# MrOlm/inStrain

Measured on AMD Instinct MI355X. Metric: Gbp profiled/s, higher is better.
Workload: dtype u32

## Files before the change

include/instrain_amd.h:

```cpp
#ifndef INSTRAIN_AMD_H
#define INSTRAIN_AMD_H

#include <stdint.h>

#ifdef __cplusplus
extern "C" {
#endif

#define ISX_OK 0
#define ISX_ERR_ARG (-1)
#define ISX_ERR_HIP (-2)
#define ISX_ERR_CAPACITY (-3)
#define ISX_ERR_MM_RANGE (-4)
#define ISX_ERR_IO (-5)
#define ISX_ERR_STATE (-6)

#define ISX_ABI_VERSION 5


typedef struct isx_ctx isx_ctx;
typedef struct isx_batch isx_batch;
typedef struct isx_bam isx_bam;
struct isx_bam_params_s;
struct isx_bam_info_s;
// ... 231 lines not shown
int isx_genes_create(isx_ctx *ctx, int64_t n_genes, const isx_gene *genes, const char *seq, int64_t seq_bytes, isx_genes **out);
void isx_genes_destroy(isx_genes *g);
int isx_genes_sites(isx_genes *g, double *sites, float *device_ms);
int isx_batch_profile_genes(isx_batch *b, isx_genes *g, int32_t n_scaffolds, const int64_t *scaffold_bounds, const int32_t *gene_first,
                            const int32_t *gene_last, isx_gene_cov *cov_out, uint8_t *scaffold_flags, float *device_ms);
int isx_genes_profile_snvs(isx_genes *g, int32_t n_scaffolds, const int64_t *scaffold_bounds, const int32_t *gene_first,
                           const int32_t *gene_last, int64_t n_snv, const isx_snv *snv, int32_t n_levels, isx_gene_mutation *mut_out,
                           isx_gene_snv_count *cnt_out, float *device_ms);

typedef struct isx_pipe isx_pipe;

typedef struct {
    int64_t max_pos;
    int64_t max_obs;
    int32_t max_splits;
    int32_t depth;
    int32_t host_threads;
    int32_t pin_threads;
    double jump_slack;
    int32_t want_counts;
    int32_t ring_kib;
    int32_t stage_async;
    int32_t lean_output;
    int64_t max_segs;
} isx_pipe_params;

typedef struct {
    uint32_t gpos;
    float clon_rarefied;
} isx_rare;

typedef struct {
    uint32_t gpos;
    uint32_t coverage;
} isx_sat;

typedef struct {
    int64_t ticket;
    int64_t n_pos, n_obs;
    isx_sizes sizes;
    const uint16_t *coverage16;
    const float *clon;
    const isx_rare *rare;
    int64_t n_rare, n_saturated;
    const uint32_t *counts;
    const float *clon_rarefied;
    const isx_snv *snv;
    isx_batch *batch;
    float encode_ms;
    float h2d_ms, kernel_ms, d2h_ms;
    float collect_wait_ms;
    int32_t record_bytes;
    int32_t encode_passes;
    int64_t h2d_bytes, d2h_bytes;
    const isx_ld *ld;
    const uint8_t *coverage8;
    const isx_rare *clon_sparse;
    int64_t n_clon;
    const isx_sat *saturated;
    const uint8_t *coverage4;
    const uint16_t *cov_rows;
    const uint32_t *cov_row_window;
    int64_t n_cov_rows;
    int32_t cov_window, pad_cov;
    const void *lev_mask;
    const void *lev_cov;
    const uint32_t *lev_win_off;
    const isx_rare *lev_clon, *lev_rare;
    const isx_sat *lev_sat;
    int64_t n_lev, n_lev_clon, n_lev_rare, n_lev_sat;
    int32_t lev_mask_bytes, lev_cov_bytes, lev_window, n_lev_windows, lev_min_cov, pad_lev;
    uint64_t rows_checksum;
} isx_pipe_result;

int isx_levels_expand(const isx_pipe_result *r, int32_t host_threads, uint32_t *gpos, uint32_t *mm_cov, float *clon, float *clon_rarefied);

int isx_pipe_create(isx_ctx *ctx, const isx_params *params, const isx_pipe_params *pp, isx_pipe **out);
void isx_pipe_destroy(isx_pipe *p);
int isx_pipe_submit(isx_pipe *p, int64_t n_pos, const uint8_t *ref, int32_t n_splits, const int64_t *split_bounds,
                    int64_t n_obs, const isx_obs *obs, const uint32_t *pair, int64_t *ticket);
int isx_pipe_submit_bam(isx_pipe *p, isx_bam *bam, const struct isx_bam_params_s *bp, const int32_t *refs, int32_t n_refs,
                        const uint8_t *ref, int32_t n_splits, const int64_t *split_bounds, struct isx_bam_info_s *info,
                        int64_t *ticket);
int isx_pipe_collect(isx_pipe *p, int64_t ticket, isx_pipe_result *out);
int isx_pipe_release(isx_pipe *p, int64_t ticket);
int isx_pipe_fetch_entries(isx_pipe *p, int64_t ticket, isx_entry *out);
int isx_pipe_fetch_entries_shrunk(isx_pipe *p, int64_t ticket, uint32_t *gpos, uint32_t *mm_cov, float *clon, float *clon_rarefied);


#define ISX_SEG_BASES 150
#define ISX_SEG_WORDS 15
#define ISX_SEG_SKIP_WORD 0x24924924u
#define ISX_DREC_WORDS 8
#define ISX_DREC_EXC 6
#define ISX_DREC_EXC_FULL 3
#define ISX_DREC_DUAL 0x80000000u
#define ISX_DREC_NO_EXC 0x3FFFFFFFu

typedef struct {
    int64_t n_seg;
    const uint32_t *gpos;
    const uint8_t *len;
    const uint8_t *mm;
    const uint32_t *pair;
    const uint32_t *bases;
} isx_segs;

int isx_batch_create_reads(isx_ctx *ctx, const isx_params *params, int64_t n_pos, const uint8_t *ref, int32_t n_splits,
                           const int64_t *split_bounds, const isx_segs *segs, isx_batch **out);
int isx_pipe_submit_reads(isx_pipe *p, int64_t n_pos, const uint8_t *ref, int32_t n_splits, const int64_t *split_bounds,
                          const isx_segs *segs, int64_t *ticket);

typedef struct isx_wire isx_wire;
int isx_pipe_stage_reads(isx_pipe *p, int64_t n_pos, const uint8_t *ref, int32_t n_splits, const int64_t *split_bounds,
                         const isx_segs *segs, isx_wire **out);
int isx_pipe_submit_wire(isx_pipe *p, const isx_wire *wire, int64_t *ticket);
int64_t isx_wire_bytes(const isx_wire *wire);
void isx_wire_free(isx_wire *wire);
int isx_wire_keep_reference(isx_pipe *p, isx_wire *wire);

#define ISX_PLANE_WORDS 8
typedef struct {
    int64_t n_seg;
    const uint32_t *gpos;
    const uint8_t *len;
    const uint32_t *pair;
    const uint64_t *planes;
    const uint8_t *mm;
} isx_read_planes;

typedef struct {
    const uint8_t *plane2;
    const uint8_t *nplane;
    uint64_t key;
} isx_ref_planes;

int isx_pack_ref_planes(const uint8_t *ref, int64_t n_pos, int32_t host_threads, uint8_t *plane2, uint8_t *nplane, int32_t *has_n);
int isx_planes_from_segs(const isx_segs *segs, int32_t host_threads, uint64_t *planes);
int isx_pack_read_planes(int64_t n_reads, const int64_t *ref_start, const int64_t *clip_lo, const int64_t *clip_hi,
                         const uint32_t *cigar, const int64_t *cigar_off, const char *seq, const uint8_t *qual, const int64_t *seq_off,
                         const uint32_t *pair, int32_t min_base_quality, int64_t cap_seg, uint32_t *seg_gpos,
                         uint8_t *seg_len, uint32_t *seg_pair, uint64_t *seg_planes, int64_t *n_seg);
int isx_pipe_submit_planes(isx_pipe *p, int64_t n_pos, const isx_ref_planes *ref, int32_t n_splits, const int64_t *split_bounds,
                           const isx_read_planes *reads, int64_t *ticket);
int isx_pipe_stage_planes(isx_pipe *p, int64_t n_pos, const isx_ref_planes *ref, int32_t n_splits, const int64_t *split_bounds,
                          const isx_read_planes *reads, isx_wire **out);
int isx_pipe_set_reference_budget(isx_pipe *p, int64_t mib);
int isx_host_register(const void *ptr, int64_t bytes);
int isx_host_unregister(const void *ptr);
int isx_encode_planes(const isx_read_planes *reads, const isx_ref_planes *ref, int64_t n_pos, int32_t host_threads, int32_t slack_groups,
                      int64_t cap_rec, int64_t ring_records, uint32_t *rec, uint32_t *gbase, int64_t *n_rec, int64_t *need_slack);
int isx_encode_planes_mm(const isx_read_planes *reads, const isx_ref_planes *ref, int64_t n_pos, int32_t n_mm_bins, int32_t host_threads, int32_t slack_groups,
                         int64_t cap_rec, int64_t ring_records, uint32_t *rec, uint32_t *gbase, int64_t *n_rec, int64_t *need_slack);

int isx_count_read_segs(int64_t n_reads, const uint32_t *cigar, const int64_t *cigar_off, const int64_t *ref_start,
                        const int64_t *clip_lo, const int64_t *clip_hi, int64_t *n_seg);
int isx_pack_reads(int64_t n_reads, const int64_t *ref_start, const int64_t *clip_lo, const int64_t *clip_hi,
                   const uint32_t *cigar, const int64_t *cigar_off, const char *seq, const uint8_t *qual, const int64_t *seq_off,
                   const uint8_t *mm, const uint32_t *pair, int32_t min_base_quality, int64_t cap_seg, uint32_t *seg_gpos,
                   uint8_t *seg_len, uint8_t *seg_mm, uint32_t *seg_pair, uint32_t *seg_bases, int64_t *n_seg);

int isx_encode_segs(const isx_segs *segs, int64_t n_pos, int32_t n_mm_bins, int32_t host_threads, int64_t cap_rec, uint32_t *rec,
                    uint32_t *gbase, uint32_t *pair_out, int64_t *n_rec);
int64_t isx_seg_records_needed(const uint32_t *gpos, int64_t n_seg, int32_t host_threads);
int isx_encode_segs_ring(const isx_segs *segs, int64_t n_pos, int32_t n_mm_bins, int32_t host_threads, int64_t cap_rec, int64_t ring_records,
                         uint32_t *rec, uint32_t *gbase, uint32_t *pair_out, int64_t *n_rec);

int isx_encode_delta(const isx_segs *segs, const uint8_t *ref, int64_t n_pos, int32_t n_mm_bins, int32_t host_threads, int32_t slack_groups,
                     int64_t cap_rec, int64_t ring_records, uint32_t *rec, uint32_t *gbase, uint32_t *pair_out, int64_t *n_rec, int64_t *need_slack);
int64_t isx_delta_records_needed(const uint32_t *gpos, int64_t n_seg, int32_t host_threads, int32_t slack_groups);

int isx_encode_obs(const isx_obs *obs, const uint32_t *pair, int64_t n_obs, int64_t n_pos, int32_t record_bytes,
                   int32_t host_threads, double slack, int64_t cap_rec, void *rec, uint32_t *gbase, uint32_t *pair_out,
                   int64_t *n_rec, int32_t *passes);
int isx_encode_obs_ring(const isx_obs *obs, const uint32_t *pair, int64_t n_obs, int64_t n_pos, int32_t record_bytes,
                        int32_t host_threads, double slack, int64_t cap_rec, int64_t ring_records, void *rec,
                        uint32_t *gbase, uint32_t *pair_out, int64_t *n_rec, int32_t *passes);

typedef struct {
    int64_t in_off;
    int32_t in_len;
    int32_t out_len;
    int64_t out_off;
} isx_bgzf_block;
int isx_bgzf_index(const uint8_t *image, int64_t n_bytes, int64_t cap_blocks, isx_bgzf_block *blocks, int64_t *n_blocks, int64_t *out_bytes);
int isx_bgzf_inflate_device(isx_ctx *ctx, const uint8_t *image, int64_t n_bytes, const isx_bgzf_block *blocks, int64_t n_blocks,
                            uint8_t *out, int64_t out_bytes, float *kernel_ms);
int isx_bgzf_inflate_host(const uint8_t *image, int64_t n_bytes, const isx_bgzf_block *blocks, int64_t n_blocks, uint8_t *out, int64_t out_bytes);
int isx_bgzf_inflate_fast(const uint8_t *image, int64_t n_bytes, const isx_bgzf_block *blocks, int64_t n_blocks, uint8_t *out, int64_t out_bytes);

typedef struct isx_bam_params_s {
    double min_read_ani;
    int32_t min_mapq;
    double max_insert_relative;
    int32_t min_insert;
    int32_t min_base_quality;
    int32_t skip_mm;
    int32_t window_length;
    int32_t pairing_filter;
} isx_bam_params;

typedef struct isx_bam_info_s {
    int32_t n_refs;
    int32_t n_splits;
    int64_t n_reads;
    int64_t n_pos;
    int64_t n_obs;
    int64_t n_pairs;
    int64_t unfiltered_pairs, filtered_pairs;
    int64_t filtered_bases;
    double median_insert;
    int32_t max_mm;
    int32_t pad;
    int64_t unfiltered_reads, unfiltered_singletons, filtered_singletons;
    int64_t n_segs;
} isx_bam_info;

int isx_bam_open(const char *path, isx_bam **out);
void isx_bam_close(isx_bam *bam);
void isx_bam_close_wait(isx_bam *bam);
int isx_bam_set_threads(isx_bam *bam, int32_t threads);
int isx_bam_ref(const isx_bam *bam, int32_t i, const char **name, int64_t *length, int64_t *flat_offset);
int isx_bam_set_priority_reads(isx_bam *bam, int64_t n, const char *names, const int64_t *offs);
int isx_bam_scan(isx_bam *bam, isx_bam_info *info );
int isx_bam_scan_part(isx_bam *bam, int32_t part, int32_t n_parts, isx_bam_info *info );
int isx_bam_set_wanted_refs(isx_bam *bam, const int32_t *refs, int32_t n);
int isx_bam_insert_sizes(isx_bam *bam, int64_t *out, int64_t cap, int64_t *n);
int isx_bam_filter(isx_bam *bam, const isx_bam_params *p, double median_insert , isx_bam_info *info);
int isx_bam_pair_keys(isx_bam *bam, uint64_t *h1, uint64_t *h2, int32_t *tid, int64_t *info4, int64_t cap, int64_t *n);
int isx_bam_set_cross_names(isx_bam *bam, int64_t n, const int64_t *entry, const int64_t *occurrences, const int64_t *info4);
int isx_bam_filter_insert_sizes(isx_bam *bam, int64_t *out, int64_t cap, int64_t *n);
int isx_bam_set_r2m(isx_bam *bam, int32_t ref, int64_t n, const char *names, const int64_t *offs, const int32_t *mm );
int isx_bam_set_mm_cap(isx_bam *bam, int32_t cap);
int isx_bam_mm_levels(const isx_bam *bam, int32_t *levels, int32_t cap, int32_t *n);
int isx_bam_set_mm_levels(isx_bam *bam, const int32_t *levels, int32_t n);
int isx_bam_batch_pair_names(const isx_bam *bam, int64_t *n, int64_t *name_bytes, char *names, int64_t *offs);
int isx_bam_r2m(const isx_bam *bam, int32_t ref, int64_t *n, int64_t *name_bytes, char *names, int64_t *offs, int32_t *mm);
int isx_bam_drop_names(isx_bam *bam);
int isx_bam_ref_counts(const isx_bam *bam, int64_t *reads, int64_t *filtered_pairs);
int isx_bam_expand_refs(isx_bam *bam, const isx_bam_params *p, const int32_t *refs, int32_t n_refs, isx_bam_info *info);
int isx_bam_segment_refs(isx_bam *bam, const isx_bam_params *p, const int32_t *refs, int32_t n_refs, isx_bam_info *info, int64_t *n_seg);
int isx_bam_copy_segs(const isx_bam *bam, uint32_t *gpos, uint8_t *len, uint8_t *mm, uint32_t *pair, uint32_t *bases,
                      int64_t *split_bounds, int32_t *split_ref);
int isx_bam_copy_read_planes(const isx_bam *bam, uint64_t *planes);
int isx_bam_expand_region(isx_bam *bam, const isx_bam_params *p, int32_t ref, int64_t start, int64_t stop, isx_bam_info *info);
int isx_bam_expand(isx_bam *bam, const isx_bam_params *p, isx_bam_info *info);
int isx_bam_copy(const isx_bam *bam, isx_obs *obs, uint32_t *pair, int64_t *split_bounds, int32_t *split_ref);
int isx_bam_view(const isx_bam *bam, const isx_obs **obs, const uint32_t **pair);

#ifdef __cplusplus
}
#endif
#endif
```

instrain_amd/_lib.py:

```python
import ctypes as C
import os

import numpy as np

_HERE = os.path.dirname(os.path.abspath(__file__))
LIB_PATH = os.path.join(_HERE, "libinstrain_amd.so")
if os.environ.get("ISX_LIB"):
    LIB_PATH = os.path.abspath(os.environ["ISX_LIB"])

BGZF_BLOCK_DT = np.dtype([("in_off", np.int64), ("in_len", np.int32), ("out_len", np.int32), ("out_off", np.int64)])
OBS_DT = np.dtype([("gpos", "<u4"), ("mm", "<u2"), ("base", "u1"), ("flags", "u1")])
ENTRY_DT = np.dtype([("gpos", "<u4"), ("mm", "<u2"), ("flags", "<u2"), ("cnt", "<u4", (4,)), ("clon", "<f4"),
                     ("clon_rarefied", "<f4")])
SNV_DT = np.dtype([("gpos", "<u4"), ("mm", "<u2"), ("con_base", "u1"), ("var_base", "u1"),
                   ("allele_count", "u1"), ("cls", "u1"), ("cryptic", "u1"), ("ref_base", "u1"),
                   ("cnt", "<u4", (4,))])
LD_DT = np.dtype([("gpos_a", "<u4"), ("gpos_b", "<u4"), ("mm", "<u2"), ("allele_A", "u1"), ("allele_a", "u1"),
                  ("allele_B", "u1"), ("allele_b", "u1"), ("pad", "<u2"), ("total", "<u4"), ("countAB", "<u4"),
                  ("countAb", "<u4"), ("countaB", "<u4"), ("countab", "<u4"), ("pad2", "<u4"),
                  ("r2", "<f8"), ("d_prime", "<f8"), ("r2_normalized", "<f8"), ("d_prime_normalized", "<f8")])
AO_DT = np.dtype([("pair", "<u4"), ("gpos", "<u4"), ("order", "<u4"), ("mm", "<u2"), ("base", "u1"), ("pad", "u1")])
assert AO_DT.itemsize == 16
assert OBS_DT.itemsize == 8 and ENTRY_DT.itemsize == 32 and SNV_DT.itemsize == 28 and LD_DT.itemsize == 72


class Params(C.Structure):
    _fields_ = [("min_cov", C.c_int32), ("min_snp", C.c_int32), ("min_freq", C.c_double),
                ("rarefied_coverage", C.c_int32), ("n_mm_bins", C.c_int32), ("enable_linkage", C.c_int32),
                ("linkage_mode", C.c_int32), ("window", C.c_int32), ("seed", C.c_uint64), ("layout", C.c_int32),
                ("reserved", C.c_int32)]


LAYOUT_WIDE_RECORDS, LAYOUT_NO_SHORT_RECORDS, LAYOUT_NO_PACKED_COUNTERS, LAYOUT_SEG64_RECORDS = 1, 2, 4, 8


class PipeParams(C.Structure):
    _fields_ = [("max_pos", C.c_int64), ("max_obs", C.c_int64), ("max_splits", C.c_int32), ("depth", C.c_int32),
                ("host_threads", C.c_int32), ("pin_threads", C.c_int32), ("jump_slack", C.c_double),
                ("want_counts", C.c_int32), ("ring_kib", C.c_int32), ("stage_async", C.c_int32), ("lean_output", C.c_int32),
                ("max_segs", C.c_int64)]


SEG_BASES, SEG_WORDS, SEG_SKIP_WORD = 150, 15, 0x24924924


class Segs(C.Structure):
    _fields_ = [("n_seg", C.c_int64), ("gpos", C.c_void_p), ("len", C.c_void_p), ("mm", C.c_void_p), ("pair", C.c_void_p),
                ("bases", C.c_void_p)]


PLANE_WORDS = 8
LAYOUT_MM_ENTRIES = 16
LAYOUT_MM_DELTA_RECORDS = 32
ABI_VERSION = 5


class ReadPlanes(C.Structure):
    _fields_ = [("n_seg", C.c_int64), ("gpos", C.c_void_p), ("len", C.c_void_p), ("pair", C.c_void_p), ("planes", C.c_void_p), ("mm", C.c_void_p)]


class RefPlanes(C.Structure):
    _fields_ = [("plane2", C.c_void_p), ("nplane", C.c_void_p), ("key", C.c_uint64)]


RARE_DT = np.dtype([("gpos", "<u4"), ("clon_rarefied", "<f4")])
CLON_DT = np.dtype([("gpos", "<u4"), ("clon", "<f4")])
SAT_DT = np.dtype([("gpos", "<u4"), ("coverage", "<u4")])


class Sizes(C.Structure):
    _fields_ = [(n, C.c_int64) for n in ("n_entries", "n_snv", "n_sites", "n_allele_obs", "n_increments",
                                         "n_edges", "n_ld")]


class Timings(C.Structure):
    _fields_ = [(n, C.c_float) for n in ("pileup_ms", "sites_ms", "allele_ms", "group_ms", "incr_ms", "ld_ms",
                                         "total_ms")] + \
               [(n, C.c_int32) for n in ("pileup_blocks", "pileup_threads", "pileup_lds_bytes", "pileup_window")] + \
               [("mfma_ms", C.c_float), ("dense_tiles", C.c_int32), ("dense_macs", C.c_int64), ("dense_bytes", C.c_int64),
                ("record_bytes", C.c_int32), ("pad", C.c_int32)]


class PipeResult(C.Structure):
    _fields_ = [("ticket", C.c_int64), ("n_pos", C.c_int64), ("n_obs", C.c_int64), ("sizes", Sizes),
                ("coverage16", C.c_void_p), ("clon", C.c_void_p), ("rare", C.c_void_p), ("n_rare", C.c_int64),
                ("n_saturated", C.c_int64), ("counts", C.c_void_p), ("clon_rarefied", C.c_void_p), ("snv", C.c_void_p),
                ("batch", C.c_void_p),
                ("encode_ms", C.c_float), ("h2d_ms", C.c_float), ("kernel_ms", C.c_float), ("d2h_ms", C.c_float),
                ("collect_wait_ms", C.c_float), ("record_bytes", C.c_int32), ("encode_passes", C.c_int32),
                ("h2d_bytes", C.c_int64), ("d2h_bytes", C.c_int64), ("ld", C.c_void_p),
                ("coverage8", C.c_void_p), ("clon_sparse", C.c_void_p), ("n_clon", C.c_int64), ("saturated", C.c_void_p),
                ("coverage4", C.c_void_p), ("cov_rows", C.c_void_p), ("cov_row_window", C.c_void_p), ("n_cov_rows", C.c_int64),
                ("cov_window", C.c_int32), ("pad_cov", C.c_int32),
                ("lev_mask", C.c_void_p), ("lev_cov", C.c_void_p), ("lev_win_off", C.c_void_p), ("lev_clon", C.c_void_p), ("lev_rare", C.c_void_p),
                ("lev_sat", C.c_void_p), ("n_lev", C.c_int64), ("n_lev_clon", C.c_int64), ("n_lev_rare", C.c_int64), ("n_lev_sat", C.c_int64),
                ("lev_mask_bytes", C.c_int32), ("lev_cov_bytes", C.c_int32), ("lev_window", C.c_int32), ("n_lev_windows", C.c_int32),
                ("lev_min_cov", C.c_int32), ("pad_lev", C.c_int32), ("rows_checksum", C.c_uint64)]


class BamParams(C.Structure):
    _fields_ = [("min_read_ani", C.c_double), ("min_mapq", C.c_int32), ("max_insert_relative", C.c_double),
                ("min_insert", C.c_int32), ("min_base_quality", C.c_int32), ("skip_mm", C.c_int32),
                ("window_length", C.c_int32), ("pairing_filter", C.c_int32)]


PAIRING_FILTERS = {"paired_only": 0, "non_discordant": 1, "all_reads": 2}


class BamInfo(C.Structure):
    _fields_ = [("n_refs", C.c_int32), ("n_splits", C.c_int32), ("n_reads", C.c_int64), ("n_pos", C.c_int64),
                ("n_obs", C.c_int64), ("n_pairs", C.c_int64), ("unfiltered_pairs", C.c_int64),
                ("filtered_pairs", C.c_int64), ("filtered_bases", C.c_int64), ("median_insert", C.c_double),
                ("max_mm", C.c_int32), ("pad", C.c_int32), ("unfiltered_reads", C.c_int64),
                ("unfiltered_singletons", C.c_int64), ("filtered_singletons", C.c_int64), ("n_segs", C.c_int64)]


SCAFFOLD_LEVEL_DT = np.dtype([("nonzero", "<i8"), ("sum_cov", "<u8"), ("sumsq_cov", "<u8"), ("median_cov", "<f8"),
                              ("counted", "<i8"), ("sum_clon", "<f8"), ("median_clon", "<f8"),
                              ("counted_rarefied", "<i8"), ("sum_clon_rarefied", "<f8"),
                              ("median_clon_rarefied", "<f8"), ("mm", "<i4"), ("present", "<i4")])
assert SCAFFOLD_LEVEL_DT.itemsize == 88
GENOME_LEVEL_DT = np.dtype([("n", "<i8"), ("sum_cov", "<u8"), ("sumsq_cov", "<u8"), ("median_cov", "<f8"), ("mm", "<i4"), ("pad", "<i4")])
assert GENOME_LEVEL_DT.itemsize == 40
GENOME_COV_DT = np.dtype([("n", "<i8"), ("sum_cov", "<u8"), ("sumsq_cov", "<u8"), ("max_cov", "<u4"), ("pad", "<u4")])
SNV_LEVEL_DT = np.dtype([(n, "<u4") for n in ("divergent", "sns", "snv", "con", "pop")])
LD_LEVEL_DT = np.dtype([("n", "<i8"), ("n_r2", "<i8"), ("n_dprime", "<i8"), ("sum_distance", "<i8"), ("sum_r2", "<f8"), ("sum_dprime", "<f8")])
assert GENOME_COV_DT.itemsize == 32 and SNV_LEVEL_DT.itemsize == 20 and LD_LEVEL_DT.itemsize == 48


COMPARE_LEVEL_DT = np.dtype([("both", "<i8"), ("either", "<i8"), ("mm", "<i4"), ("present_a", "<i4"),
                             ("present_b", "<i4"), ("pad", "<i4"), ("consensus_snps", "<i8"), ("population_snps", "<i8")])
assert COMPARE_LEVEL_DT.itemsize == 48
COMPARE_SNP_DT = np.dtype([("gpos", "<u4"), ("mm", "<u2"), ("consensus_snp", "u1"), ("population_snp", "u1"),
                           ("has_a", "u1"), ("has_b", "u1"), ("con_a", "u1"), ("ref_a", "u1"), ("var_a", "u1"),
                           ("con_b", "u1"), ("ref_b", "u1"), ("var_b", "u1"), ("cnt_a", "<u4", (4,)), ("cnt_b", "<u4", (4,))])
assert COMPARE_SNP_DT.itemsize == 48


GENE_DT = np.dtype([("start", "<i8"), ("end", "<i8"), ("seq_off", "<i8"), ("strand", "<i4"), ("pad", "<i4")])
GENE_COV_DT = np.dtype([("sum_cov", "<u8"), ("nonzero", "<u4"), ("counted", "<u4"), ("sum_clon", "<f8")])
GENE_SNV_COUNT_DT = np.dtype([(n, "<u4") for n in ("divergent", "sns", "sns_n", "sns_s", "snv", "snv_n", "snv_s")])
GENE_MUTATION_DT = np.dtype([("gene", "<i4"), ("k", "<i4"), ("type", "u1"), ("aa_old", "u1"), ("aa_new", "u1"), ("n_genes", "u1"),
                             ("pad", "<u4")])
assert GENE_DT.itemsize == 32 and GENE_COV_DT.itemsize == 24 and GENE_SNV_COUNT_DT.itemsize == 28 and GENE_MUTATION_DT.itemsize == 16
GENE_LEVEL_PRESENT, GENE_COV_ANY, GENE_CLON_ANY = 1, 2, 4


ERR_CAPACITY = -3


class IsxError(RuntimeError):
    def __init__(self, code, msg):
        super().__init__("libinstrain_amd error %d: %s" % (code, msg))
        self.code = code


SYMBOLS = ["isx_last_error", "isx_abi_version", "isx_ctx_create", "isx_ctx_destroy", "isx_ctx_reserve_cus", "isx_set_null_model",
           "isx_batch_create", "isx_batch_create_reads", "isx_batch_destroy", "isx_batch_run", "isx_batch_launch", "isx_batch_wait", "isx_batch_sizes", "isx_batch_timings",
           "isx_batch_fetch_entries", "isx_batch_fetch_dense", "isx_batch_fetch_snv", "isx_batch_fetch_ld", "isx_batch_fetch_allele_obs",
           "isx_batch_summarize", "isx_batch_summarize_genomes", "isx_batch_genome_coverage", "isx_snv_level_counts", "isx_ld_level_sums", "isx_compare_coverage", "isx_compare_scaffolds", "isx_compare_fetch_snps",
           "isx_genes_create", "isx_genes_destroy", "isx_genes_sites", "isx_batch_profile_genes", "isx_genes_profile_snvs",
           "isx_pipe_create", "isx_pipe_destroy", "isx_pipe_submit", "isx_pipe_submit_reads", "isx_pipe_stage_reads", "isx_pipe_submit_wire", "isx_wire_bytes", "isx_wire_free", "isx_wire_keep_reference", "isx_pipe_submit_bam", "isx_encode_segs", "isx_encode_segs_ring", "isx_seg_records_needed", "isx_encode_delta", "isx_delta_records_needed", "isx_count_read_segs", "isx_pack_reads", "isx_pipe_collect", "isx_pipe_release", "isx_pipe_fetch_entries", "isx_pipe_fetch_entries_shrunk", "isx_levels_expand", "isx_encode_obs", "isx_encode_obs_ring",
           "isx_pack_ref_planes", "isx_planes_from_segs", "isx_pack_read_planes", "isx_pipe_submit_planes", "isx_pipe_stage_planes", "isx_encode_planes", "isx_encode_planes_mm", "isx_pipe_set_reference_budget", "isx_host_register", "isx_host_unregister",
           "isx_bgzf_index", "isx_bgzf_inflate_device", "isx_bgzf_inflate_host", "isx_bgzf_inflate_fast",
           "isx_bam_open", "isx_bam_close", "isx_bam_close_wait", "isx_bam_set_threads", "isx_bam_ref", "isx_bam_set_priority_reads", "isx_bam_scan", "isx_bam_scan_part",
           "isx_bam_insert_sizes", "isx_bam_set_wanted_refs", "isx_bam_pair_keys", "isx_bam_set_cross_names", "isx_bam_filter_insert_sizes", "isx_bam_filter", "isx_bam_set_r2m", "isx_bam_r2m", "isx_bam_drop_names", "isx_bam_batch_pair_names", "isx_bam_set_mm_cap", "isx_bam_mm_levels", "isx_bam_set_mm_levels", "isx_bam_ref_counts",
           "isx_bam_expand_refs", "isx_bam_segment_refs", "isx_bam_copy_segs", "isx_bam_copy_read_planes", "isx_bam_expand_region", "isx_bam_expand", "isx_bam_copy", "isx_bam_view"]

_lib = None


def load():
    global _lib
    if _lib is not None:
        return _lib
    if not os.path.exists(LIB_PATH):
        raise IsxError(-2, "%s not built: run `python -c 'import __graft_entry__ as g; g.build()'` "
                           "(hipcc --offload-arch=gfx950)" % LIB_PATH)
    lib = C.CDLL(LIB_PATH)
    vp, i32, i64 = C.c_void_p, C.c_int32, C.c_int64
    lib.isx_last_error.restype = C.c_char_p
    lib.isx_abi_version.restype = C.c_int
    if lib.isx_abi_version() != ABI_VERSION:
        raise IsxError(-6, "%s has ABI version %d, this package binds version %d: rebuild it (python -c 'import __graft_entry__ as g; g.build()')"
                       % (LIB_PATH, lib.isx_abi_version(), ABI_VERSION))
    lib.isx_ctx_create.argtypes = [C.c_int, C.POINTER(vp)]
    lib.isx_ctx_destroy.argtypes = [vp]
    lib.isx_ctx_reserve_cus.argtypes = [vp, C.c_int]
    lib.isx_bgzf_index.argtypes = [vp, i64, i64, vp, C.POINTER(i64), C.POINTER(i64)]
    lib.isx_bgzf_inflate_device.argtypes = [vp, vp, i64, vp, i64, vp, i64, C.POINTER(C.c_float)]
    lib.isx_bgzf_inflate_host.argtypes = [vp, i64, vp, i64, vp, i64]
    lib.isx_bgzf_inflate_fast.argtypes = [vp, i64, vp, i64, vp, i64]
    lib.isx_ctx_destroy.restype = None
    lib.isx_set_null_model.argtypes = [vp, vp, i64, i32]
    lib.isx_batch_create.argtypes = [vp, C.POINTER(Params), i64, vp, i32, vp, i64, vp, vp, C.POINTER(vp)]
    lib.isx_batch_create_reads.argtypes = [vp, C.POINTER(Params), i64, vp, i32, vp, C.POINTER(Segs), C.POINTER(vp)]
    lib.isx_pipe_submit_reads.argtypes = [vp, i64, vp, i32, vp, C.POINTER(Segs), C.POINTER(i64)]
    lib.isx_pipe_stage_reads.argtypes = [vp, i64, vp, i32, vp, C.POINTER(Segs), C.POINTER(vp)]
    lib.isx_pipe_submit_wire.argtypes = [vp, vp, C.POINTER(i64)]
    lib.isx_wire_bytes.argtypes = [vp]
    lib.isx_wire_bytes.restype = i64
    lib.isx_wire_free.argtypes = [vp]
    lib.isx_wire_keep_reference.argtypes = [vp, vp]
    lib.isx_wire_free.restype = None
    lib.isx_encode_segs.argtypes = [C.POINTER(Segs), i64, i32, i32, i64, vp, vp, vp, C.POINTER(i64)]
    lib.isx_encode_segs_ring.argtypes = [C.POINTER(Segs), i64, i32, i32, i64, i64, vp, vp, vp, C.POINTER(i64)]
    lib.isx_encode_delta.argtypes = [C.POINTER(Segs), vp, i64, i32, i32, i32, i64, i64, vp, vp, vp, C.POINTER(i64), C.POINTER(i64)]
    lib.isx_delta_records_needed.argtypes = [vp, i64, i32, i32]
    lib.isx_delta_records_needed.restype = i64
    lib.isx_seg_records_needed.argtypes = [vp, i64, i32]
    lib.isx_seg_records_needed.restype = i64
    lib.isx_count_read_segs.argtypes = [i64, vp, vp, vp, vp, vp, C.POINTER(i64)]
    lib.isx_pack_reads.argtypes = [i64, vp, vp, vp, vp, vp, vp, vp, vp, vp, vp, i32, i64, vp, vp, vp, vp, vp, C.POINTER(i64)]
    lib.isx_batch_destroy.argtypes = [vp]
    lib.isx_batch_destroy.restype = None
    lib.isx_batch_run.argtypes = [vp]
    lib.isx_batch_launch.argtypes = [vp]
    lib.isx_batch_wait.argtypes = [vp]
    lib.isx_batch_sizes.argtypes = [vp, C.POINTER(Sizes)]
    lib.isx_batch_timings.argtypes = [vp, C.POINTER(Timings)]
    for f in ("isx_batch_fetch_entries", "isx_batch_fetch_snv", "isx_batch_fetch_ld", "isx_batch_fetch_allele_obs"):
        getattr(lib, f).argtypes = [vp, vp]
    lib.isx_batch_fetch_dense.argtypes = [vp, vp, vp, vp]
    lib.isx_batch_summarize.argtypes = [vp, i32, vp, vp, C.POINTER(C.c_float)]
    lib.isx_batch_summarize_genomes.argtypes = [vp, i32, vp, i32, vp, i32, vp, C.POINTER(C.c_float)]
    lib.isx_batch_genome_coverage.argtypes = [vp, i32, vp, vp, i32, i32, i32, vp, vp, C.POINTER(C.c_float)]
    lib.isx_snv_level_counts.argtypes = [vp, i32, vp, i64, vp, i32, vp, C.POINTER(C.c_float)]
    lib.isx_ld_level_sums.argtypes = [vp, i32, vp, i64, vp, i32, vp, C.POINTER(C.c_float)]
    lib.isx_compare_coverage.argtypes = [vp, vp, i32, vp, i32, vp, C.POINTER(C.c_float)]
    lib.isx_compare_scaffolds.argtypes = [vp, vp, i32, vp, i32, C.c_double, vp, C.POINTER(i64), C.POINTER(C.c_float)]
    lib.isx_compare_fetch_snps.argtypes = [vp, vp]
    lib.isx_genes_create.argtypes = [vp, i64, vp, C.c_char_p, i64, C.POINTER(vp)]
    lib.isx_genes_destroy.argtypes = [vp]
    lib.isx_genes_destroy.restype = None
    lib.isx_genes_sites.argtypes = [vp, vp, C.POINTER(C.c_float)]
    lib.isx_batch_profile_genes.argtypes = [vp, vp, i32, vp, vp, vp, vp, vp, C.POINTER(C.c_float)]
    lib.isx_genes_profile_snvs.argtypes = [vp, i32, vp, vp, vp, i64, vp, i32, vp, vp, C.POINTER(C.c_float)]
    lib.isx_pipe_create.argtypes = [vp, C.POINTER(Params), C.POINTER(PipeParams), C.POINTER(vp)]
    lib.isx_pipe_destroy.argtypes = [vp]
    lib.isx_pipe_destroy.restype = None
    lib.isx_pipe_submit.argtypes = [vp, i64, vp, i32, vp, i64, vp, vp, C.POINTER(i64)]
    lib.isx_pipe_submit_bam.argtypes = [vp, vp, C.POINTER(BamParams), vp, i32, vp, i32, vp, C.POINTER(BamInfo), C.POINTER(i64)]
    lib.isx_pipe_collect.argtypes = [vp, i64, C.POINTER(PipeResult)]
    lib.isx_pipe_release.argtypes = [vp, i64]
    lib.isx_pipe_fetch_entries.argtypes = [vp, i64, vp]
    lib.isx_pipe_fetch_entries_shrunk.argtypes = [vp, i64, vp, vp, vp, vp]
    lib.isx_levels_expand.argtypes = [C.POINTER(PipeResult), i32, vp, vp, vp, vp]
    lib.isx_encode_obs.argtypes = [vp, vp, i64, i64, i32, i32, C.c_double, i64, vp, vp, vp, C.POINTER(i64), C.POINTER(i32)]
    lib.isx_encode_obs_ring.argtypes = [vp, vp, i64, i64, i32, i32, C.c_double, i64, i64, vp, vp, vp, C.POINTER(i64), C.POINTER(i32)]
    lib.isx_bam_open.argtypes = [C.c_char_p, C.POINTER(vp)]
    lib.isx_bam_close.argtypes = [vp]
    lib.isx_bam_close.restype = None
    lib.isx_bam_close_wait.argtypes = [vp]
    lib.isx_bam_close_wait.restype = None
    lib.isx_bam_expand.argtypes = [vp, C.POINTER(BamParams), C.POINTER(BamInfo)]
    lib.isx_bam_set_threads.argtypes = [vp, i32]
    lib.isx_bam_set_priority_reads.argtypes = [vp, i64, C.c_char_p, vp]
    lib.isx_bam_scan.argtypes = [vp, C.POINTER(BamInfo)]
    lib.isx_bam_scan_part.argtypes = [vp, i32, i32, C.POINTER(BamInfo)]
    lib.isx_bam_set_wanted_refs.argtypes = [vp, vp, i32]
    lib.isx_bam_insert_sizes.argtypes = [vp, vp, i64, C.POINTER(i64)]
    lib.isx_bam_filter_insert_sizes.argtypes = [vp, vp, i64, C.POINTER(i64)]
    lib.isx_bam_pair_keys.argtypes = [vp, vp, vp, vp, vp, i64, C.POINTER(i64)]
    lib.isx_bam_set_cross_names.argtypes = [vp, i64, vp, vp, vp]
    lib.isx_bam_filter.argtypes = [vp, C.POINTER(BamParams), C.c_double, C.POINTER(BamInfo)]
    lib.isx_bam_set_r2m.argtypes = [vp, i32, i64, C.c_char_p, vp, vp]
    lib.isx_bam_drop_names.argtypes = [vp]
    lib.isx_bam_r2m.argtypes = [vp, i32, C.POINTER(i64), C.POINTER(i64), vp, vp, vp]
    lib.isx_bam_batch_pair_names.argtypes = [vp, C.POINTER(i64), C.POINTER(i64), vp, vp]
    lib.isx_bam_set_mm_cap.argtypes = [vp, i32]
    lib.isx_bam_mm_levels.argtypes = [vp, vp, i32, vp]
    lib.isx_bam_set_mm_levels.argtypes = [vp, vp, i32]
    lib.isx_bam_ref_counts.argtypes = [vp, vp, vp]
    lib.isx_bam_expand_region.argtypes = [vp, C.POINTER(BamParams), i32, i64, i64, C.POINTER(BamInfo)]
    lib.isx_bam_expand_refs.argtypes = [vp, C.POINTER(BamParams), vp, i32, C.POINTER(BamInfo)]
    lib.isx_bam_segment_refs.argtypes = [vp, C.POINTER(BamParams), vp, i32, C.POINTER(BamInfo), C.POINTER(i64)]
    lib.isx_bam_copy_segs.argtypes = [vp, vp, vp, vp, vp, vp, vp, vp]
    lib.isx_bam_copy_read_planes.argtypes = [vp, vp]
    lib.isx_pack_ref_planes.argtypes = [vp, i64, i32, vp, vp, C.POINTER(i32)]
    lib.isx_planes_from_segs.argtypes = [C.POINTER(Segs), i32, vp]
    lib.isx_pack_read_planes.argtypes = [i64, vp, vp, vp, vp, vp, vp, vp, vp, vp, i32, i64, vp, vp, vp, vp, C.POINTER(i64)]
    lib.isx_pipe_submit_planes.argtypes = [vp, i64, C.POINTER(RefPlanes), i32, vp, C.POINTER(ReadPlanes), C.POINTER(i64)]
    lib.isx_pipe_set_reference_budget.argtypes = [vp, i64]
    lib.isx_host_register.argtypes = [vp, i64]
    lib.isx_host_unregister.argtypes = [vp]
    lib.isx_pipe_stage_planes.argtypes = [vp, i64, C.POINTER(RefPlanes), i32, vp, C.POINTER(ReadPlanes), C.POINTER(vp)]
    lib.isx_encode_planes.argtypes = [C.POINTER(ReadPlanes), C.POINTER(RefPlanes), i64, i32, i32, i64, i64, vp, vp, C.POINTER(i64), C.POINTER(i64)]
    lib.isx_encode_planes_mm.argtypes = [C.POINTER(ReadPlanes), C.POINTER(RefPlanes), i64, i32, i32, i32, i64, i64, vp, vp, C.POINTER(i64), C.POINTER(i64)]
    lib.isx_bam_ref.argtypes = [vp, i32, C.POINTER(C.c_char_p), C.POINTER(i64), C.POINTER(i64)]
    lib.isx_bam_copy.argtypes = [vp, vp, vp, vp, vp]
    lib.isx_bam_view.argtypes = [vp, C.POINTER(vp), C.POINTER(vp)]
    _lib = lib
    return lib


def check(rc):
    if rc != 0:
        raise IsxError(rc, load().isx_last_error().decode(errors="replace"))
```

instrain_amd/csrc/isx_api.hip:

```cpp
#include <algorithm>
#include <atomic>
#include <cmath>
#include <chrono>
#include <cstdlib>
#include <cstring>
#include <map>
#include <mutex>
#include <string>
#include <unordered_map>
#include <thread>
#include <type_traits>
#include <vector>
#include <unistd.h>
#include <sys/prctl.h>
#include <time.h>

#include "isx_batch.h"
#include "seg_encode.h"

static thread_local std::string g_err;
void isx_set_error(const std::string &msg) { g_err = msg; }

namespace {
struct BlockCache {
// ... 19 lines not shown
        const size_t m = (v + (((size_t)1 << e) - 1)) >> e;
        return m << e;
    }
    int current() const
    {
        int d = -1;
        if (per_device && hipGetDevice(&d) != hipSuccess) d = -1;
        return d;
    }
    void trim(int dev = -2)
    {
        std::vector<std::pair<int, void *>> dead;
        {
            std::lock_guard<std::mutex> lk(mu);
            for (auto it = free_blocks.begin(); it != free_blocks.end();) {
                if (dev < -1 || it->first.dev == dev) {
                    dead.emplace_back(it->first.dev, it->second);
                    cached[it->first.dev] -= it->first.cls;
                    it = free_blocks.erase(it);
                } else ++it;
            }
        }
        int keep = -1;
        const bool sw = per_device && hipGetDevice(&keep) == hipSuccess;
        for (auto &d : dead) {
            if (sw && d.first >= 0) (void)hipSetDevice(d.first);
            (void)raw_free(d.second);
        }
        if (sw && keep >= 0) (void)hipSetDevice(keep);
    }
    hipError_t get(void **p, size_t bytes)
    {
        const Key k{current(), class_of(bytes)};
        {
            std::lock_guard<std::mutex> lk(mu);
            auto it = free_blocks.find(k);
            if (it != free_blocks.end()) {
                *p = it->second;
                free_blocks.erase(it);
                cached[k.dev] -= k.cls;
                live[*p] = k;
                return hipSuccess;
            }
        }
        hipError_t e = raw_alloc(p, k.cls);
        if (e != hipSuccess) {
            (void)hipGetLastError();
            trim();
            e = raw_alloc(p, k.cls);
            if (e != hipSuccess) return e;
        }
        std::lock_guard<std::mutex> lk(mu);
        live[*p] = k;
        return hipSuccess;
    }
    void put(void *p)
    {
        if (!p) return;
        {
            std::lock_guard<std::mutex> lk(mu);
            auto it = live.find(p);
            if (it != live.end()) {
                const Key k = it->second;
                live.erase(it);
                if (cached[k.dev] + k.cls <= limit_of(k.dev)) { free_blocks.emplace(k, p); cached[k.dev] += k.cls; return; }
            }
        }
        (void)raw_free(p);
    }
};
hipError_t raw_dev_alloc(void **p, size_t n) { return hipMalloc(p, n); }
hipError_t raw_dev_free(void *p) { return hipFree(p); }
hipError_t raw_pin_alloc(void **p, size_t n) { return hipHostMalloc(p, n, hipHostMallocDefault); }
hipError_t raw_pin_free(void *p) { return hipHostFree(p); }
size_t dev_limit(int dev)
{
    static std::mutex mu;
    static std::map<int, size_t> lim;
    std::lock_guard<std::mutex> lk(mu);
    auto it = lim.find(dev);
    if (it != lim.end()) return it->second;
    size_t v = (size_t)8 << 30;
    hipDeviceProp_t pr;
    if (dev >= 0 && hipGetDeviceProperties(&pr, dev) == hipSuccess) v = pr.totalGlobalMem / 6;
    else (void)hipGetLastError();
    lim[dev] = v;
    return v;
}
size_t pin_limit(int)
{
    static const size_t v = [] {
        const long pages = sysconf(_SC_PHYS_PAGES), psz = sysconf(_SC_PAGE_SIZE);
        const size_t ram = pages > 0 && psz > 0 ? (size_t)pages * (size_t)psz : (size_t)64 << 30;
        return std::min<size_t>((size_t)8 << 30, ram / 8);
    }();
    return v;
}
BlockCache &dev_cache() { static BlockCache c(true, dev_limit, raw_dev_alloc, raw_dev_free); return c; }
BlockCache &pin_cache() { static BlockCache c(false, pin_limit, raw_pin_alloc, raw_pin_free); return c; }
}

hipError_t isx_dev_malloc(void **p, size_t bytes) { return dev_cache().get(p, bytes); }
void isx_dev_free(void *p) { dev_cache().put(p); }
hipError_t isx_pin_malloc(void **p, size_t bytes) { return pin_cache().get(p, bytes); }
void isx_pin_free(void *p) { pin_cache().put(p); }
void isx_dev_trim() { dev_cache().trim(); pin_cache().trim(); }
hipError_t isx_raw_dev_malloc(void **p, size_t bytes)
{
    hipError_t e = hipMalloc(p, bytes);
    if (e != hipSuccess) {
        (void)hipGetLastError();
        dev_cache().trim();
        e = hipMalloc(p, bytes);
    }
    return e;
}

namespace {
struct HostRange { uintptr_t a; size_t n; };
std::mutex g_hreg_mu;
std::vector<HostRange> g_hreg;
}

bool isx_host_is_registered(const void *ptr, size_t bytes)
{
    if (!ptr || !bytes) return false;
    const uintptr_t a = reinterpret_cast<uintptr_t>(ptr);
    std::lock_guard<std::mutex> lk(g_hreg_mu);
    for (const HostRange &r : g_hreg) if (a >= r.a && a + bytes <= r.a + r.n) return true;
    return false;
}

extern "C" int isx_host_register(const void *ptr, int64_t bytes)
{
    if (!ptr || bytes <= 0) { isx_set_error("isx_host_register: bad argument"); return ISX_ERR_ARG; }
    const uintptr_t a = reinterpret_cast<uintptr_t>(ptr);
    const uintptr_t pa = a & ~(uintptr_t)4095, pe = (a + (size_t)bytes + 4095) & ~(uintptr_t)4095;
    std::lock_guard<std::mutex> lk(g_hreg_mu);
    for (const HostRange &r : g_hreg) {
        const uintptr_t ra = r.a & ~(uintptr_t)4095, re = (r.a + r.n + 4095) & ~(uintptr_t)4095;
        if (pa < re && ra < pe) { isx_set_error("isx_host_register: the range shares a page with a registered one"); return ISX_ERR_ARG; }
    }
    HIP_TRY(hipHostRegister(const_cast<void *>(ptr), (size_t)bytes, hipHostRegisterDefault));
    g_hreg.push_back(HostRange{a, (size_t)bytes});
    return ISX_OK;
}

extern "C" int isx_host_unregister(const void *ptr)
{
    const uintptr_t a = reinterpret_cast<uintptr_t>(ptr);
    std::lock_guard<std::mutex> lk(g_hreg_mu);
    for (size_t i = 0; i < g_hreg.size(); i++)
        if (g_hreg[i].a == a) {
            g_hreg.erase(g_hreg.begin() + (long)i);
            HIP_TRY(hipHostUnregister(const_cast<void *>(ptr)));
            return ISX_OK;
        }
    isx_set_error("isx_host_unregister: not a registered range");
    return ISX_ERR_ARG;
}

namespace {
__global__ void __launch_bounds__(256) k_copy_out(uint4 *__restrict__ dst, const uint4 *__restrict__ src, size_t n16)
{
    typedef uint32_t u32x4 __attribute__((ext_vector_type(4)));
    const size_t stride = (size_t)gridDim.x * blockDim.x;
    for (size_t i = (size_t)blockIdx.x * blockDim.x + threadIdx.x; i < n16; i += stride) {
        const u32x4 v = __builtin_nontemporal_load(reinterpret_cast<const u32x4 *>(src) + i);
        reinterpret_cast<u32x4 *>(dst)[i] = v;
    }
}
}

namespace {
template <class T>
__global__ void __launch_bounds__(256) k_copy_small(T *__restrict__ dst, const T *__restrict__ src, size_t n)
{
    const size_t stride = (size_t)gridDim.x * blockDim.x;
    for (size_t i = (size_t)blockIdx.x * blockDim.x + threadIdx.x; i < n; i += stride) dst[i] = src[i];
}
}

hipError_t isx_copy_to_host(void *hdst, const void *dsrc, size_t bytes, hipStream_t stream)
{
    static const size_t dma_min = [] { const char *e = getenv("ISX_D2H_DMA_MIN"); return e ? (size_t)atoll(e) : (size_t)1 << 20; }();
    return isx_copy_to_host_route(hdst, dsrc, bytes, stream, bytes < dma_min);
}

hipError_t isx_copy_to_host_route(void *hdst, const void *dsrc, size_t bytes, hipStream_t stream, bool by_kernel)
{
    if (!bytes) return hipSuccess;
    if (!by_kernel) return hipMemcpyAsync(hdst, dsrc, bytes, hipMemcpyDeviceToHost, stream);
    const uintptr_t both = reinterpret_cast<uintptr_t>(hdst) | reinterpret_cast<uintptr_t>(dsrc);
    size_t done = 0;
    if ((both & 15) == 0 && bytes >= 4096) {
        const size_t n16 = bytes / 16;
        const int blocks = (int)std::min<size_t>(128, (n16 + 1023) / 1024);
        hipLaunchKernelGGL(k_copy_out, dim3(blocks), dim3(256), 0, stream, static_cast<uint4 *>(hdst), static_cast<const uint4 *>(dsrc), n16);
        done = n16 * 16;
    }
    if (done < bytes) {
        const size_t rest = bytes - done;
        uint8_t *d = static_cast<uint8_t *>(hdst) + done;
        const uint8_t *s = static_cast<const uint8_t *>(dsrc) + done;
        const bool words = (((both | rest) & 3) == 0);
        const size_t n = words ? rest / 4 : rest;
        const int blocks = (int)std::min<size_t>(64, (n + 255) / 256);
        if (words) hipLaunchKernelGGL(k_copy_small<uint32_t>, dim3(blocks), dim3(256), 0, stream, reinterpret_cast<uint32_t *>(d), reinterpret_cast<const uint32_t *>(s), n);
        else hipLaunchKernelGGL(k_copy_small<uint8_t>, dim3(blocks), dim3(256), 0, stream, d, s, n);
    }
    return hipGetLastError();
}

namespace {
__global__ void __launch_bounds__(256) k_copy_counted(uint4 *__restrict__ dst, const uint4 *__restrict__ src, const uint32_t *cursor,
                                                      uint32_t base, uint32_t row_bytes, uint64_t cap_rows)
{
    const uint64_t rows = min((uint64_t)(*cursor - base), cap_rows);
    const uint64_t n16 = (rows * row_bytes + 15) / 16;
    const uint64_t stride = (uint64_t)gridDim.x * blockDim.x;
    for (uint64_t i = (uint64_t)blockIdx.x * blockDim.x + threadIdx.x; i < n16; i += stride) dst[i] = src[i];
}
}

hipError_t isx_copy_rows_to_host(void *hdst, const void *dsrc, const uint32_t *d_cursor, uint32_t base, uint32_t row_bytes,
                                 size_t cap_rows, hipStream_t stream)
{
    if (!cap_rows) return hipSuccess;
    if (((reinterpret_cast<uintptr_t>(hdst) | reinterpret_cast<uintptr_t>(dsrc)) & 15) != 0) return hipErrorInvalidValue;
    const size_t n16 = (cap_rows * row_bytes + 15) / 16;
    const int blocks = (int)std::min<size_t>(64, (n16 + 1023) / 1024);
    hipLaunchKernelGGL(k_copy_counted, dim3(std::max(blocks, 1)), dim3(256), 0, stream, static_cast<uint4 *>(hdst), static_cast<const uint4 *>(dsrc),
                       d_cursor, base, row_bytes, (uint64_t)cap_rows);
    return hipGetLastError();
}

namespace {
struct CopyJobs { uint4 *dst[ISX_COPY_JOBS]; const uint4 *src[ISX_COPY_JOBS]; uint32_t n16[ISX_COPY_JOBS]; uint32_t first[ISX_COPY_JOBS + 1]; int n; };
__global__ void __launch_bounds__(256) k_copy_multi(const CopyJobs J)
{
    int j = 0;
    while (j + 1 < J.n && blockIdx.x >= J.first[j + 1]) j++;
    const uint32_t nb = J.first[j + 1] - J.first[j], lb = blockIdx.x - J.first[j];
    for (uint32_t i = lb * 256u + threadIdx.x; i < J.n16[j]; i += nb * 256u) J.dst[j][i] = J.src[j][i];
}
}

hipError_t isx_copy_multi_to_host(const isx_copy_job *jobs, int n, hipStream_t stream)
{
    CopyJobs J{};
    uint32_t blocks = 0;
    for (int i = 0; i < n && J.n < ISX_COPY_JOBS; i++) {
        if (!jobs[i].bytes) continue;
        if (((reinterpret_cast<uintptr_t>(jobs[i].dst) | reinterpret_cast<uintptr_t>(jobs[i].src)) & 15) != 0 || jobs[i].bytes > ((size_t)1 << 35)) return hipErrorInvalidValue;
        const uint32_t n16 = (uint32_t)((jobs[i].bytes + 15) / 16);
        J.dst[J.n] = static_cast<uint4 *>(jobs[i].dst); J.src[J.n] = static_cast<const uint4 *>(jobs[i].src); J.n16[J.n] = n16;
        J.first[J.n] = blocks;
        blocks += std::max<uint32_t>(1, std::min<uint32_t>(64, (n16 + 1023) / 1024));
        J.n++;
    }
    if (!J.n) return hipSuccess;
    J.first[J.n] = blocks;
    hipLaunchKernelGGL(k_copy_multi, dim3(blocks), dim3(256), 0, stream, J);
    return hipGetLastError();
}

namespace {
struct ReadBack {
    uint8_t *pin = nullptr;
    size_t used = 0;
    struct Item { void *dst; size_t off, bytes; };
    std::vector<Item> items;
    bool batching = false;
    std::vector<isx_copy_job> jobs;
    static constexpr size_t CAP = (size_t)1 << 20;
    ~ReadBack() { if (pin) isx_pin_free(pin); }
};
thread_local ReadBack g_rb;
}

void isx_read_batch(bool on) { g_rb.batching = on; }

hipError_t isx_read_back(void *host_dst, const void *dsrc, size_t bytes, hipStream_t stream)
{
    if (!bytes) return hipSuccess;
    ReadBack &rb = g_rb;
    if (!rb.pin && isx_pin_malloc(reinterpret_cast<void **>(&rb.pin), ReadBack::CAP) != hipSuccess) rb.pin = nullptr;
    const size_t off = (rb.used + 15) & ~(size_t)15;
    if (!rb.pin || off + ((bytes + 15) & ~(size_t)15) > ReadBack::CAP) {
        const hipError_t e = hipMemcpyAsync(host_dst, dsrc, bytes, hipMemcpyDeviceToHost, stream);
        if (e != hipSuccess) { rb.items.clear(); rb.jobs.clear(); rb.used = 0; }
        return e;
    }
    if (rb.batching && (reinterpret_cast<uintptr_t>(dsrc) & 15) == 0 && rb.jobs.size() < ISX_COPY_JOBS) {
        rb.jobs.push_back(isx_copy_job{rb.pin + off, dsrc, bytes});
    } else {
        const hipError_t e = isx_copy_to_host(rb.pin + off, dsrc, bytes, stream);
        if (e != hipSuccess) { rb.items.clear(); rb.jobs.clear(); rb.used = 0; return e; }
    }
    rb.items.push_back({host_dst, off, bytes});
    rb.used = off + bytes;
    return hipSuccess;
}

void isx_read_drop()
{
    g_rb.items.clear();
    g_rb.jobs.clear();
// ... 1531 lines not shown
```

instrain_amd/csrc/isx_pipe.hip:

```cpp
#include <atomic>
#include <algorithm>
#include <chrono>
#include <cmath>
#include <condition_variable>
#include <cstring>
#include <deque>
#include <mutex>
#include <memory>
#include <string>
#include <thread>
#include <vector>

#include "bam_front.h"
#include "isx_batch.h"
#include "obs_encode.h"
#include "seg_encode.h"
#include "isx_summary.h"
#include <unordered_map>

namespace {

constexpr size_t ALIGN = 256;
inline size_t up(size_t v, size_t a = ALIGN) { return (v + a - 1) / a * a; }

double now_ms()
{
    return std::chrono::duration<double, std::milli>(std::chrono::steady_clock::now().time_since_epoch()).count();
}

int host_block_alloc(void **p, size_t bytes, bool pinned)
{
    *p = nullptr;
    if (pinned) { HIP_TRY(isx_pin_malloc(p, std::max<size_t>(bytes, 1))); return ISX_OK; }
    if (posix_memalign(p, 4096, std::max<size_t>(bytes, 4096)) != 0) { *p = nullptr; isx_set_error("out of host memory"); return ISX_ERR_ARG; }
    return ISX_OK;
}

void host_block_free(void *p, bool pinned)
{
    if (!p) return;
    if (pinned) isx_pin_free(p); else free(p);
}

static const bool pipe_timing = getenv("ISX_PIPE_TIMING") != nullptr;
#define H2D(p, s) ((s).h2d ? (s).h2d : (p)->s_h2d)
struct Slot {
    isx_batch *b = nullptr;
    hipStream_t h2d = nullptr;
    uint8_t *h_in = nullptr, *d_in = nullptr;
    size_t in_bytes = 0;
    size_t off_bounds = 0, off_win = 0, off_ref = 0, off_gbase = 0, off_ridx = 0, off_rec = 0;
    size_t off_pairs = 0;
    isxenc::PairRun *h_runs = nullptr;
    bool runs_pinned = true;
    uint2 *d_runs = nullptr;
    size_t cap_runs = 0;
    hipEvent_t ev_ring[2] = {nullptr, nullptr};
    bool ring_busy[2] = {false, false};
    uint8_t *h_out = nullptr;
    uint8_t *h_small = nullptr;
    size_t small_bytes = 0;
    bool out_pinned = true;
    size_t out_bytes = 0, o_counts = 0, o_clon = 0, o_clonr = 0, o_snv = 0, o_cov16 = 0, o_rare = 0;
    bool rare_dense = false;
    bool cov8 = false, clon_sparse = false;
    bool cov4 = false;
    size_t cov_rows_off = 0;
    int cov_window = 0;
    std::vector<uint32_t> cov_row_win;
    std::vector<isx_sat> sat_rows;
    bool sat_complete = true;
    void *sort_temp = nullptr;
    size_t sort_temp_bytes = 0;
    std::vector<float> clonr_big;
    std::vector<isx_rare> rare_big;
    std::vector<uint32_t> cmin, cmax, dir_pmax, dir_smin;
    std::vector<uint8_t> cany;
    std::vector<uint2> win;
    size_t o_lmask = 0, o_lwin = 0, o_lcov = 0, o_lclon = 0, o_lrare = 0;
    size_t lcov_room = 0, lclon_room = 0, lrare_room = 0;
    std::vector<uint8_t> lcov_big;
    std::vector<isx_rare> lclon_big, lrare_big;
    std::vector<isx_snv> snv_big;
    std::vector<isx_ld> ld_rows;
    uint64_t rows_checksum = 0;
    hipEvent_t ev_h2d0 = nullptr, ev_h2d1 = nullptr, ev_pass = nullptr, ev_d2h0 = nullptr, ev_d2h1 = nullptr;
    hipEvent_t ev_h2da = nullptr, ev_h2db = nullptr;
    bool h2d_split = false;
    int64_t ticket = -1;
    BamBatch *dead_batch = nullptr;
    bool ref_has_n = false;
    int state = 0;
    int rc = 0;
    std::string err;
    float finish_wait_ms = 0.f;
    float encode_ms = 0.f;
    int encode_passes = 0;
    int64_t h2d_bytes = 0, d2h_bytes = 0;
    uint16_t *d_gpos16 = nullptr;
};

static uint64_t bytes_checksum(const void *p, size_t bytes, uint64_t seed)
{
    const uint8_t *b = static_cast<const uint8_t *>(p);
    uint64_t a[4] = {seed ^ 0x9E3779B97F4A7C15ull, seed + 0xC2B2AE3D27D4EB4Full, seed ^ 0x165667B19E3779F9ull, seed + 0x27D4EB2F165667C5ull};
    const size_t n8 = bytes / 8;
    size_t i = 0;
    for (; i + 4 <= n8; i += 4) {
        uint64_t w[4];
        memcpy(w, b + 8 * i, 32);
        for (int k = 0; k < 4; k++) a[k] = a[k] * 0x100000001B3ull + w[k];
    }
    uint64_t h = (uint64_t)bytes;
    for (; i < n8; i++) { uint64_t w; memcpy(&w, b + 8 * i, 8); h = h * 0x100000001B3ull + w; }
    for (size_t j = n8 * 8; j < bytes; j++) h = h * 0x100000001B3ull + b[j];
    for (int k = 0; k < 4; k++) { h ^= a[k]; h *= 0xFF51AFD7ED558CCDull; h ^= h >> 33; }
    return h;
}

static inline size_t ref2_bytes(int64_t n_pos) { return (((size_t)n_pos + 3) / 4 + 15) & ~(size_t)15; }
static inline size_t refn_bytes(int64_t n_pos) { return (((size_t)n_pos + 7) / 8 + 15) & ~(size_t)15; }

static bool copy_ref_planes(isxenc::HostPool &pool, const isx_ref_planes *rp, int64_t n_pos, uint8_t *plane2, uint8_t *nplane)
{
    const size_t b2 = ((size_t)n_pos + 3) / 4, bn = ((size_t)n_pos + 7) / 8;
    const size_t piece = (size_t)1 << 20;
    const int t2 = (int)((b2 + piece - 1) / piece), tn = rp->nplane ? (int)((bn + piece - 1) / piece) : 0;
    std::atomic<int> any{0};
    pool.run(t2 + tn, [&](int t) {
        if (t < t2) { const size_t a = (size_t)t * piece; memcpy(plane2 + a, rp->plane2 + a, std::min(piece, b2 - a)); return; }
        const size_t a = (size_t)(t - t2) * piece, n = std::min(piece, bn - a);
        const uint8_t *src = rp->nplane + a;
        uint8_t acc = 0;
        for (size_t i = 0; i < n; i++) acc |= src[i];
        memcpy(nplane + a, src, n);
        if (acc) any.store(1, std::memory_order_relaxed);
    });
    return any.load() != 0;
}

static bool plane_any(isxenc::HostPool &pool, const uint8_t *pl, size_t bytes)
{
    const size_t piece = (size_t)1 << 20;
    const int nt = (int)((bytes + piece - 1) / piece);
    std::atomic<int> any{0};
    pool.run(nt, [&](int t) {
        const size_t a = (size_t)t * piece, n = std::min(piece, bytes - a);
        uint64_t acc = 0;
        size_t i = 0;
        for (; i + 8 <= n; i += 8) { uint64_t v; memcpy(&v, pl + a + i, 8); acc |= v; }
        for (; i < n; i++) acc |= pl[a + i];
        if (acc) any.store(1, std::memory_order_relaxed);
    });
    return any.load() != 0;
}

static uint64_t ref_plane_checksum(const uint8_t *plane2, int64_t n_pos)
{
    const size_t words = (((size_t)n_pos + 3) / 4) / 8;
    uint64_t h = 0x9E3779B97F4A7C15ull ^ (uint64_t)n_pos;
    if (!words) { for (size_t i = 0; i < ((size_t)n_pos + 3) / 4; i++) h = (h ^ plane2[i]) * 0x100000001B3ull; return h; }
    const size_t n_s = std::min<size_t>(words, 4096), step = words / n_s;
    for (size_t k = 0; k < n_s; k++) {
        uint64_t w;
        memcpy(&w, plane2 + 8 * (k * step), 8);
        h = (h ^ w) * 0x100000001B3ull;
        h ^= h >> 29;
    }
    return h;
}

int cgroup_cpus()
{
    if (FILE *f = fopen("/sys/fs/cgroup/cpu.max", "r")) {
        char q[64] = {0};
        long period = 0;
        const int n = fscanf(f, "%63s %ld", q, &period);
        fclose(f);
        if (n == 2 && period > 0 && strcmp(q, "max") != 0) return (int)std::max<long>(1, atol(q) / period);
    }
    return 0;
}

int gpu_numa_node(int device)
{
    char bus[64] = {0};
    if (hipDeviceGetPCIBusId(bus, sizeof bus, device) != hipSuccess) return -1;
    std::string id(bus);
    std::transform(id.begin(), id.end(), id.begin(), [](unsigned char ch) { return (char)std::tolower(ch); });
    int node = -1;
    if (FILE *f = fopen(("/sys/bus/pci/devices/" + id + "/numa_node").c_str(), "r")) {
        if (fscanf(f, "%d", &node) != 1) node = -1;
        fclose(f);
    }
    return node;
}

}

struct isx_pipe {
    isx_ctx *ctx = nullptr;
    isx_params prm{};
    isx_pipe_params pp{};
    std::unique_ptr<isxenc::HostPool> pool;
    std::vector<Slot> slots;
// ... 83 lines not shown
    }
    if (p->finisher.joinable()) {
        { std::lock_guard<std::mutex> lk(p->mu); p->stop = true; }
        p->cv_work.notify_all();
        p->finisher.join();
        if (p->finisher2.joinable()) p->finisher2.join();
        for (auto &t : p->more_finishers) if (t.joinable()) t.join();
    }
    (void)hipSetDevice(p->ctx->device);
    if (p->s_h2d) (void)isx_wait_stream(p->s_h2d);
    if (p->s_h2d2) (void)isx_wait_stream(p->s_h2d2);
    if (p->s_d2h) (void)isx_wait_stream(p->s_d2h);
    if (p->s_fin) (void)isx_wait_stream(p->s_fin);
    if (p->s_fin2) (void)isx_wait_stream(p->s_fin2);
    for (hipStream_t st : p->extra_fin) (void)isx_wait_stream(st);
    for (int i = 0; i < 2; i++) if (p->ctx->pstream[i]) (void)isx_wait_stream(p->ctx->pstream[i]);
    const double t_f0 = now_ms();
    double t_batch = 0, t_dev = 0, t_pin = 0;
    for (Slot &s : p->slots) {
        double t_x = now_ms();
        if (s.b) {
            isx_batch *b = s.b;
            b->d_seg = nullptr; b->d_drec = nullptr;
            b->d_rec = nullptr; b->d_rec32 = nullptr; b->d_rec16 = nullptr; b->d_gbase = nullptr; b->d_pair = nullptr;
            b->d_pair_runs = nullptr; b->d_run_index = nullptr;
            b->d_gpos = nullptr; b->d_gpos16 = nullptr; b->d_cbase = nullptr; b->d_ref = nullptr; b->d_win = nullptr;
            b->d_bounds = nullptr;
            isx_batch_destroy(b);
        }
        t_batch += now_ms() - t_x; t_x = now_ms();
        if (s.sort_temp) isx_dev_free(s.sort_temp);
        if (s.d_gpos16) isx_dev_free(s.d_gpos16);
        if (s.d_in) isx_dev_free(s.d_in);
        if (s.d_runs) isx_dev_free(s.d_runs);
        t_dev += now_ms() - t_x; t_x = now_ms();
        if (s.h_in) isx_pin_free(s.h_in);
        host_block_free(s.h_runs, s.runs_pinned);
        for (hipEvent_t e : s.ev_ring) if (e) (void)hipEventDestroy(e);
        host_block_free(s.h_out, s.out_pinned);
        if (s.h_small) isx_pin_free(s.h_small);
        t_pin += now_ms() - t_x;
        for (hipEvent_t e : {s.ev_h2d0, s.ev_h2d1, s.ev_pass, s.ev_d2h0, s.ev_d2h1, s.ev_h2da, s.ev_h2db}) if (e) (void)hipEventDestroy(e);
    }
    if (pipe_timing)
        fprintf(stderr, "[isx_pipe_destroy] device tables %.1f ms, device arena %.1f ms, pinned staging %.1f ms, total %.1f ms\n", t_batch, t_dev, t_pin, now_ms() - t_f0);
    for (auto &kv : p->ref_cache) { if (kv.second.d) isx_dev_free(kv.second.d); if (kv.second.ready) (void)hipEventDestroy(kv.second.ready); }
    for (int i = 0; i < 2; i++) {
        if (p->bounce[i]) isx_pin_free(p->bounce[i]);
        if (p->bounce_ev[i]) (void)hipEventDestroy(p->bounce_ev[i]);
    }
    if (p->s_h2d) (void)hipStreamDestroy(p->s_h2d);
    if (p->s_h2d2) (void)hipStreamDestroy(p->s_h2d2);
    if (p->s_d2h) (void)hipStreamDestroy(p->s_d2h);
    if (p->s_fin) (void)hipStreamDestroy(p->s_fin);
    if (p->s_fin2) (void)hipStreamDestroy(p->s_fin2);
    for (hipStream_t st : p->extra_fin) (void)hipStreamDestroy(st);
    delete p;
}

static int slot_batch_create(isx_pipe *p, Slot &s, int index)
{
    isx_ctx *c = p->ctx;
    const isx_params *prm = &p->prm;
    const double t_s0 = now_ms();
    isx_batch *b = new isx_batch();
    s.b = b;
    b->ctx = c; b->prm = *prm; b->M = prm->n_mm_bins;
    b->ps = getenv("ISX_ONE_PASS_QUEUE") ? 0 : (index & 1);
    b->cap_pos = p->pp.max_pos; b->cap_obs = p->pp.max_obs; b->arena = true; b->ref_packed = 2;
    b->n_pos = p->pp.max_pos; b->n_obs = p->pp.max_obs;
    b->segs = p->segs; b->drec = p->drec;
    b->lean = p->pp.lean_output != 0 && !p->pp.want_counts;
    b->lev_sparse = b->M > 1 && b->M <= 32 && p->segs && !p->pp.want_counts && !(prm->layout & ISX_LAYOUT_MM_ENTRIES);
    b->spin_us = (p->pp.host_threads > 0 && p->pp.host_threads < 8) ? 200 : 2000;
    const bool dense = b->M == 1;
    batch_pick_block(b);
    const int64_t cap_pos = p->pp.max_pos;
    for (auto &e : b->ev) HIP_TRY(hipEventCreate(&e));
    for (auto &e : b->ev_sum) HIP_TRY(hipEventCreate(&e));
    HIP_TRY(isx_dev_malloc(reinterpret_cast<void **>(&b->d_cursors), (CUR_N + 4) * sizeof(uint32_t)));
    b->d_flags = b->d_cursors + CUR_N;
    HIP_TRY(hipHostMalloc(&b->h_state, (CUR_N + 8) * sizeof(uint32_t), hipHostMallocMapped | hipHostMallocCoherent));
    memset(b->h_state, 0, (CUR_N + 8) * sizeof(uint32_t));
    HIP_TRY(hipHostGetDevicePointer(reinterpret_cast<void **>(&b->d_host_state), b->h_state, 0));
    HIP_TRY(hipMemset(b->d_cursors, 0, (CUR_N + 4) * sizeof(uint32_t)));
    {
        std::vector<uint16_t> thr = build_thresholds(c->h_lut, c->fallback, prm->min_freq);
        HIP_TRY(isx_dev_malloc(reinterpret_cast<void **>(&b->d_thr), thr.size() * sizeof(uint16_t)));
        HIP_TRY(hipMemcpy(b->d_thr, thr.data(), thr.size() * sizeof(uint16_t), hipMemcpyHostToDevice));
    }
    const uint64_t npm = (uint64_t)cap_pos * b->M;
    const uint64_t cap_obs = (uint64_t)std::max<int64_t>(p->pp.max_obs, 1);
    if (dense) {
        if (p->pp.want_counts) HIP_TRY(isx_dev_malloc(reinterpret_cast<void **>(&b->d_counts), (size_t)cap_pos * sizeof(uint4)));
        else {
            b->cap_clon = (size_t)cap_pos / 2 + 65536;
            HIP_TRY(isx_dev_malloc(reinterpret_cast<void **>(&b->d_cov8), (size_t)cap_pos));
            if (p->pp.lean_output) {
                b->cap_cov_row_win = (size_t)cap_pos / 64 + 2;
                HIP_TRY(isx_dev_malloc(reinterpret_cast<void **>(&b->d_cov_row_win), b->cap_cov_row_win * sizeof(uint32_t)));
            }
            HIP_TRY(isx_dev_malloc(reinterpret_cast<void **>(&b->d_clon_list), b->cap_clon * sizeof(uint2)));
            HIP_TRY(isx_dev_malloc(reinterpret_cast<void **>(&b->d_clon_sorted), b->cap_clon * sizeof(uint2)));
        }
        b->cap_sat = (size_t)cap_pos / 16 + 65536;
        HIP_TRY(isx_dev_malloc(reinterpret_cast<void **>(&b->d_sat), b->cap_sat * sizeof(uint2)));
        HIP_TRY(isx_dev_malloc(reinterpret_cast<void **>(&b->d_clon), (size_t)cap_pos * sizeof(float)));
        HIP_TRY(isx_dev_malloc(reinterpret_cast<void **>(&b->d_clon_r), (size_t)cap_pos * sizeof(float)));
        HIP_TRY(isx_dev_malloc(reinterpret_cast<void **>(&b->d_cov16), (size_t)cap_pos * sizeof(uint16_t)));
        if (prm->rarefied_coverage > 0) {
            b->cap_rare = p->cap_rare;
            HIP_TRY(isx_dev_malloc(reinterpret_cast<void **>(&b->d_rare), b->cap_rare * sizeof(uint2)));
        }
    } else if (b->lev_sparse) {
        b->lev_mask_bytes = b->M <= 8 ? 1 : (b->M <= 16 ? 2 : 4);
        b->cap_lev = (size_t)std::min<uint64_t>(std::min<uint64_t>(npm, 0xFFFFFFF0ull), std::max<uint64_t>((uint64_t)cap_pos * (uint64_t)std::min(b->M, 4), 1u << 20));
        HIP_TRY(isx_dev_malloc(&b->d_lev_mask, (size_t)cap_pos * b->lev_mask_bytes + 64));
        HIP_TRY(isx_dev_malloc(&b->d_lev_cov, b->cap_lev * 2 + 64));
        HIP_TRY(isx_dev_malloc(reinterpret_cast<void **>(&b->d_lev_win_off), ((size_t)cap_pos / 64 + 2) * sizeof(uint32_t)));
        if (!b->lean) {
            b->cap_entries = b->cap_lev;
            HIP_TRY(isx_dev_malloc(reinterpret_cast<void **>(&b->d_entries), b->cap_entries * sizeof(isx_entry)));
        }
        b->cap_clon = (size_t)cap_pos / 4 + 65536;
        HIP_TRY(isx_dev_malloc(reinterpret_cast<void **>(&b->d_clon_list), b->cap_clon * sizeof(uint2)));
        b->cap_sat = (size_t)cap_pos / 16 + 65536;
        HIP_TRY(isx_dev_malloc(reinterpret_cast<void **>(&b->d_sat), b->cap_sat * sizeof(uint2)));
        if (prm->rarefied_coverage > 0) {
            b->cap_rare = p->cap_rare;
            HIP_TRY(isx_dev_malloc(reinterpret_cast<void **>(&b->d_rare), b->cap_rare * sizeof(uint2)));
        }
    } else {
        b->slab_region = (size_t)(cap_pos + 2 * b->block) * (size_t)std::min(b->M, 4);
        const size_t ovf = b->M <= 4 ? 16 : (size_t)std::max<uint64_t>(1u << 20, std::min<uint64_t>(cap_obs, npm) / 4);
        if (b->slab_region + ovf >= 0xFFFFFFFFull) { isx_set_error("mm path: more than 2^32 entry slots in one batch"); return ISX_ERR_ARG; }
        b->cap_entries = b->slab_region + ovf;
        HIP_TRY(isx_dev_malloc(reinterpret_cast<void **>(&b->d_entries), b->cap_entries * sizeof(isx_entry)));
        HIP_TRY(isx_dev_malloc(reinterpret_cast<void **>(&b->d_win_nent), ((size_t)cap_pos / 64 + 2) * sizeof(uint32_t)));
    }
    b->cap_snv = (size_t)std::min<uint64_t>(npm, std::max<uint64_t>((uint64_t)cap_pos / 2, 1u << 20));
    b->cap_sites = (size_t)std::min<uint64_t>((uint64_t)cap_pos, std::max<uint64_t>((uint64_t)cap_pos / 4, 1u << 20));
    b->cap_ao = (size_t)std::max<uint64_t>(1, std::min<uint64_t>(cap_obs, std::max<uint64_t>(cap_obs / 4, 1u << 20)));
    HIP_TRY(isx_dev_malloc(reinterpret_cast<void **>(&b->d_snv), b->cap_snv * sizeof(isx_snv)));
    HIP_TRY(isx_dev_malloc(reinterpret_cast<void **>(&b->d_sites), b->cap_sites * sizeof(isx_site)));
    if (prm->enable_linkage) HIP_TRY(isx_dev_malloc(reinterpret_cast<void **>(&b->d_ao), b->cap_ao * sizeof(isx_ao)));
    if (!dense) {
        b->cap_slev = b->cap_sites * (size_t)std::min(b->M, 8);
        HIP_TRY(isx_dev_malloc(reinterpret_cast<void **>(&b->d_slev), b->cap_slev * sizeof(isx_slev)));
    }
    size_t o = 0;
    s.off_bounds = o; o = up(o + (size_t)(p->pp.max_splits + 1) * sizeof(int64_t));
    s.off_win = o; o = up(o + ((size_t)cap_pos / 64 + 2) * sizeof(uint2));
    s.off_ref = o; o = up(o + ref2_bytes(cap_pos) + refn_bytes(cap_pos));
    s.off_gbase = o; o = up(o + ((size_t)(p->cap_rec / p->G) + ISX_TAIL_GROUPS) * sizeof(uint32_t));
    s.off_ridx = o; if (prm->enable_linkage && !p->segs) o = up(o + ((size_t)p->cap_rec / ISX_CHUNK + 2) * sizeof(uint32_t));
    s.off_pairs = o; if (prm->enable_linkage && p->segs && !p->drec) o = up(o + (size_t)p->cap_rec * sizeof(uint32_t));
    s.off_rec = o;
    s.in_bytes = up(o + (size_t)p->cap_rec * p->rb + ISX_TAIL_BYTES);
    const size_t host_bytes = p->ring_half ? up(o + 2 * (size_t)p->ring_half * p->rb) : s.in_bytes;
    const double t_a0 = now_ms();
    HIP_TRY(isx_pin_malloc(reinterpret_cast<void **>(&s.h_in), host_bytes));
    const double t_a1 = now_ms();
    HIP_TRY(isx_dev_malloc(reinterpret_cast<void **>(&s.d_in), s.in_bytes));
    if (pipe_timing)
        fprintf(stderr, "[isx_pipe_create] slot %d: device tables %.1f ms, pinned input %.1f MB %.1f ms, device arena %.1f MB %.1f ms\n", index,
                t_a0 - t_s0, host_bytes / 1e6, t_a1 - t_a0, s.in_bytes / 1e6, now_ms() - t_a1);
    if (prm->enable_linkage && !p->segs) {
        s.cap_runs = (size_t)p->cap_rec / 64 + 4096;
        s.runs_pinned = p->pp.depth > 1;
        { const int hrc = host_block_alloc(reinterpret_cast<void **>(&s.h_runs), s.cap_runs * sizeof(isxenc::PairRun), s.runs_pinned); if (hrc != ISX_OK) return hrc; }
        HIP_TRY(isx_dev_malloc(reinterpret_cast<void **>(&s.d_runs), s.cap_runs * sizeof(uint2)));
    }
    if (p->ring_half) for (hipEvent_t &e : s.ev_ring) HIP_TRY(hipEventCreateWithFlags(&e, hipEventDisableTiming));
    if (prm->enable_linkage && p->rb == 4) HIP_TRY(isx_dev_malloc(reinterpret_cast<void **>(&s.d_gpos16), (size_t)p->cap_rec * sizeof(uint16_t)));
    o = 0;
    s.o_snv = o; o = up(o + p->snv_prefix * sizeof(isx_snv));
    s.o_rare = o; if (dense && prm->rarefied_coverage > 0) o = up(o + p->rare_prefix * sizeof(isx_rare));
    s.small_bytes = o;
    HIP_TRY(isx_pin_malloc(reinterpret_cast<void **>(&s.h_small), std::max<size_t>(s.small_bytes, 1)));
    o = 0;
    if (dense) {
        s.o_cov16 = o; o = up(o + (size_t)cap_pos * 2);
        s.o_clon = o; o = up(o + (size_t)cap_pos * 4);
        if (p->pp.want_counts) {
            s.o_counts = o; o = up(o + (size_t)cap_pos * 16);
            s.o_clonr = o; if (prm->rarefied_coverage > 0) o = up(o + (size_t)cap_pos * 4);
        }
    }
    if (b->lev_sparse) {
        s.o_lmask = o; o = up(o + (size_t)cap_pos * b->lev_mask_bytes);
        s.o_lwin = o; o = up(o + ((size_t)cap_pos / 64 + 2) * sizeof(uint32_t));
        s.lcov_room = (size_t)cap_pos * (size_t)std::min(b->M, 4);
        s.o_lcov = o; o = up(o + s.lcov_room);
        s.lclon_room = (size_t)cap_pos;
        s.o_lclon = o; o = up(o + s.lclon_room);
        s.lrare_room = prm->rarefied_coverage > 0 ? (size_t)cap_pos / 2 : 0;
        s.o_lrare = o; o = up(o + s.lrare_room);
    }
    s.out_bytes = o;
    const double t_o0 = now_ms();
    s.out_pinned = s.out_bytes <= ((size_t)64 << 20) || p->pp.depth > 2;
    { const int hrc = host_block_alloc(reinterpret_cast<void **>(&s.h_out), s.out_bytes, s.out_pinned); if (hrc != ISX_OK) return hrc; }
    if (pipe_timing) fprintf(stderr, "[isx_pipe_create] slot %d: %s results %.1f MB %.1f ms\n", index, s.out_pinned ? "pinned" : "pageable", s.out_bytes / 1e6, now_ms() - t_o0);
    for (hipEvent_t *e : {&s.ev_h2d0, &s.ev_h2d1, &s.ev_pass, &s.ev_d2h0, &s.ev_d2h1, &s.ev_h2da, &s.ev_h2db}) HIP_TRY(hipEventCreate(e));
    const size_t n_chunks = (size_t)(p->cap_rec / (p->segs ? (int64_t)p->G : (int64_t)ISX_CHUNK)) + 2;
    s.cmin.resize(n_chunks); s.cmax.resize(n_chunks); s.cany.resize(n_chunks);
    return ISX_OK;
}

static int finish_slot(isx_pipe *p, Slot &s, hipStream_t sfin)
{
    isx_ctx *c = p->ctx;
    isx_batch *b = s.b;
    const bool dense = b->M == 1;
    const double t0 = now_ms();
    HIP_TRY(isx_wait_event(s.ev_d2h1));
    s.finish_wait_ms = (float)(now_ms() - t0);
    const double t_c0 = now_ms();
    double t_fin = 0, t_rare = 0;
    hipStream_t ps = c->pstream[b->ps];
    bool redo = false;
    for (int attempt = 0;; attempt++) {
        uint32_t cf = 0;
        int rc = finish_pass_sizes(b, &cf, sfin);
        if (rc != ISX_OK) return rc;
        const bool cov8_overflow = !cf && dense && b->sparse_out && b->cov8_out && !b->nib_pass && (size_t)b->n_sat > b->cap_sat;
        const bool nib_overflow = !cf && dense && b->nib_pass &&
                                  ((size_t)b->n_pos / 2 + 128 + (size_t)b->n_cov_rows * (size_t)b->W * 2 > (size_t)b->n_pos * 2 ||
                                   ((size_t)b->n_cov_rows + 1) * (size_t)b->W > (size_t)(b->cap_pos ? b->cap_pos : b->n_pos));
        const bool clon_overflow = !cf && dense && b->sparse_out && b->lean && !b->clon_dense &&
                                   ((size_t)b->n_clon > b->cap_clon || (size_t)b->n_clon * 2 > (size_t)b->n_pos);
        const bool rare_overflow = !cf && dense && p->prm.rarefied_coverage > 0 && !b->rare_dense &&
                                   ((size_t)b->n_rare > p->cap_rare || (size_t)b->n_rare * 8 > (size_t)b->n_pos);
        const bool lev_overflow = !cf && b->lev_sparse && ((size_t)b->n_clon > b->cap_clon || (size_t)b->n_sat > b->cap_sat ||
                                                           (p->prm.rarefied_coverage > 0 && (size_t)b->n_rare > b->cap_rare));
        if (!cf && !cov8_overflow && !clon_overflow && !nib_overflow && !rare_overflow && !lev_overflow) break;
        if (attempt == 7) { isx_set_error("output tables still too small after 8 growth steps"); return ISX_ERR_CAPACITY; }
        if (cov8_overflow) b->cov8_out = false;
        if (nib_overflow) b->nib_out = false;
        if (clon_overflow) b->clon_dense = true;
        if (rare_overflow) b->rare_dense = true;
        if (cf && (rc = batch_grow_tables(b, cf)) != ISX_OK) return rc;
        if (lev_overflow) {
            auto regrow_list = [&](uint2 **lp, size_t *cap, size_t need) -> int {
                if (need <= *cap) return ISX_OK;
                HIP_TRY(isx_wait_stream(ps));
                if (*lp) isx_dev_free(*lp);
                *lp = nullptr;
                const size_t want = need + need / 4 + 65536;
                HIP_TRY(isx_dev_malloc(reinterpret_cast<void **>(lp), want * sizeof(uint2)));
                *cap = want;
                return ISX_OK;
            };
            if ((rc = regrow_list(&b->d_clon_list, &b->cap_clon, b->n_clon)) != ISX_OK) return rc;
            if ((rc = regrow_list(&b->d_sat, &b->cap_sat, b->n_sat)) != ISX_OK) return rc;
            if (p->prm.rarefied_coverage > 0 && (rc = regrow_list(&b->d_rare, &b->cap_rare, b->n_rare)) != ISX_OK) return rc;
        }
        if (!dense && !b->lev_sparse) b->cap_ovf = b->cap_entries - (size_t)b->n_win * b->slab;
        std::lock_guard<std::mutex> lk(p->launch_mu);
        if (dense && p->prm.rarefied_coverage > 0 && b->rare_dense)
            HIP_TRY(hipMemsetD32Async(reinterpret_cast<hipDeviceptr_t>(b->d_clon_r), 0x7FC00000, (size_t)b->n_pos, ps));
        if ((rc = launch_pass(b)) != ISX_OK) return rc;
        {
            PileupArgs pa{};
            pa.cursors = b->d_cursors; pa.host_state = b->d_host_state;
            launch_publish_state(pa, b->epoch, ps);
            b->publish_enqueued = true;
            if (c->unpublished[b->ps] == b) c->unpublished[b->ps] = nullptr;
        }
        redo = true;
    }
    s.d2h_bytes += (int64_t)(std::min((size_t)b->sizes.n_snv, p->snv_prefix) * sizeof(isx_snv));
    if (dense && p->prm.rarefied_coverage > 0) s.d2h_bytes += (int64_t)(std::min((size_t)b->n_rare, p->rare_prefix) * sizeof(isx_rare));
    auto pull = [&](void *hdst, const void *dsrc, size_t bytes) -> int {
        if (!bytes) return ISX_OK;
        HIP_TRY(isx_read_back(hdst, dsrc, bytes, sfin));
        HIP_TRY(isx_read_sync(sfin));
        return ISX_OK;
    };
    struct ReadBatch { ReadBatch() { isx_read_batch(true); } ~ReadBatch() { isx_read_drop(); } } read_batch;
    auto fetch = [&](void *hdst, const void *dsrc, size_t bytes) -> int {
        if (!bytes) return ISX_OK;
        if (!s.out_pinned) return bounce_d2h(p, hdst, dsrc, bytes, sfin);
        HIP_TRY(isx_copy_to_host(hdst, dsrc, bytes, sfin));
        return ISX_OK;
    };
    if (dense) {
        int rc = ISX_OK;
        if (redo) HIP_TRY(isx_wait_stream(ps));
        s.cov8 = false; s.cov4 = false; s.clon_sparse = false; s.sat_complete = (size_t)b->n_sat <= b->cap_sat;
        if (b->sparse_out) {
            s.cov8 = b->cov8_out && !b->nib_pass;
            if (b->nib_pass) {
                const size_t nib_bytes = ((size_t)b->n_pos + 1) / 2, rows_bytes = (size_t)b->n_cov_rows * (size_t)b->W * 2;
                s.cov4 = true; s.cov_window = b->W;
                s.cov_rows_off = (nib_bytes + 63) & ~(size_t)63;
                rc = fetch(s.h_out + s.o_cov16, b->d_cov8, nib_bytes);
                if (rc == ISX_OK) rc = fetch(s.h_out + s.o_cov16 + s.cov_rows_off, b->d_cov16, rows_bytes);
                s.cov_row_win.resize(b->n_cov_rows);
                if (rc == ISX_OK && b->n_cov_rows && isx_read_back(s.cov_row_win.data(), b->d_cov_row_win, (size_t)b->n_cov_rows * sizeof(uint32_t), sfin) != hipSuccess) {
                    isx_set_error("isx_pipe finisher: read-back of the coverage rows' windows"); isx_read_drop(); rc = ISX_ERR_HIP;
                }
                s.d2h_bytes += (int64_t)(nib_bytes + rows_bytes + (size_t)b->n_cov_rows * 4);
            } else if (s.cov8) rc = fetch(s.h_out + s.o_cov16, b->d_cov8, (size_t)b->n_pos);
            else rc = fetch(s.h_out + s.o_cov16, b->d_cov16, (size_t)b->n_pos * 2);
            if (rc != ISX_OK) return rc;
// ... 353 lines not shown
        *ticket = s.ticket;
        p->work.push_back(s.ticket);
    }
    p->cv_work.notify_one();
    return ISX_OK;
}


static int check_capacity(const isx_pipe *p, const char *who, int64_t n_pos, int64_t n_items, int64_t max_items, int32_t n_splits)
{
    if (n_pos > p->pp.max_pos || n_items > max_items || n_splits > p->pp.max_splits) {
        isx_set_error(std::string(who) + ": batch larger than the pipe was created for");
        return ISX_ERR_CAPACITY;
    }
    return ISX_OK;
}

static int slot_acquire(isx_pipe *p, const char *who, Slot **out)
{
    Slot &s = p->slots[(size_t)(p->next_ticket % (int64_t)p->slots.size())];
    {
        std::lock_guard<std::mutex> lk(p->mu);
        if (s.state != 0) { isx_set_error(std::string(who) + ": every slot is in use (collect + release the oldest batch first)"); return ISX_ERR_STATE; }
    }
    HIP_TRY(hipSetDevice(p->ctx->device));
    *out = &s;
    return ISX_OK;
}

static int queue_for_stager(isx_pipe *p, isx_pipe::StageJob &&job, const char *who, int64_t *ticket)
{
    const int rc = check_capacity(p, who, job.n_pos, job.planes ? job.reads.n_seg : job.segs.n_seg, p->pp.max_segs, (int32_t)job.bounds.size() - 1);
    if (rc != ISX_OK) return rc;
    {
        std::lock_guard<std::mutex> lk(p->mu);
        const int64_t t = p->next_promise, n = (int64_t)p->slots.size();
        const Slot &s = p->slots[(size_t)(t % n)];
        if (t - n >= p->next_ticket || s.state != 0) { isx_set_error(std::string(who) + ": every slot is in use (collect + release the oldest batch first)"); return ISX_ERR_STATE; }
        job.ticket = t;
        p->next_promise = t + 1;
        *ticket = t;
        p->stage_q.push_back(std::move(job));
    }
    p->cv_stage.notify_one();
    return ISX_OK;
}

struct RingFeed { hipError_t err = hipSuccess; size_t bytes = 0; };

static int ring_feed_install(isx_pipe *p, Slot &s, RingFeed &r, int64_t &ring_groups, std::function<void(int)> &wave_begin,
                             std::function<void(int, int64_t, int64_t)> &wave_flush)
{
    if (p->ring_half <= 0) return ISX_OK;
    HIP_TRY(hipEventRecord(s.ev_h2d0, H2D(p, s)));
    const size_t half_bytes = (size_t)p->ring_half * (size_t)p->rb, grp_bytes = (size_t)p->G * (size_t)p->rb;
    uint8_t *d_rec = s.d_in + s.off_rec;
    ring_groups = p->ring_half / (int64_t)p->G;
    wave_begin = [&s, &r](int h) {
        if (s.ring_busy[h]) { const hipError_t e = isx_wait_event(s.ev_ring[h]); if (e != hipSuccess && r.err == hipSuccess) r.err = e; s.ring_busy[h] = false; }
    };
    wave_flush = [p, &s, &r, half_bytes, grp_bytes, d_rec](int h, int64_t g0, int64_t g1) {
        const size_t n = (size_t)(g1 - g0) * grp_bytes;
        if (g0 == 0) r.bytes = 0;
        hipError_t e = hipMemcpyAsync(d_rec + (size_t)g0 * grp_bytes, s.h_in + s.off_rec + (size_t)h * half_bytes, n, hipMemcpyHostToDevice, H2D(p, s));
        if (e == hipSuccess) e = hipEventRecord(s.ev_ring[h], H2D(p, s));
        if (e != hipSuccess && r.err == hipSuccess) r.err = e;
        s.ring_busy[h] = true;
        r.bytes += n;
    };
    return ISX_OK;
}

static int slot_choose_windows(isx_pipe *p, Slot &s, uint32_t chunk, bool threads)
{
    isx_batch *b = s.b;
    DirThreads mt{*p->pool, s.dir_pmax, s.dir_smin};
    const ChunkDir dir{s.cmin.data(), s.cmax.data(), s.cany.data(), b->n_rec / chunk, chunk};
    b->W = choose_windows(b, b->n_pos, dir, threads ? &mt : nullptr, s.win, &b->packed);
    b->n_win = (int)s.win.size();
    if (s.win.size() > (size_t)p->pp.max_pos / 64 + 2) { isx_set_error("internal: window directory larger than the arena"); return ISX_ERR_STATE; }
    memcpy(s.h_in + s.off_win, s.win.data(), s.win.size() * sizeof(uint2));
    return ISX_OK;
}

constexpr double COV8_BELOW_DEPTH = 16.0;
constexpr double NIB_BELOW_DEPTH = 6.0;
constexpr double LEV_COV8_BELOW_DEPTH = 64.0;
constexpr double RARE_DENSE_OBS_FACTOR = 4.0;

static int slot_shape_pass(isx_pipe *p, Slot &s)
{
    isx_batch *b = s.b;
    const bool dense = b->M == 1;
    const double n_obs = (double)b->n_obs, n_pos = (double)b->n_pos;
    b->sparse_out = dense && b->d_clon_list != nullptr;
    b->cov8_out = b->sparse_out && n_obs < COV8_BELOW_DEPTH * n_pos;
    b->nib_out = b->cov8_out && b->lean && n_obs < NIB_BELOW_DEPTH * n_pos;
    b->clon_dense = false;
    b->rare_dense = !(b->lean && b->sparse_out) || n_obs * RARE_DENSE_OBS_FACTOR >= (double)p->prm.rarefied_coverage * n_pos;
    if (b->lev_sparse) b->lev_cov_bytes = n_obs < LEV_COV8_BELOW_DEPTH * n_pos ? 1 : 2;
    const int rc = batch_set_geometry(b);
    if (rc != ISX_OK) return rc;
    if (!dense && !b->lev_sparse) {
        const size_t used = (size_t)b->n_win * b->slab;
        if (used > b->slab_region) { isx_set_error("internal: entry slabs larger than the slot's region"); return ISX_ERR_STATE; }
        b->cap_ovf = b->cap_entries - used;
    }
    return ISX_OK;
}

static void slot_bind_inputs(isx_pipe *p, Slot &s, uint8_t *resident_ref)
{
    isx_batch *b = s.b;
    const bool linkage = p->prm.enable_linkage != 0;
    uint8_t *rec = s.d_in + s.off_rec;
    b->d_bounds = reinterpret_cast<int64_t *>(s.d_in + s.off_bounds);
    b->d_win = reinterpret_cast<uint2 *>(s.d_in + s.off_win);
    b->d_ref = resident_ref ? resident_ref : s.d_in + s.off_ref;
    b->d_ref_n = s.ref_has_n ? b->d_ref + ref2_bytes(b->n_pos) : nullptr;
    b->d_gbase = reinterpret_cast<uint32_t *>(s.d_in + s.off_gbase);
    b->d_rec16 = p->rb == 2 ? reinterpret_cast<uint16_t *>(rec) : nullptr;
    b->d_rec32 = p->rb == 4 ? reinterpret_cast<uint32_t *>(rec) : nullptr;
    if (p->segs) {
        b->d_seg = p->drec ? nullptr : reinterpret_cast<uint4 *>(rec);
        b->d_drec = p->drec ? reinterpret_cast<uint4 *>(rec) : nullptr;
        b->d_pair = linkage && !p->drec ? reinterpret_cast<uint32_t *>(s.d_in + s.off_pairs) : nullptr;
        b->d_pair_runs = nullptr; b->d_run_index = nullptr; b->n_runs = 0;
    } else {
        b->d_pair = nullptr;
        b->d_pair_runs = linkage ? s.d_runs : nullptr;
        b->d_run_index = linkage ? reinterpret_cast<uint32_t *>(s.d_in + s.off_ridx) : nullptr;
        b->d_gpos16 = s.d_gpos16; b->gpos16_shift = 5;
    }
}

static void ref_cache_insert(isx_pipe *p, Slot &s, const isx_ref_planes *rp, int64_t n_pos)
{
    const size_t rb_all = ref2_bytes(n_pos) + (s.ref_has_n ? refn_bytes(n_pos) : 0);
    if (p->ref_cache_bytes + rb_all > p->ref_cache_budget.load(std::memory_order_relaxed)) return;
    isx_pipe::RefEntry e;
    bool ok = isx_dev_malloc(reinterpret_cast<void **>(&e.d), rb_all + 64) == hipSuccess && hipEventCreateWithFlags(&e.ready, hipEventDisableTiming) == hipSuccess;
    ok = ok && hipMemcpyAsync(e.d, s.d_in + s.off_ref, rb_all, hipMemcpyDeviceToDevice, H2D(p, s)) == hipSuccess && hipEventRecord(e.ready, H2D(p, s)) == hipSuccess;
    if (ok) {
        e.bytes = rb_all; e.n_pos = n_pos; e.has_n = s.ref_has_n; e.sum = ref_plane_checksum(rp->plane2, n_pos);
        p->ref_cache_bytes += rb_all;
        p->ref_cache.emplace(rp->key, e);
    } else {
        if (e.d) isx_dev_free(e.d);
        if (e.ready) (void)hipEventDestroy(e.ready);
        (void)hipGetLastError();
    }
}

struct RefStage {
    bool early = false;
    uint8_t *resident = nullptr;
    double host_ms = 0.0;
};

static int stage_reference(isx_pipe *p, Slot &s, int64_t n_pos, const uint8_t *ref, const isx_ref_planes *rp, isxenc::SegJob &J, RefStage *out)
{
    const bool ring = p->ring_half > 0;
    const double t_r = now_ms();
    const size_t b2 = ((size_t)n_pos + 3) / 4, bn = ((size_t)n_pos + 7) / 8;
    hipStream_t st = H2D(p, s);

    const auto hit = rp && rp->key ? p->ref_cache.find(rp->key) : p->ref_cache.end();
    if (hit != p->ref_cache.end()) {
        const isx_pipe::RefEntry &e = hit->second;
        if (e.n_pos != n_pos || e.has_n != (rp->nplane != nullptr && e.has_n) || e.sum != ref_plane_checksum(rp->plane2, n_pos)) {
            isx_set_error("isx_pipe_submit_planes: the reference key stands for other planes (positions / non-ACGT plane / content differ)");
            return ISX_ERR_ARG;
        }
        s.ref_has_n = e.has_n;
        J.ref2 = rp->plane2; J.refn = e.has_n ? rp->nplane : nullptr;
        out->resident = e.d;
        HIP_TRY(hipStreamWaitEvent(st, e.ready, 0));
        if (!ring) HIP_TRY(hipEventRecord(s.ev_h2d0, st));
        HIP_TRY(hipEventRecord(s.ev_h2da, st));
        out->early = true;
        out->host_ms = now_ms() - t_r;
        return ISX_OK;
    }

    const bool first_trip = rp && rp->key && p->ref_cache_budget.load(std::memory_order_relaxed) > 0;
    if (rp && !first_trip && isx_host_is_registered(rp->plane2, b2) && (!rp->nplane || isx_host_is_registered(rp->nplane, bn))) {
        const bool any_n = rp->nplane && plane_any(*p->pool, rp->nplane, bn);
        s.ref_has_n = any_n;
        J.ref2 = rp->plane2; J.refn = any_n ? rp->nplane : nullptr;
        out->host_ms = now_ms() - t_r;
        if (!ring) HIP_TRY(hipEventRecord(s.ev_h2d0, st));
        HIP_TRY(hipMemcpyAsync(s.d_in + s.off_ref, rp->plane2, b2, hipMemcpyHostToDevice, st));
        if (any_n) HIP_TRY(hipMemcpyAsync(s.d_in + s.off_ref + ref2_bytes(n_pos), rp->nplane, bn, hipMemcpyHostToDevice, st));
        if (!ring) HIP_TRY(hipEventRecord(s.ev_h2da, st));
        out->early = true;
        return ISX_OK;
    }

    uint8_t *h2 = s.h_in + s.off_ref, *hn = h2 + ref2_bytes(n_pos);
    s.ref_has_n = rp ? copy_ref_planes(*p->pool, rp, n_pos, h2, hn) : isxenc::pack_ref_planes(*p->pool, ref, n_pos, h2, hn);
    J.ref2 = h2; J.refn = s.ref_has_n ? hn : nullptr;
    out->host_ms = now_ms() - t_r;
    static const bool late_dma = getenv("ISX_PIPE_LATE_DMA") != nullptr;
    if (late_dma) return ISX_OK;
    if (!ring) HIP_TRY(hipEventRecord(s.ev_h2d0, st));
    HIP_TRY(hipMemcpyAsync(s.d_in + s.off_ref, h2, ref2_bytes(n_pos) + (s.ref_has_n ? refn_bytes(n_pos) : 0), hipMemcpyHostToDevice, st));
    if (!ring) HIP_TRY(hipEventRecord(s.ev_h2da, st));
    out->early = true;
    if (rp && rp->key) ref_cache_insert(p, s, rp, n_pos);
    return ISX_OK;
}

static int submit_common(isx_pipe *p, int64_t n_pos, const uint8_t *ref, int32_t n_splits, const int64_t *split_bounds,
                         int64_t n_obs, isxenc::EncodeJob &J, int64_t *ticket)
{
    static const char who[] = "isx_pipe_submit";
    int rc;
    if ((rc = check_capacity(p, who, n_pos, n_obs, p->pp.max_obs, n_splits)) != ISX_OK) return rc;
    if ((rc = check_split_bounds(n_pos, n_splits, split_bounds)) != ISX_OK) return rc;
    Slot *slot = nullptr;
    if ((rc = slot_acquire(p, who, &slot)) != ISX_OK) return rc;
    Slot &s = *slot;
    isx_batch *b = s.b;
    const bool linkage = p->prm.enable_linkage != 0;

    const double t0 = now_ms();
    const bool ring = p->ring_half > 0;
    uint8_t *d_rec = s.d_in + s.off_rec;
    RingFeed feed;
    J.n_obs = n_obs; J.n_pos = n_pos; J.record_bytes = p->rb;
    J.rec = s.h_in + s.off_rec; J.gbase = reinterpret_cast<uint32_t *>(s.h_in + s.off_gbase);
    J.pair_out = nullptr;
    J.cmin = s.cmin.data(); J.cmax = s.cmax.data(); J.cany = s.cany.data();
    J.cap_rec = p->cap_rec;
    if ((rc = ring_feed_install(p, s, feed, J.ring_groups, J.wave_begin, J.wave_flush)) != ISX_OK) return rc;
    int erc = 0;
    for (int attempt = 0;; attempt++) {
        if (linkage) {
            J.runs_out = s.h_runs; J.cap_runs = s.cap_runs;
            J.run_index_out = reinterpret_cast<uint32_t *>(s.h_in + s.off_ridx);
        }
        J.slack = p->slack;
        feed.bytes = 0;
        erc = isxenc::encode_obs(*p->pool, J);
        if (erc != isxenc::ENC_OK || !linkage || J.n_runs <= s.cap_runs || attempt == 1) break;
        HIP_TRY(isx_wait_stream(H2D(p, s)));
        host_block_free(s.h_runs, s.runs_pinned); s.h_runs = nullptr;
        isx_dev_free(s.d_runs); s.d_runs = nullptr;
        s.cap_runs = J.n_runs + J.n_runs / 4 + 4096;
        { const int hrc = host_block_alloc(reinterpret_cast<void **>(&s.h_runs), s.cap_runs * sizeof(isxenc::PairRun), s.runs_pinned); if (hrc != ISX_OK) return hrc; }
        HIP_TRY(isx_dev_malloc(reinterpret_cast<void **>(&s.d_runs), s.cap_runs * sizeof(uint2)));
    }
    const double t_enc = now_ms();
    if (feed.err != hipSuccess) { isx_set_error(std::string("isx_pipe_submit: staging ring: ") + hipGetErrorString(feed.err)); return ISX_ERR_HIP; }
    if (erc == isxenc::ENC_CAPACITY) { isx_set_error("isx_pipe_submit: the stream jumps too often for the pipe's record capacity (raise jump_slack)"); return ISX_ERR_CAPACITY; }
    if (erc == isxenc::ENC_MM_RANGE) { isx_set_error("an observation has mm >= 256"); return ISX_ERR_MM_RANGE; }
    if (erc == isxenc::ENC_BAD_POS) { isx_set_error("observation gpos >= n_pos"); return ISX_ERR_ARG; }
    if (linkage) {
        if (J.n_runs > s.cap_runs) { isx_set_error("isx_pipe_submit: internal: pair-id run table did not fit after growing it"); return ISX_ERR_STATE; }
        b->n_runs = (uint32_t)J.n_runs;
    }
    if (J.passes > 1 && J.n_groups_in > 0)
        p->slack = std::max(p->slack, 1.25 * ((double)J.n_groups_real / (double)J.n_groups_in - 1.0) + 0.01);
    s.ref_has_n = isxenc::pack_ref_planes(*p->pool, ref, n_pos, s.h_in + s.off_ref, s.h_in + s.off_ref + ref2_bytes(n_pos));
    memcpy(s.h_in + s.off_bounds, split_bounds, (size_t)(n_splits + 1) * sizeof(int64_t));

    b->n_pos = n_pos; b->n_obs = n_obs; b->n_splits = n_splits; b->n_rec = (uint64_t)J.n_rec;
    b->n_pairs = (uint64_t)J.max_pair + 1;
    if ((rc = slot_choose_windows(p, s, ISX_CHUNK, false)) != ISX_OK) return rc;
    if ((rc = slot_shape_pass(p, s)) != ISX_OK) return rc;
    slot_bind_inputs(p, s, nullptr);
    s.encode_ms = (float)(now_ms() - t0);
    s.encode_passes = J.passes;
    if (pipe_timing)
        fprintf(stderr, "[isx_pipe_submit] records %.2f ms (%d pass), reference + bounds + windows %.2f ms; %lld obs, %lld runs\n",
                t_enc - t0, J.passes, now_ms() - t_enc, (long long)n_obs, (long long)J.n_runs);

    if (!ring) HIP_TRY(hipEventRecord(s.ev_h2d0, H2D(p, s)));
    const size_t ref_bytes = ref2_bytes(n_pos) + (s.ref_has_n ? refn_bytes(n_pos) : 0);
    const size_t head = (size_t)(n_splits + 1) * sizeof(int64_t) + s.win.size() * sizeof(uint2) + ref_bytes;
    memset(s.h_in + s.off_gbase + (size_t)(b->n_rec / p->G) * sizeof(uint32_t), 0, ISX_TAIL_GROUPS * sizeof(uint32_t));
    const size_t gb_bytes = ((size_t)(b->n_rec / p->G) + ISX_TAIL_GROUPS) * sizeof(uint32_t), rec_bytes = (size_t)b->n_rec * p->rb + ISX_TAIL_BYTES;
    HIP_TRY(hipMemcpyAsync(s.d_in + s.off_bounds, s.h_in + s.off_bounds, (size_t)(n_splits + 1) * sizeof(int64_t), hipMemcpyHostToDevice, H2D(p, s)));
    HIP_TRY(hipMemcpyAsync(s.d_in + s.off_win, s.h_in + s.off_win, s.win.size() * sizeof(uint2), hipMemcpyHostToDevice, H2D(p, s)));
    HIP_TRY(hipMemcpyAsync(s.d_in + s.off_ref, s.h_in + s.off_ref, ref_bytes, hipMemcpyHostToDevice, H2D(p, s)));
    HIP_TRY(hipMemcpyAsync(s.d_in + s.off_gbase, s.h_in + s.off_gbase, gb_bytes, hipMemcpyHostToDevice, H2D(p, s)));
    if (ring) {
        if (p->rb == 2) HIP_TRY(hipMemsetD8Async(reinterpret_cast<hipDeviceptr_t>(d_rec + (size_t)b->n_rec * 2), 0xFF, ISX_TAIL_BYTES, H2D(p, s)));
        else HIP_TRY(hipMemsetD32Async(reinterpret_cast<hipDeviceptr_t>(d_rec + (size_t)b->n_rec * 4), (int)ISX_PAD32, ISX_TAIL_BYTES / 4, H2D(p, s)));
        if (feed.bytes != (size_t)b->n_rec * p->rb) { isx_set_error("internal: the staging ring did not carry the whole stream"); return ISX_ERR_STATE; }
    } else {
        if (p->rb == 2) memset(s.h_in + s.off_rec + (size_t)b->n_rec * 2, 0xFF, ISX_TAIL_BYTES);
        else std::fill_n(reinterpret_cast<uint32_t *>(s.h_in + s.off_rec + (size_t)b->n_rec * 4), ISX_TAIL_BYTES / 4, (uint32_t)ISX_PAD32);
        HIP_TRY(hipMemcpyAsync(d_rec, s.h_in + s.off_rec, rec_bytes, hipMemcpyHostToDevice, H2D(p, s)));
    }
    s.h2d_bytes = (int64_t)(head + gb_bytes + rec_bytes);
    if (linkage) {
        const size_t rb = (size_t)b->n_runs * sizeof(isxenc::PairRun), ib = (size_t)(b->n_rec / ISX_CHUNK) * sizeof(uint32_t);
        HIP_TRY(hipMemcpyAsync(s.d_runs, s.h_runs, rb, hipMemcpyHostToDevice, H2D(p, s)));
        HIP_TRY(hipMemcpyAsync(s.d_in + s.off_ridx, s.h_in + s.off_ridx, ib, hipMemcpyHostToDevice, H2D(p, s)));
        s.h2d_bytes += (int64_t)(rb + ib);
    }
    HIP_TRY(hipEventRecord(s.ev_h2d1, H2D(p, s)));
    s.h2d_split = false;

    return enqueue_pass(p, s, n_pos, ticket);
}

static int encode_reads(isx_pipe *p, Slot &s, isxenc::SegJob &J, bool planes_in, RingFeed &feed)
{
    s.encode_passes = 1;
    if (!p->drec) return isxenc::encode_segs(*p->pool, J);
    std::vector<int64_t> exact;
    for (int attempt = 0;; attempt++) {
        J.slack_groups = p->dslack;
        J.task_groups = exact.empty() ? nullptr : exact.data();
        feed.bytes = 0;
        const int erc = planes_in ? isxenc::encode_planes(*p->pool, J) : isxenc::encode_delta(*p->pool, J);
        if (erc != isxenc::SEG_CAPACITY || J.need_slack <= p->dslack || attempt != 0) return erc;
        exact = J.task_need;
        int64_t tot = 0;
        for (int64_t v : exact) tot += v;
        const int64_t n_t = (int64_t)exact.size(), base_tot = J.n_rec / ISX_DREC_GROUP - n_t * p->dslack;
        p->dslack = std::max<int64_t>(p->dslack, 1 + (tot - base_tot + n_t - 1) / std::max<int64_t>(n_t, 1));
        s.encode_passes = 2;
    }
}

static int submit_segs_common(isx_pipe *p, int64_t n_pos, const uint8_t *ref, int32_t n_splits, const int64_t *split_bounds,
                              isxenc::SegJob &J, int64_t *ticket, const isx_ref_planes *rp)
{
    static const char who[] = "isx_pipe_submit_reads";
    const bool planes_in = J.in2.planes != nullptr || (bool)J.produce_planes || (J.n_seg == 0 && rp != nullptr);
    int rc;
    if ((rc = check_capacity(p, who, n_pos, J.n_seg, p->pp.max_segs, n_splits)) != ISX_OK) return rc;
    if ((rc = check_split_bounds(n_pos, n_splits, split_bounds)) != ISX_OK) return rc;
    Slot *slot = nullptr;
    if ((rc = slot_acquire(p, who, &slot)) != ISX_OK) return rc;
    Slot &s = *slot;
    isx_batch *b = s.b;
    const bool linkage = p->prm.enable_linkage != 0;

    const double t0 = now_ms();
    J.n_pos = n_pos; J.n_mm_bins = b->M;
    J.rec = reinterpret_cast<uint32_t *>(s.h_in + s.off_rec);
    J.gbase = reinterpret_cast<uint32_t *>(s.h_in + s.off_gbase);
    J.pair_out = linkage && !p->drec ? reinterpret_cast<uint32_t *>(s.h_in + s.off_pairs) : nullptr;
    J.cmin = s.cmin.data(); J.cmax = s.cmax.data(); J.cany = s.cany.data();
    J.cap_rec = p->cap_rec;
    const bool ring = p->ring_half > 0;
    RingFeed feed;
    if ((rc = ring_feed_install(p, s, feed, J.ring_groups, J.wave_begin, J.wave_flush)) != ISX_OK) return rc;
    RefStage rs;
    if (planes_in) {
        if (!p->drec) { isx_set_error("bit-plane reads need a pipe whose batches travel as reference-delta records (one mm bin, or ISX_LAYOUT_MM_DELTA_RECORDS)"); return ISX_ERR_STATE; }
        if ((rc = stage_reference(p, s, n_pos, ref, rp, J, &rs)) != ISX_OK) return rc;
    }
    if (p->drec) J.ref = ref;
    const int erc = encode_reads(p, s, J, planes_in, feed);
    const double t_enc = now_ms();
    if (feed.err != hipSuccess) { isx_set_error(std::string("isx_pipe_submit_reads: staging ring: ") + hipGetErrorString(feed.err)); return ISX_ERR_HIP; }
    if ((rc = seg_status_error(erc, "isx_pipe_submit_reads: the stream jumps too often for the pipe's record capacity (raise jump_slack)", ISX_ERR_CAPACITY)) != ISX_OK) return rc;
    if (J.n_bases > p->pp.max_obs) { isx_set_error("isx_pipe_submit_reads: more bases than the pipe's max_obs"); return ISX_ERR_CAPACITY; }
    bool early_rec = false;
    if (rs.early && !ring) {
        const size_t gb_bytes0 = (size_t)(J.n_rec / (int64_t)p->G) * sizeof(uint32_t), rec_bytes0 = (size_t)J.n_rec * (size_t)p->rb;
        HIP_TRY(hipEventRecord(s.ev_h2db, H2D(p, s)));
        if (s.off_pairs == s.off_rec && s.off_ridx == s.off_rec && s.off_rec - s.off_gbase < ((size_t)2 << 20)) {
            HIP_TRY(hipMemcpyAsync(s.d_in + s.off_gbase, s.h_in + s.off_gbase, (s.off_rec - s.off_gbase) + rec_bytes0, hipMemcpyHostToDevice, H2D(p, s)));
        } else {
            HIP_TRY(hipMemcpyAsync(s.d_in + s.off_gbase, s.h_in + s.off_gbase, gb_bytes0, hipMemcpyHostToDevice, H2D(p, s)));
            HIP_TRY(hipMemcpyAsync(s.d_in + s.off_rec, s.h_in + s.off_rec, rec_bytes0, hipMemcpyHostToDevice, H2D(p, s)));
        }
        early_rec = true;
    }
    if (!planes_in) s.ref_has_n = isxenc::pack_ref_planes(*p->pool, ref, n_pos, s.h_in + s.off_ref, s.h_in + s.off_ref + ref2_bytes(n_pos));
    const double t_ref = now_ms();
    memcpy(s.h_in + s.off_bounds, split_bounds, (size_t)(n_splits + 1) * sizeof(int64_t));

    b->n_pos = n_pos; b->n_obs = J.n_bases; b->n_splits = n_splits; b->n_rec = (uint64_t)J.n_rec;
    b->n_pairs = (uint64_t)J.max_pair + 1;
    if ((rc = slot_choose_windows(p, s, p->G, true)) != ISX_OK) return rc;
    if ((rc = slot_shape_pass(p, s)) != ISX_OK) return rc;
    slot_bind_inputs(p, s, rs.resident);
    s.encode_ms = (float)(now_ms() - t0);
    if (pipe_timing)
        fprintf(stderr, "[isx_pipe_submit_reads] records %.2f ms, reference %.2f ms, bounds + windows %.2f ms; %lld segments, %lld records%s\n",
                t_enc - t0 - rs.host_ms, t_ref - t_enc + rs.host_ms, now_ms() - t_ref, (long long)J.n_seg, (long long)J.n_rec, planes_in ? " (bit planes)" : "");
    const double t_q0 = now_ms();

    if (!ring && !rs.early) HIP_TRY(hipEventRecord(s.ev_h2d0, H2D(p, s)));
    const size_t ref_bytes = ref2_bytes(n_pos) + (s.ref_has_n ? refn_bytes(n_pos) : 0);
    const size_t head = (size_t)(n_splits + 1) * sizeof(int64_t) + s.win.size() * sizeof(uint2) + ref_bytes;
    const size_t gb_bytes = (size_t)(b->n_rec / p->G) * sizeof(uint32_t), rec_bytes = (size_t)b->n_rec * (size_t)p->rb;
    if (s.off_win - s.off_bounds < ((size_t)1 << 20)) {
        HIP_TRY(hipMemcpyAsync(s.d_in + s.off_bounds, s.h_in + s.off_bounds, (s.off_win - s.off_bounds) + s.win.size() * sizeof(uint2), hipMemcpyHostToDevice, H2D(p, s)));
    } else {
        HIP_TRY(hipMemcpyAsync(s.d_in + s.off_bounds, s.h_in + s.off_bounds, (size_t)(n_splits + 1) * sizeof(int64_t), hipMemcpyHostToDevice, H2D(p, s)));
        HIP_TRY(hipMemcpyAsync(s.d_in + s.off_win, s.h_in + s.off_win, s.win.size() * sizeof(uint2), hipMemcpyHostToDevice, H2D(p, s)));
    }
    if (!rs.early) HIP_TRY(hipMemcpyAsync(s.d_in + s.off_ref, s.h_in + s.off_ref, ref_bytes, hipMemcpyHostToDevice, H2D(p, s)));
    if (!early_rec) HIP_TRY(hipMemcpyAsync(s.d_in + s.off_gbase, s.h_in + s.off_gbase, gb_bytes, hipMemcpyHostToDevice, H2D(p, s)));
    if (ring) { if (feed.bytes != rec_bytes) { isx_set_error("internal: the staging ring did not carry the whole stream"); return ISX_ERR_STATE; } }
    else if (!early_rec) HIP_TRY(hipMemcpyAsync(s.d_in + s.off_rec, s.h_in + s.off_rec, rec_bytes, hipMemcpyHostToDevice, H2D(p, s)));
    s.h2d_bytes = (int64_t)(head + gb_bytes + rec_bytes) - (rs.resident ? (int64_t)ref_bytes : 0);
    if (linkage && !p->drec) {
        HIP_TRY(hipMemcpyAsync(s.d_in + s.off_pairs, s.h_in + s.off_pairs, (size_t)b->n_rec * sizeof(uint32_t), hipMemcpyHostToDevice, H2D(p, s)));
        s.h2d_bytes += (int64_t)b->n_rec * 4;
    }
    HIP_TRY(hipEventRecord(s.ev_h2d1, H2D(p, s)));
    s.h2d_split = early_rec;
    const double t_q1 = now_ms();
    rc = enqueue_pass(p, s, n_pos, ticket);
    if (pipe_timing) fprintf(stderr, "[isx_pipe_submit_reads] copy-in queue %.2f ms, pass + copy-out queue %.2f ms\n", t_q1 - t_q0, now_ms() - t_q1);
    return rc;
}

struct isx_wire {
    isx_pipe *pipe = nullptr;
    uint8_t *h = nullptr;
    size_t bytes = 0;
    size_t o_bounds = 0, o_win = 0, o_ref = 0, o_gbase = 0, o_pairs = 0, o_rec = 0;
    size_t bounds_bytes = 0, win_bytes = 0, ref_bytes = 0, gbase_bytes = 0, pairs_bytes = 0, rec_bytes = 0;
    int64_t n_pos = 0, n_bases = 0, n_rec = 0, n_seg = 0;
    int32_t n_splits = 0;
    uint64_t n_pairs = 0;
    int W = 0, packed = 0;
    bool ref_has_n = false;
    float stage_ms = 0.f;
    int encode_passes = 1;
    uint8_t *d_ref = nullptr;
    int device = 0;
};

static int stage_common(isx_pipe *p, int64_t n_pos, const uint8_t *ref, const isx_ref_planes *rp, int32_t n_splits, const int64_t *split_bounds,
                        const isx_segs *segs, const isx_read_planes *reads, isx_wire **out)
{
    isx_segs as_segs{};
    if (reads) { as_segs.n_seg = reads->n_seg; as_segs.gpos = reads->gpos; as_segs.len = reads->len; as_segs.pair = reads->pair; segs = &as_segs; }
    *out = nullptr;
    if (!p->segs) { isx_set_error("isx_pipe_stage_reads: not a read-level pipe (isx_pipe_params.max_segs == 0)"); return ISX_ERR_STATE; }
    const bool linkage = p->prm.enable_linkage != 0;
    if (linkage && segs->n_seg && !segs->pair) { isx_set_error("linkage needs the pair array"); return ISX_ERR_ARG; }
    int rc;
    if ((rc = check_capacity(p, "isx_pipe_stage_reads", n_pos, segs->n_seg, p->pp.max_segs, n_splits)) != ISX_OK) return rc;
    if ((rc = check_split_bounds(n_pos, n_splits, split_bounds)) != ISX_OK) return rc;
    HIP_TRY(hipSetDevice(p->ctx->device));
    const double t0 = now_ms();
    std::unique_ptr<isx_wire, void (*)(isx_wire *)> w(new isx_wire(), isx_wire_free);
    w->pipe = p; w->n_pos = n_pos; w->n_splits = n_splits; w->n_seg = segs->n_seg;
    const isx_batch *b0 = p->slots[0].b;
    const int M = b0->M;
    const size_t G = p->G, rb = (size_t)p->rb;
    auto up = [](size_t v) { return (v + 255) & ~(size_t)255; };
    isxenc::SegJob J;
    std::vector<uint32_t> cmin, cmax;
    std::vector<uint8_t> cany;
    std::vector<int64_t> exact;
    for (int attempt = 0;; attempt++) {
        int64_t cap = p->drec ? isxenc::delta_groups_needed(*p->pool, segs->gpos, segs->n_seg, p->dslack) * ISX_DREC_GROUP
                              : isxenc::seg_groups_needed(*p->pool, segs->gpos, segs->n_seg) * ISX_SEG_GROUP;
        if (!exact.empty()) { cap = 0; for (int64_t v : exact) cap += std::max<int64_t>(v, 1) * ISX_DREC_GROUP; }
        if (cap > p->cap_rec) { isx_set_error("isx_pipe_stage_reads: the stream needs more records than the pipe's capacity (raise jump_slack)"); return ISX_ERR_CAPACITY; }
        const size_t n_groups = (size_t)cap / G;
        w->bounds_bytes = (size_t)(n_splits + 1) * sizeof(int64_t);
        w->ref_bytes = ref2_bytes(n_pos) + refn_bytes(n_pos);
        const size_t win_cap = ((size_t)n_pos / 64 + 2) * sizeof(uint2);
        size_t o = 0;
        w->o_bounds = o; o = up(o + w->bounds_bytes);
        w->o_win = o; o = up(o + win_cap);
        w->o_ref = o; o = up(o + w->ref_bytes);
        w->o_gbase = o; o = up(o + n_groups * sizeof(uint32_t));
        w->o_pairs = o; if (linkage && !p->drec) o = up(o + (size_t)cap * sizeof(uint32_t));
        w->o_rec = o; o = up(o + (size_t)cap * rb);
        if (w->h) { isx_pin_free(w->h); w->h = nullptr; }
        HIP_TRY(isx_pin_malloc(reinterpret_cast<void **>(&w->h), o));
        w->bytes = o;
        cmin.assign(n_groups + 2, 0xFFFFFFFFu); cmax.assign(n_groups + 2, 0u); cany.assign(n_groups + 2, 0);
        J = isxenc::SegJob();
        J.n_seg = segs->n_seg; J.n_pos = n_pos; J.n_mm_bins = M;
        if (reads) { J.in2 = *reads; if (!linkage) J.in2.pair = nullptr; }
        else { J.in = *segs; if (!linkage) J.in.pair = nullptr; }
        J.rec = reinterpret_cast<uint32_t *>(w->h + w->o_rec);
        J.gbase = reinterpret_cast<uint32_t *>(w->h + w->o_gbase);
        J.pair_out = linkage && !p->drec ? reinterpret_cast<uint32_t *>(w->h + w->o_pairs) : nullptr;
        J.cmin = cmin.data(); J.cmax = cmax.data(); J.cany = cany.data();
        J.cap_rec = cap;
        int erc;
        if (reads) {
            uint8_t *h2 = w->h + w->o_ref, *hn = h2 + ref2_bytes(n_pos);
            w->ref_has_n = rp ? copy_ref_planes(*p->pool, rp, n_pos, h2, hn) : isxenc::pack_ref_planes(*p->pool, ref, n_pos, h2, hn);
            J.ref2 = h2; J.refn = w->ref_has_n ? hn : nullptr;
        }
        if (p->drec) {
            J.ref = ref; J.slack_groups = p->dslack;
            J.task_groups = exact.empty() ? nullptr : exact.data();
            erc = reads ? isxenc::encode_planes(*p->pool, J) : isxenc::encode_delta(*p->pool, J);
            if (erc == isxenc::SEG_CAPACITY && J.need_slack > p->dslack && attempt == 0) { exact = J.task_need; w->encode_passes = 2; continue; }
        } else erc = isxenc::encode_segs(*p->pool, J);
        if ((rc = seg_status_error(erc, "isx_pipe_stage_reads: the stream does not fit the record capacity", ISX_ERR_CAPACITY)) != ISX_OK) return rc;
        break;
    }
    if (J.n_bases > p->pp.max_obs) { isx_set_error("isx_pipe_stage_reads: more bases than the pipe's max_obs"); return ISX_ERR_CAPACITY; }
    w->n_rec = J.n_rec; w->n_bases = J.n_bases; w->n_pairs = (uint64_t)J.max_pair + 1;
    w->gbase_bytes = (size_t)(J.n_rec / (int64_t)G) * sizeof(uint32_t);
    w->rec_bytes = (size_t)J.n_rec * rb;
    w->pairs_bytes = linkage && !p->drec ? (size_t)J.n_rec * sizeof(uint32_t) : 0;
    if (!reads) w->ref_has_n = isxenc::pack_ref_planes(*p->pool, ref, n_pos, w->h + w->o_ref, w->h + w->o_ref + ref2_bytes(n_pos));
    if (!w->ref_has_n) w->ref_bytes = ref2_bytes(n_pos);
    memcpy(w->h + w->o_bounds, split_bounds, w->bounds_bytes);
    {
        std::vector<uint2> win;
        std::vector<uint32_t> dir_pmax, dir_smin;
        DirThreads mt{*p->pool, dir_pmax, dir_smin};
        w->W = choose_windows(b0, n_pos, ChunkDir{cmin.data(), cmax.data(), cany.data(), (uint64_t)J.n_rec / G, (uint32_t)G}, &mt, win, &w->packed);
        w->win_bytes = win.size() * sizeof(uint2);
        if (w->win_bytes > ((size_t)n_pos / 64 + 2) * sizeof(uint2) || win.size() > (size_t)p->pp.max_pos / 64 + 2) { isx_set_error("internal: window directory larger than its region"); return ISX_ERR_STATE; }
        memcpy(w->h + w->o_win, win.data(), w->win_bytes);
    }
    w->stage_ms = (float)(now_ms() - t0);
    *out = w.release();
    return ISX_OK;
}

int isx_pipe_stage_reads(isx_pipe *p, int64_t n_pos, const uint8_t *ref, int32_t n_splits, const int64_t *split_bounds,
                         const isx_segs *segs, isx_wire **out)
{
    if (!p || !ref || !split_bounds || !out || n_pos <= 0 || n_splits <= 0 || !segs || segs->n_seg < 0 ||
        (segs->n_seg && (!segs->gpos || !segs->len || !segs->bases))) {
        isx_set_error("isx_pipe_stage_reads: bad argument");
        return ISX_ERR_ARG;
    }
    return stage_common(p, n_pos, ref, nullptr, n_splits, split_bounds, segs, nullptr, out);
}

int isx_pipe_stage_planes(isx_pipe *p, int64_t n_pos, const isx_ref_planes *ref, int32_t n_splits, const int64_t *split_bounds,
                          const isx_read_planes *reads, isx_wire **out)
{
    if (!p || !ref || !ref->plane2 || !split_bounds || !out || n_pos <= 0 || n_splits <= 0 || !reads || reads->n_seg < 0 ||
        (reads->n_seg && (!reads->gpos || !reads->len || !reads->planes))) {
        isx_set_error("isx_pipe_stage_planes: bad argument");
        return ISX_ERR_ARG;
    }
    if (!p->drec) { isx_set_error("isx_pipe_stage_planes: bit-plane reads need a read-level pipe with one mm bin or ISX_LAYOUT_MM_DELTA_RECORDS"); return ISX_ERR_STATE; }
    return stage_common(p, n_pos, nullptr, ref, n_splits, split_bounds, nullptr, reads, out);
}

void isx_wire_free(isx_wire *w)
{
    if (!w) return;
    if (w->h) isx_pin_free(w->h);
    if (w->d_ref) { (void)hipSetDevice(w->device); isx_dev_free(w->d_ref); }
    delete w;
}

int isx_wire_keep_reference(isx_pipe *p, isx_wire *w)
{
    if (!p || !w || w->pipe != p) { isx_set_error("isx_wire_keep_reference: bad argument"); return ISX_ERR_ARG; }
// ... 366 lines not shown
```

instrain_amd/csrc/seg_encode.cpp:

```cpp
#include "seg_encode.h"

#include <immintrin.h>

#include <algorithm>
#include <atomic>
#include <cstdlib>
#include <cstring>
#include <string>
#include <vector>

void isx_set_error(const std::string &msg);

namespace isxenc {

namespace {

constexpr int64_t TASK = 4096;
constexpr uint32_t SPAN = 65535u;

inline int64_t count_groups(const uint32_t *gpos, int64_t a, int64_t e, int64_t group = ISX_SEG_GROUP)
{
    int64_t n = 0;
    for (int64_t i = a; i < e;) {
        uint32_t lo = gpos[i], hi = gpos[i];
// ... 370 lines not shown
            } else {
                h = 2 * G.n;
                uint32_t *o = G.rec[G.n];
                if (plain) {
                    o[0] = (len << 16) | ISX_DREC_DUAL; o[1] = pid; o[2] = exc[0]; o[3] = exc[1];
                    o[4] = ISX_DREC_DUAL; o[5] = 0; o[6] = o[7] = ISX_DREC_NO_EXC;
                    G.open = G.n;
                } else {
                    o[0] = len << 16;
                    o[1] = (uint32_t)msk[0]; o[2] = (uint32_t)(msk[0] >> 32); o[3] = exc[0];
                    o[4] = (uint32_t)msk[1]; o[5] = (uint32_t)(msk[1] >> 32); o[6] = (uint32_t)msk[2]; o[7] = pid;
                    G.open = -1;
                }
                G.used[h + 1] = false;
                G.n++;
            }
            G.used[h] = true; G.start[h] = start; G.last[h] = start + (len & 0xFFu) - 1;
            np++;
        };
        Cols C;
        for (int64_t s = a; s < e; s++) {
            const uint32_t L = ln[s], m = mm ? mm[s] : 0u, p = gp[s];
            if (L == 0 || L > ISX_SEG_BASES) { err.store(SEG_BAD_LEN); return; }
            if ((int64_t)p + (int64_t)L > J.n_pos || p != gpos_all[s]) { err.store(SEG_BAD_POS); return; }
            if ((int)m >= J.n_mm_bins) { err.store(SEG_MM_RANGE); return; }
            const uint32_t pid = pr ? pr[s] : 0u;
            maxp = std::max(maxp, pid);
            nb += L;
            if (vbmi) cols_vbmi(bs + (size_t)s * ISX_SEG_WORDS, J.ref + p, L, C);
            else cols_scalar(bs + (size_t)s * ISX_SEG_WORDS, J.ref + p, L, C);
            if (J.n_mm_bins > 1) {
                C.exc[0] |= C.nbase[0]; C.exc[1] |= C.nbase[1]; C.exc[2] |= C.nbase[2];
            }
            const int n_exc = __builtin_popcountll(C.exc[0]) + __builtin_popcountll(C.exc[1]) + __builtin_popcountll(C.exc[2]);
            const bool plain = (C.skip[0] | C.skip[1] | C.skip[2]) == 0;
            if (n_exc == 0) {
                const uint32_t none[2] = {ISX_DREC_NO_EXC, ISX_DREC_NO_EXC};
                add_piece(p, L, pid, C.skip, none, plain, m);
                continue;
            }
            const uint32_t max_exc = plain ? ISX_DREC_EXC : ISX_DREC_EXC_FULL;
            uint64_t ex[3] = {C.exc[0], C.exc[1], C.exc[2]};
            uint32_t b = 0;
            while (b < L) {
                uint32_t f[ISX_DREC_EXC], nf = 0, end = L;
                for (int k = 0; k < 3; k++) {
                    while (ex[k]) {
                        const uint32_t col = (uint32_t)(64 * k + __builtin_ctzll(ex[k]));
                        if (nf == max_exc) { end = col; goto cut; }
                        ex[k] &= ex[k] - 1;
                        f[nf++] = ((col - b) & 0xFFu) | ((uint32_t)(C.code[col] & 3u) << 8);
                    }
                }
            cut:
                uint32_t w[2] = {ISX_DREC_NO_EXC, ISX_DREC_NO_EXC};
                for (uint32_t i = 0; i < nf; i++) {
                    const int wi = i / 3, sh = 10 * (int)(i % 3);
                    w[wi] = (w[wi] & ~(0x3FFu << sh)) | (f[i] << sh);
                }
                uint64_t msk[3];
                window160(C.skip, b, end - b, msk);
                add_piece(p + b, end - b, pid, msk, w, plain, m);
                b = end;
            }
        }
        close_group();
        need_of[(size_t)t] = used;
        for (; g < g_end; g++) {
            put_empty_group(rec_at(g));
            J.gbase[g] = 0; J.cmin[g] = 0xFFFFFFFFu; J.cmax[g] = 0; J.cany[g] = 0;
        }
        bases_of[(size_t)t] = nb; maxp_of[(size_t)t] = maxp; pieces_of[(size_t)t] = np;
    };
    if (!RG) pool.run(n_tasks, [&](int t) { run_task(t, 0, 0); });
    else {
        int half = 0;
        for (int t0 = 0; t0 < n_tasks && err.load() == SEG_OK;) {
            int t1 = t0 + 1;
            while (t1 < n_tasks && g_at[(size_t)t1 + 1] - g_at[(size_t)t0] <= RG) t1++;
            if (g_at[(size_t)t1] - g_at[(size_t)t0] > RG) return SEG_CAPACITY;
            J.wave_begin(half);
            const int64_t wg0 = g_at[(size_t)t0];
            pool.run(t1 - t0, [&](int k) { run_task(t0 + k, wg0, half); });
            if (err.load() == SEG_OK) J.wave_flush(half, wg0, g_at[(size_t)t1]);
            t0 = t1; half ^= 1;
        }
    }
    if (err.load() != SEG_OK) return err.load();
    J.n_bases = 0; J.max_pair = 0; J.n_pieces = 0;
    int64_t worst = 0;
    bool fits = true;
    J.task_need.assign(need_of.begin(), need_of.begin() + n_tasks);
    for (int t = 0; t < n_tasks; t++) {
        J.n_bases += bases_of[(size_t)t]; J.max_pair = std::max(J.max_pair, maxp_of[(size_t)t]); J.n_pieces += pieces_of[(size_t)t];
        const int64_t region = g_at[(size_t)t + 1] - g_at[(size_t)t];
        if (need_of[(size_t)t] > region) fits = false;
        worst = std::max(worst, need_of[(size_t)t] - (region - (J.task_groups ? 0 : slack)));
    }
    J.need_slack = fits ? slack : std::max<int64_t>(worst, slack + 1);
    if (!fits) return SEG_CAPACITY;
    return SEG_OK;
}


namespace {

struct LenMasks {
    alignas(32) uint64_t m[ISX_SEG_BASES + 1][4];
    LenMasks()
    {
        for (uint32_t L = 0; L <= ISX_SEG_BASES; L++)
            for (uint32_t k = 0; k < 4; k++) {
                const uint32_t from = 64 * k;
                m[L][k] = L <= from ? 0 : (L - from >= 64 ? ~(uint64_t)0 : (((uint64_t)1 << (L - from)) - 1));
            }
    }
};

inline bool cpu_has_bmi2()
{
    static const bool v = __builtin_cpu_supports("bmi2") && !getenv("ISX_NO_BMI2");
    return v;
}

inline uint64_t even_bits_portable(uint64_t x)
{
    x &= 0x5555555555555555ull;
    x = (x | (x >> 1)) & 0x3333333333333333ull;
    x = (x | (x >> 2)) & 0x0F0F0F0F0F0F0F0Full;
    x = (x | (x >> 4)) & 0x00FF00FF00FF00FFull;
    x = (x | (x >> 8)) & 0x0000FFFF0000FFFFull;
    x = (x | (x >> 16)) & 0x00000000FFFFFFFFull;
    return x;
}

inline void bits160(const uint8_t *q, uint32_t sh, uint64_t d[3])
{
    uint64_t w[4];
    memcpy(w, q, 32);
    for (int i = 0; i < 3; i++) d[i] = (w[i] >> sh) | ((w[i + 1] << 1) << (63 - sh));
}

struct PlaneTask {
    int64_t a, e;
    const uint32_t *gp, *pr, *gpos_all;
    const uint8_t *ln;
    const uint8_t *mm = nullptr;
    const uint64_t *pl;
    uint32_t *rec0;
    int64_t g0, ga, ge;
    bool fast_store;
    int64_t used = 0, np = 0, nb = 0;
    uint32_t maxp = 0;
};

inline void put_empty_drec(uint32_t *o)
{
    o[0] = o[1] = o[2] = o[4] = o[5] = o[6] = o[7] = 0;
    o[3] = ISX_DREC_NO_EXC;
}

#ifndef ISX_PLANES_PREFETCH
#define ISX_PLANES_PREFETCH 16
#endif
constexpr int64_t PLANES_PREFETCH = ISX_PLANES_PREFETCH;
struct PlaneGroup {
    alignas(64) uint32_t rec[ISX_DREC_GROUP][ISX_DREC_WORDS];
    int n = 0, open = -1;
    uint32_t lo = 0, hi = 0, last = 0;
    int64_t g = 0, used = 0;
};
__attribute__((noinline)) void rebase_drecs(PlaneGroup &G, uint32_t new_lo)
{
    const uint32_t up = G.lo - new_lo;
    for (int r = 0; r < G.n; r++) {
        uint32_t *o = G.rec[r];
        if ((o[0] >> 16) & 0xFFu) o[0] += up;
        if ((o[0] & ISX_DREC_DUAL) && ((o[4] >> 16) & 0xFFu)) o[4] += up;
    }
    G.lo = new_lo;
}

struct PlaneScratch {
    std::vector<uint32_t> gpos, pair;
    std::vector<uint8_t> len, mm;
    std::vector<uint64_t> planes;
    uint64_t *pl = nullptr;
};

#define ISX_PLANES_FN planes_task_portable
#define ISX_CLOSE_FN close_group_portable
#define ISX_DIFFERS_FN differs160_portable
#define ISX_PLANES_VARIANT 0
#include "seg_planes.inc"
#undef ISX_PLANES_FN
#undef ISX_CLOSE_FN
#undef ISX_DIFFERS_FN
#undef ISX_PLANES_VARIANT
#pragma GCC push_options
#pragma GCC target("bmi,bmi2,popcnt,lzcnt")
#define ISX_PLANES_FN planes_task_bmi2
#define ISX_CLOSE_FN close_group_bmi2
#define ISX_DIFFERS_FN differs160_bmi2
#define ISX_PLANES_VARIANT 1
#include "seg_planes.inc"
#undef ISX_PLANES_FN
#undef ISX_CLOSE_FN
#undef ISX_DIFFERS_FN
#undef ISX_PLANES_VARIANT
#pragma GCC pop_options
#pragma GCC push_options
#pragma GCC target("bmi,bmi2,popcnt,lzcnt,avx512f,avx512bw,avx512vl,avx512vbmi2,gfni")
#define ISX_PLANES_FN planes_task_avx512
#define ISX_CLOSE_FN close_group_avx512
#define ISX_DIFFERS_FN differs160_avx512
#define ISX_PLANES_VARIANT 2
#include "seg_planes.inc"
#undef ISX_PLANES_FN
#undef ISX_CLOSE_FN
#undef ISX_DIFFERS_FN
#undef ISX_PLANES_VARIANT
#pragma GCC pop_options

inline int planes_variant()
{
    static const int v = [] {
        if (const char *e = getenv("ISX_PLANES_VARIANT")) return std::max(0, std::min(2, atoi(e)));
        if (!cpu_has_bmi2()) return 0;
        return cpu_has_avx512() && __builtin_cpu_supports("avx512vbmi2") && __builtin_cpu_supports("gfni") ? 2 : 1;
    }();
    if (v == 2 && !(cpu_has_avx512() && __builtin_cpu_supports("avx512vbmi2") && __builtin_cpu_supports("gfni") && __builtin_cpu_supports("bmi2"))) return __builtin_cpu_supports("bmi2") ? 1 : 0;
    if (v == 1 && !__builtin_cpu_supports("bmi2")) return 0;
    return v;
}

}

int encode_planes(HostPool &pool, SegJob &J)
{
    const int64_t n = J.n_seg;
    const bool producer = (bool)J.produce_planes;
    const uint32_t *gpos_all = producer ? J.gpos_all : J.in2.gpos;
    const int n_tasks = (int)((n + TASK - 1) / TASK);
    const int64_t slack = std::max<int64_t>(J.slack_groups, 1);
    std::vector<int64_t> g_at((size_t)n_tasks + 1, 0);
    if (J.task_groups) for (int t = 0; t < n_tasks; t++) g_at[(size_t)t + 1] = std::max<int64_t>(J.task_groups[t], 1);
    else pool.run(n_tasks, [&](int t) {
        const int64_t a = (int64_t)t * TASK, e = std::min<int64_t>(n, a + TASK);
        g_at[(size_t)t + 1] = count_groups(gpos_all, a, e, 2 * ISX_DREC_GROUP) + slack;
    });
    for (int t = 0; t < n_tasks; t++) g_at[(size_t)t + 1] += g_at[(size_t)t];
    const int64_t n_groups = std::max<int64_t>(g_at[(size_t)n_tasks], 1);
    J.n_rec = n_groups * ISX_DREC_GROUP;
    J.need_slack = slack;
    if (J.n_rec > J.cap_rec) return SEG_CAPACITY;
    std::atomic<int> err{SEG_OK};
    std::vector<int64_t> bases_of((size_t)std::max(n_tasks, 1), 0), need_of((size_t)std::max(n_tasks, 1), 0), pieces_of((size_t)std::max(n_tasks, 1), 0);
    std::vector<uint32_t> maxp_of((size_t)std::max(n_tasks, 1), 0);
    const bool pairs = producer ? J.want_pairs : J.in2.pair != nullptr;
    const int64_t RG = J.ring_groups;
    constexpr size_t group_words = (size_t)ISX_DREC_GROUP * ISX_DREC_WORDS;
    const bool fast_store = cpu_has_avx512() && (reinterpret_cast<uintptr_t>(J.rec) & 63) == 0;
    const int variant = planes_variant();
    if (n == 0) {
        if (RG) J.wave_begin(0);
        for (int r = 0; r < ISX_DREC_GROUP; r++) put_empty_drec(J.rec + (size_t)r * ISX_DREC_WORDS);
        J.gbase[0] = 0; J.cmin[0] = 0xFFFFFFFFu; J.cmax[0] = 0; J.cany[0] = 0;
        J.n_bases = 0; J.max_pair = 0; J.n_pieces = 0;
        if (RG) J.wave_flush(0, 0, 1);
        return SEG_OK;
    }
    auto run_task = [&](int t, int64_t wave_g0, int half) {
        if (err.load(std::memory_order_relaxed) != SEG_OK) return;
        const int64_t a = (int64_t)t * TASK, e = std::min<int64_t>(n, a + TASK);
        const uint32_t *gp, *pr;
        const uint8_t *ln, *mmv = nullptr;
        const uint64_t *pl;
        if (producer) {
            thread_local PlaneScratch S;
            if (S.gpos.size() < (size_t)TASK) {
                S.gpos.resize((size_t)TASK); S.pair.resize((size_t)TASK); S.len.resize((size_t)TASK); S.mm.resize((size_t)TASK);
                S.planes.resize((size_t)TASK * ISX_PLANE_WORDS + 8);
                S.pl = reinterpret_cast<uint64_t *>((reinterpret_cast<uintptr_t>(S.planes.data()) + 63) & ~(uintptr_t)63);
            }
            J.produce_planes(a, e - a, S.gpos.data(), S.len.data(), J.n_mm_bins > 1 ? S.mm.data() : nullptr, pairs ? S.pair.data() : nullptr, S.pl);
            gp = S.gpos.data() - a; ln = S.len.data() - a; pr = pairs ? S.pair.data() - a : nullptr;
            if (J.n_mm_bins > 1) mmv = S.mm.data() - a;
            pl = S.pl - (size_t)a * ISX_PLANE_WORDS;
        } else {
            gp = J.in2.gpos; ln = J.in2.len; pr = pairs ? J.in2.pair : nullptr; pl = J.in2.planes;
            if (J.n_mm_bins > 1) mmv = J.in2.mm;
        }
        PlaneTask K;
        K.a = a; K.e = e; K.gp = gp; K.ln = ln; K.mm = mmv; K.pr = pr; K.pl = pl; K.gpos_all = gpos_all;
        K.rec0 = RG ? J.rec + (size_t)((int64_t)half * RG) * group_words : J.rec;
        K.g0 = RG ? wave_g0 : 0; K.ga = g_at[(size_t)t]; K.ge = g_at[(size_t)t + 1]; K.fast_store = fast_store;
        if (variant == 2) planes_task_avx512(J, err, K);
        else if (variant == 1) planes_task_bmi2(J, err, K);
        else planes_task_portable(J, err, K);
        if (err.load(std::memory_order_relaxed) != SEG_OK) return;
        need_of[(size_t)t] = K.used;
        bases_of[(size_t)t] = K.nb; maxp_of[(size_t)t] = K.maxp; pieces_of[(size_t)t] = K.np;
    };
    if (!RG) pool.run(n_tasks, [&](int t) { run_task(t, 0, 0); });
    else {
        int half = 0;
        for (int t0 = 0; t0 < n_tasks && err.load() == SEG_OK;) {
            int t1 = t0 + 1;
            while (t1 < n_tasks && g_at[(size_t)t1 + 1] - g_at[(size_t)t0] <= RG) t1++;
            if (g_at[(size_t)t1] - g_at[(size_t)t0] > RG) return SEG_CAPACITY;
            J.wave_begin(half);
            const int64_t wg0 = g_at[(size_t)t0];
            pool.run(t1 - t0, [&](int k) { run_task(t0 + k, wg0, half); });
            if (err.load() == SEG_OK) J.wave_flush(half, wg0, g_at[(size_t)t1]);
            t0 = t1; half ^= 1;
        }
    }
    if (err.load() != SEG_OK) return err.load();
    J.n_bases = 0; J.max_pair = 0; J.n_pieces = 0;
    int64_t worst = 0;
    bool fits = true;
    J.task_need.assign(need_of.begin(), need_of.begin() + n_tasks);
    for (int t = 0; t < n_tasks; t++) {
        J.n_bases += bases_of[(size_t)t]; J.max_pair = std::max(J.max_pair, maxp_of[(size_t)t]); J.n_pieces += pieces_of[(size_t)t];
        const int64_t region = g_at[(size_t)t + 1] - g_at[(size_t)t];
        if (need_of[(size_t)t] > region) fits = false;
        worst = std::max(worst, need_of[(size_t)t] - (region - (J.task_groups ? 0 : slack)));
    }
    J.need_slack = fits ? slack : std::max<int64_t>(worst, slack + 1);
    if (!fits) return SEG_CAPACITY;
    return SEG_OK;
}


namespace {
__attribute__((target("bmi2")))
inline void pack_ref_piece_bmi2(const uint8_t *r, int64_t n, uint8_t *o2, uint8_t *on, bool &seen)
{
    int64_t i = 0;
    uint64_t any = 0;
    for (; i + 8 <= n; i += 8) {
        uint64_t x;
        memcpy(&x, r + i, 8);
        const uint64_t bad = x & 0xFCFCFCFCFCFCFCFCull;
        if (__builtin_expect(bad == 0, 1)) {
            const uint16_t v = (uint16_t)_pext_u64(x, 0x0303030303030303ull);
            memcpy(o2 + (i >> 2), &v, 2);
            on[i >> 3] = 0;
            continue;
        }
        uint64_t t = bad | (bad >> 4);
        t |= t >> 2; t |= t >> 1;
        const uint64_t nb = t & 0x0101010101010101ull;
        const uint64_t keep = ~(nb * 0xFFull);
        const uint16_t v = (uint16_t)_pext_u64(x & keep, 0x0303030303030303ull);
        memcpy(o2 + (i >> 2), &v, 2);
        on[i >> 3] = (uint8_t)_pext_u64(nb, 0x0101010101010101ull);
        any |= nb;
    }
    for (; i < n; i += 8) {
        uint32_t lo = 0, hi = 0, nbits = 0;
        const int64_t m = std::min<int64_t>(8, n - i);
        for (int64_t k = 0; k < m; k++) {
            const uint32_t c = r[i + k];
            const uint32_t b = c > 3u;
            nbits |= b << k;
            const uint32_t v = b ? 0u : c;
            if (k < 4) lo |= v << (2 * k); else hi |= v << (2 * (k - 4));
        }
        o2[i >> 2] = (uint8_t)lo;
        if (m > 4) o2[(i >> 2) + 1] = (uint8_t)hi;
        on[i >> 3] = (uint8_t)nbits;
        any |= nbits;
    }
    seen = any != 0;
}

inline void pack_ref_piece_scalar(const uint8_t *r, int64_t n, uint8_t *o2, uint8_t *on, bool &seen)
{
    seen = false;
    for (int64_t i = 0; i < n; i += 8) {
        uint32_t lo = 0, hi = 0, nb = 0;
        const int64_t m = std::min<int64_t>(8, n - i);
        for (int64_t k = 0; k < m; k++) {
            const uint32_t c = r[i + k];
            const uint32_t bad = c > 3u;
            nb |= bad << k;
            const uint32_t v = bad ? 0u : c;
            if (k < 4) lo |= v << (2 * k); else hi |= v << (2 * (k - 4));
        }
        o2[i >> 2] = (uint8_t)lo;
        if (m > 4) o2[(i >> 2) + 1] = (uint8_t)hi;
        on[i >> 3] = (uint8_t)nb;
        seen |= nb != 0;
    }
}
}

bool pack_ref_planes(HostPool &pool, const uint8_t *ref, int64_t n_pos, uint8_t *plane2, uint8_t *nplane)
{
    const int64_t piece = (int64_t)256 << 10;
    const int n_tasks = (int)((n_pos + piece - 1) / piece);
    std::atomic<int> any{0};
    const bool bmi2 = cpu_has_bmi2();
    auto cp = [&](int t) {
        const int64_t a = (int64_t)t * piece, e = std::min<int64_t>(n_pos, a + piece);
        bool seen = false;
        if (bmi2) pack_ref_piece_bmi2(ref + a, e - a, plane2 + (a >> 2), nplane + (a >> 3), seen);
        else pack_ref_piece_scalar(ref + a, e - a, plane2 + (a >> 2), nplane + (a >> 3), seen);
        if (seen) any.store(1, std::memory_order_relaxed);
    };
    if (n_tasks > 1) pool.run(n_tasks, cp); else if (n_tasks == 1) cp(0);
    return any.load() != 0;
}

void planes_from_words(const uint32_t *w, uint32_t L, uint64_t *P)
{
    uint64_t b[5] = {0, 0, 0, 0, 0}, sk[3] = {0, 0, 0};
    for (uint32_t j = 0; j < L; j++) {
        const uint32_t c = (w[j / 10] >> (3 * (j % 10))) & 7u;
        if (c >= 4) {
            sk[j >> 6] |= (uint64_t)1 << (j & 63);
            if (c == 5) { b[j >> 5] |= (uint64_t)1 << (2 * (j & 31)); sk[2] |= (uint64_t)1 << 63; }
        } else b[j >> 5] |= (uint64_t)c << (2 * (j & 31));
    }
    for (int i = 0; i < 5; i++) P[i] = b[i];
    for (int i = 0; i < 3; i++) P[5 + i] = sk[i];
}

}

namespace {

inline uint32_t ascii_code(char c)
{
    switch (c) {
    case 'A': return 0; case 'C': return 1; case 'T': return 2; case 'G': return 3;
    default: return 5;
    }
}

enum { OP_M = 0, OP_I = 1, OP_D = 2, OP_N = 3, OP_S = 4, OP_H = 5, OP_P = 6, OP_EQ = 7, OP_X = 8 };

template <class F>
inline bool for_runs(const uint32_t *cig, int64_t n_cig, int64_t ref_start, int64_t clip_lo, int64_t clip_hi, F &&f)
{
    int64_t ref = ref_start, q = 0;
    for (int64_t k = 0; k < n_cig; k++) {
        const uint32_t op = cig[k] & 15u;
// ... 59 lines not shown

int isx_encode_delta(const isx_segs *segs, const uint8_t *ref, int64_t n_pos, int32_t n_mm_bins, int32_t host_threads, int32_t slack_groups,
                     int64_t cap_rec, int64_t ring_records, uint32_t *rec, uint32_t *gbase, uint32_t *pair_out, int64_t *n_rec, int64_t *need_slack)
{
    if (!segs || !ref || !rec || !gbase || !n_rec || segs->n_seg < 0 || cap_rec < ISX_DREC_GROUP || (cap_rec % ISX_DREC_GROUP) || n_pos <= 0 ||
        (segs->n_seg && (!segs->gpos || !segs->len || !segs->bases)) || ring_records < 0 ||
        (ring_records % (2 * ISX_DREC_GROUP)) || slack_groups < 0) {
        isx_set_error("isx_encode_delta: bad argument");
        return ISX_ERR_ARG;
    }
    std::vector<uint32_t> ring;
    isxenc::HostPool pool(std::max(1, host_threads), -1, false);
    std::vector<uint32_t> cmin((size_t)(cap_rec / ISX_DREC_GROUP)), cmax(cmin.size());
    std::vector<uint8_t> cany(cmin.size());
    isxenc::SegJob J;
    J.in = *segs; J.n_seg = segs->n_seg; J.n_pos = n_pos; J.n_mm_bins = std::max(1, n_mm_bins);
    J.ref = ref; J.slack_groups = std::max(1, slack_groups);
    (void)pair_out;
    J.rec = rec; J.gbase = gbase; J.pair_out = nullptr;
    J.cmin = cmin.data(); J.cmax = cmax.data(); J.cany = cany.data(); J.cap_rec = cap_rec;
    if (ring_records) {
        const int64_t half = ring_records / 2;
        ring.assign((size_t)ring_records * ISX_DREC_WORDS, 0xABABABABu);
        J.rec = ring.data();
        J.ring_groups = half / ISX_DREC_GROUP;
        J.wave_begin = [](int) {};
        J.wave_flush = [&](int h, int64_t g0, int64_t g1) {
            const size_t gw = (size_t)ISX_DREC_GROUP * ISX_DREC_WORDS;
            memcpy(rec + (size_t)g0 * gw, ring.data() + (size_t)h * half * ISX_DREC_WORDS, (size_t)(g1 - g0) * gw * 4);
            std::fill_n(ring.begin() + (ptrdiff_t)((size_t)h * half * ISX_DREC_WORDS), (size_t)half * ISX_DREC_WORDS, 0xABABABABu);
        };
    }
    const int rc = isxenc::encode_delta(pool, J);
    if (need_slack) *need_slack = J.need_slack;
    *n_rec = J.n_rec;
    if (rc == isxenc::SEG_CAPACITY) {
        isx_set_error(J.need_slack > J.slack_groups ? "isx_encode_delta: a task needs more spare groups than slack_groups (see *need_slack)"
                                                    : "isx_encode_delta: the stream does not fit cap_rec records");
        return ISX_ERR_CAPACITY;
    }
    if (rc == isxenc::SEG_MM_RANGE) { isx_set_error("a segment has mm >= n_mm_bins"); return ISX_ERR_MM_RANGE; }
    if (rc == isxenc::SEG_BAD_POS) { isx_set_error("a segment reaches beyond n_pos"); return ISX_ERR_ARG; }
    if (rc == isxenc::SEG_BAD_LEN) { isx_set_error("a segment's length is not in [1, 150]"); return ISX_ERR_ARG; }
    return ISX_OK;
}

int64_t isx_delta_records_needed(const uint32_t *gpos, int64_t n_seg, int32_t host_threads, int32_t slack_groups)
{
    if (n_seg < 0 || (n_seg && !gpos) || slack_groups < 0) return -1;
    isxenc::HostPool pool(std::max(1, host_threads), -1, false);
    return isxenc::delta_groups_needed(pool, gpos, n_seg, std::max(1, slack_groups)) * ISX_DREC_GROUP;
}

int64_t isx_seg_records_needed(const uint32_t *gpos, int64_t n_seg, int32_t host_threads)
{
    if (n_seg < 0 || (n_seg && !gpos)) return -1;
    isxenc::HostPool pool(std::max(1, host_threads), -1, false);
    return isxenc::seg_groups_needed(pool, gpos, n_seg) * ISX_SEG_GROUP;
}

int isx_count_read_segs(int64_t n_reads, const uint32_t *cigar, const int64_t *cigar_off, const int64_t *ref_start,
                        const int64_t *clip_lo, const int64_t *clip_hi, int64_t *n_seg)
{
    if (n_reads < 0 || !n_seg || (n_reads && (!cigar || !cigar_off || !ref_start || !clip_lo || !clip_hi))) {
        isx_set_error("isx_count_read_segs: bad argument");
        return ISX_ERR_ARG;
    }
    int64_t n = 0;
    for (int64_t r = 0; r < n_reads; r++) {
        const bool ok = for_runs(cigar + cigar_off[r], cigar_off[r + 1] - cigar_off[r], ref_start[r], clip_lo[r], clip_hi[r],
                                 [&](int64_t, int64_t, int64_t cols) { n += (cols + ISX_SEG_BASES - 1) / ISX_SEG_BASES; });
        if (!ok) { isx_set_error("isx_count_read_segs: unknown CIGAR operator"); return ISX_ERR_ARG; }
    }
    *n_seg = n;
    return ISX_OK;
}

int isx_pack_reads(int64_t n_reads, const int64_t *ref_start, const int64_t *clip_lo, const int64_t *clip_hi,
                   const uint32_t *cigar, const int64_t *cigar_off, const char *seq, const uint8_t *qual, const int64_t *seq_off,
                   const uint8_t *mm, const uint32_t *pair, int32_t min_base_quality, int64_t cap_seg, uint32_t *seg_gpos,
                   uint8_t *seg_len, uint8_t *seg_mm, uint32_t *seg_pair, uint32_t *seg_bases, int64_t *n_seg)
{
    if (n_reads < 0 || !n_seg || cap_seg < 0 || (n_reads && (!ref_start || !clip_lo || !clip_hi || !cigar || !cigar_off || !seq || !qual || !seq_off)) ||
        (cap_seg && (!seg_gpos || !seg_len || !seg_bases)) || (pair && cap_seg && !seg_pair)) {
        isx_set_error("isx_pack_reads: bad argument");
        return ISX_ERR_ARG;
    }
    int64_t n = 0;
    bool full = false, bad = false;
    for (int64_t r = 0; r < n_reads && !full && !bad; r++) {
        const char *sq = seq + seq_off[r];
        const uint8_t *ql = qual + seq_off[r];
        const int64_t q_len = seq_off[r + 1] - seq_off[r];
        const bool ok = for_runs(cigar + cigar_off[r], cigar_off[r + 1] - cigar_off[r], ref_start[r], clip_lo[r], clip_hi[r],
                                 [&](int64_t pos, int64_t q0, int64_t cols) {
            if (q0 + cols > q_len || pos < 0 || pos + cols > (int64_t)0xFFFFFFFFll) { bad = true; return; }
            for (int64_t c0 = 0; c0 < cols && !full; c0 += ISX_SEG_BASES) {
                const int L = (int)std::min<int64_t>(ISX_SEG_BASES, cols - c0);
                if (n >= cap_seg) { full = true; return; }
                uint32_t *w = seg_bases + (size_t)n * ISX_SEG_WORDS;
                for (int k = 0; k < ISX_SEG_WORDS; k++) w[k] = ISX_SEG_SKIP_WORD;
                for (int j = 0; j < L; j++) {
                    const int64_t qi = q0 + c0 + j;
                    const uint32_t code = (int)ql[qi] >= min_base_quality ? ascii_code(sq[qi]) : 4u;
                    w[j / 10] = (w[j / 10] & ~(7u << (3 * (j % 10)))) | (code << (3 * (j % 10)));
                }
                seg_gpos[n] = (uint32_t)(pos + c0); seg_len[n] = (uint8_t)L;
                if (seg_mm) seg_mm[n] = mm ? mm[r] : (uint8_t)0;
                if (seg_pair) seg_pair[n] = pair ? pair[r] : 0u;
                n++;
            }
        });
        if (!ok) { isx_set_error("isx_pack_reads: unknown CIGAR operator"); return ISX_ERR_ARG; }
    }
    if (bad) { isx_set_error("isx_pack_reads: a CIGAR reaches beyond its read's bases or the flat space"); return ISX_ERR_ARG; }
    if (full) { isx_set_error("isx_pack_reads: more segments than cap_seg (isx_count_read_segs gives the number)"); return ISX_ERR_CAPACITY; }
    *n_seg = n;
    return ISX_OK;
}

int isx_pack_ref_planes(const uint8_t *ref, int64_t n_pos, int32_t host_threads, uint8_t *plane2, uint8_t *nplane, int32_t *has_n)
{
    if (!ref || n_pos <= 0 || !plane2 || !nplane) { isx_set_error("isx_pack_ref_planes: bad argument"); return ISX_ERR_ARG; }
    isxenc::HostPool pool(std::max(1, host_threads), -1, false);
    const bool any = isxenc::pack_ref_planes(pool, ref, n_pos, plane2, nplane);
    if (has_n) *has_n = any ? 1 : 0;
    return ISX_OK;
}

int isx_planes_from_segs(const isx_segs *segs, int32_t host_threads, uint64_t *planes)
{
    if (!segs || segs->n_seg < 0 || (segs->n_seg && (!segs->len || !segs->bases || !planes))) { isx_set_error("isx_planes_from_segs: bad argument"); return ISX_ERR_ARG; }
    const int64_t n = segs->n_seg, piece = 8192;
    std::atomic<bool> bad{false};
    isxenc::HostPool pool(std::max(1, host_threads), -1, false);
    pool.run((int)((n + piece - 1) / piece), [&](int t) {
        const int64_t a = (int64_t)t * piece, e = std::min<int64_t>(n, a + piece);
        for (int64_t i = a; i < e; i++) {
            const uint32_t L = segs->len[i];
            if (L == 0 || L > ISX_SEG_BASES) { bad.store(true); return; }
            isxenc::planes_from_words(segs->bases + (size_t)i * ISX_SEG_WORDS, L, planes + (size_t)i * ISX_PLANE_WORDS);
        }
    });
    if (bad.load()) { isx_set_error("a segment's length is not in [1, 150]"); return ISX_ERR_ARG; }
    return ISX_OK;
}

int isx_encode_planes(const isx_read_planes *reads, const isx_ref_planes *ref, int64_t n_pos, int32_t host_threads, int32_t slack_groups,
                      int64_t cap_rec, int64_t ring_records, uint32_t *rec, uint32_t *gbase, int64_t *n_rec, int64_t *need_slack)
{
    return isx_encode_planes_mm(reads, ref, n_pos, 1, host_threads, slack_groups, cap_rec, ring_records, rec, gbase, n_rec, need_slack);
}

int isx_encode_planes_mm(const isx_read_planes *reads, const isx_ref_planes *ref, int64_t n_pos, int32_t n_mm_bins, int32_t host_threads, int32_t slack_groups,
                         int64_t cap_rec, int64_t ring_records, uint32_t *rec, uint32_t *gbase, int64_t *n_rec, int64_t *need_slack)
{
    if (n_mm_bins < 1 || n_mm_bins > 128) { isx_set_error("isx_encode_planes: n_mm_bins must be in [1, 128]"); return ISX_ERR_ARG; }
    if (!reads || !ref || !ref->plane2 || !rec || !gbase || !n_rec || reads->n_seg < 0 || cap_rec < ISX_DREC_GROUP || (cap_rec % ISX_DREC_GROUP) || n_pos <= 0 ||
        (reads->n_seg && (!reads->gpos || !reads->len || !reads->planes)) || ring_records < 0 ||
        (ring_records % (2 * ISX_DREC_GROUP)) || slack_groups < 0) {
        isx_set_error("isx_encode_planes: bad argument");
        return ISX_ERR_ARG;
    }
    std::vector<uint32_t> ring;
    isxenc::HostPool pool(std::max(1, host_threads), -1, false);
    std::vector<uint32_t> cmin((size_t)(cap_rec / ISX_DREC_GROUP)), cmax(cmin.size());
    std::vector<uint8_t> cany(cmin.size());
    isxenc::SegJob J;
    J.in2 = *reads; J.n_seg = reads->n_seg; J.n_pos = n_pos; J.n_mm_bins = n_mm_bins;
    J.ref2 = ref->plane2; J.refn = ref->nplane; J.slack_groups = std::max(1, slack_groups);
    J.rec = rec; J.gbase = gbase; J.pair_out = nullptr;
    J.cmin = cmin.data(); J.cmax = cmax.data(); J.cany = cany.data(); J.cap_rec = cap_rec;
    if (ring_records) {
        const int64_t half = ring_records / 2;
        ring.assign((size_t)ring_records * ISX_DREC_WORDS + 16, 0xABABABABu);
        uint32_t *r0 = reinterpret_cast<uint32_t *>((reinterpret_cast<uintptr_t>(ring.data()) + 63) & ~(uintptr_t)63);
        J.rec = r0;
        J.ring_groups = half / ISX_DREC_GROUP;
        J.wave_begin = [](int) {};
        J.wave_flush = [&, r0](int h, int64_t g0, int64_t g1) {
            const size_t gw = (size_t)ISX_DREC_GROUP * ISX_DREC_WORDS;
            memcpy(rec + (size_t)g0 * gw, r0 + (size_t)h * half * ISX_DREC_WORDS, (size_t)(g1 - g0) * gw * 4);
            std::fill_n(r0 + (size_t)h * half * ISX_DREC_WORDS, (size_t)half * ISX_DREC_WORDS, 0xABABABABu);
        };
    }
    const int rc = isxenc::encode_planes(pool, J);
    if (need_slack) *need_slack = J.need_slack;
    *n_rec = J.n_rec;
    if (rc == isxenc::SEG_CAPACITY) {
        isx_set_error(J.need_slack > J.slack_groups ? "isx_encode_planes: a task needs more spare groups than slack_groups (see *need_slack)"
                                                    : "isx_encode_planes: the stream does not fit cap_rec records");
        return ISX_ERR_CAPACITY;
    }
    if (rc == isxenc::SEG_BAD_POS) { isx_set_error("a segment reaches beyond n_pos"); return ISX_ERR_ARG; }
    if (rc == isxenc::SEG_BAD_LEN) { isx_set_error("a segment's length is not in [1, 150]"); return ISX_ERR_ARG; }
    if (rc == isxenc::SEG_MM_RANGE) { isx_set_error("a segment has mm >= n_mm_bins"); return ISX_ERR_MM_RANGE; }
    return ISX_OK;
}

int isx_pack_read_planes(int64_t n_reads, const int64_t *ref_start, const int64_t *clip_lo, const int64_t *clip_hi,
                         const uint32_t *cigar, const int64_t *cigar_off, const char *seq, const uint8_t *qual, const int64_t *seq_off,
                         const uint32_t *pair, int32_t min_base_quality, int64_t cap_seg, uint32_t *seg_gpos,
                         uint8_t *seg_len, uint32_t *seg_pair, uint64_t *seg_planes, int64_t *n_seg)
{
    if (n_reads < 0 || !n_seg || cap_seg < 0 || (n_reads && (!ref_start || !clip_lo || !clip_hi || !cigar || !cigar_off || !seq || !qual || !seq_off)) ||
        (cap_seg && (!seg_gpos || !seg_len || !seg_planes)) || (pair && cap_seg && !seg_pair)) {
        isx_set_error("isx_pack_read_planes: bad argument");
        return ISX_ERR_ARG;
    }
    int64_t n = 0;
    bool full = false, bad = false;
    for (int64_t r = 0; r < n_reads && !full && !bad; r++) {
        const char *sq = seq + seq_off[r];
        const uint8_t *ql = qual + seq_off[r];
        const int64_t q_len = seq_off[r + 1] - seq_off[r];
        const bool ok = for_runs(cigar + cigar_off[r], cigar_off[r + 1] - cigar_off[r], ref_start[r], clip_lo[r], clip_hi[r],
                                 [&](int64_t pos, int64_t q0, int64_t cols) {
            if (q0 + cols > q_len || pos < 0 || pos + cols > (int64_t)0xFFFFFFFFll) { bad = true; return; }
            for (int64_t c0 = 0; c0 < cols && !full; c0 += ISX_SEG_BASES) {
                const int L = (int)std::min<int64_t>(ISX_SEG_BASES, cols - c0);
                if (n >= cap_seg) { full = true; return; }
                uint64_t *P = seg_planes + (size_t)n * ISX_PLANE_WORDS;
                for (int k = 0; k < ISX_PLANE_WORDS; k++) P[k] = 0;
                for (int j = 0; j < L; j++) {
                    const int64_t qi = q0 + c0 + j;
                    const uint32_t code = (int)ql[qi] >= min_base_quality ? ascii_code(sq[qi]) : 4u;
                    if (code >= 4) {
                        P[5 + (j >> 6)] |= (uint64_t)1 << (j & 63);
                        if (code == 5) { P[j >> 5] |= (uint64_t)1 << (2 * (j & 31)); P[7] |= (uint64_t)1 << 63; }
                    } else P[j >> 5] |= (uint64_t)code << (2 * (j & 31));
                }
                seg_gpos[n] = (uint32_t)(pos + c0); seg_len[n] = (uint8_t)L;
                if (seg_pair) seg_pair[n] = pair ? pair[r] : 0u;
                n++;
            }
        });
        if (!ok) { isx_set_error("isx_pack_read_planes: unknown CIGAR operator"); return ISX_ERR_ARG; }
    }
    if (bad) { isx_set_error("isx_pack_read_planes: a CIGAR reaches beyond its read's bases or the flat space"); return ISX_ERR_ARG; }
    if (full) { isx_set_error("isx_pack_read_planes: more segments than cap_seg (isx_count_read_segs gives the number)"); return ISX_ERR_CAPACITY; }
    *n_seg = n;
    return ISX_OK;
}

}
```

instrain_amd/csrc/seg_encode.h:

```cpp
#pragma once
#include <stdint.h>

#include <functional>
#include <vector>

#include "../../include/instrain_amd.h"
#include "obs_encode.h"

#define ISX_SEG_GROUP 16
#define ISX_SEG_REC_WORDS 16
#define ISX_DREC_GROUP 32

namespace isxenc {

struct SegJob {
    isx_segs in{};
    std::function<void(int64_t first, int64_t count, uint32_t *gpos, uint8_t *len, uint8_t *mm, uint32_t *pair, uint32_t *bases)> produce;
    const uint32_t *gpos_all = nullptr;
    isx_read_planes in2{};
    std::function<void(int64_t first, int64_t count, uint32_t *gpos, uint8_t *len, uint8_t *mm, uint32_t *pair, uint64_t *planes)> produce_planes;
    const uint8_t *ref2 = nullptr, *refn = nullptr;
    int64_t n_seg = 0, n_pos = 0;
    int n_mm_bins = 1;
    bool want_pairs = false;
    uint32_t *rec = nullptr;
    uint32_t *gbase = nullptr;
    uint32_t *pair_out = nullptr;
    uint32_t *cmin = nullptr, *cmax = nullptr;
    uint8_t *cany = nullptr;
    int64_t cap_rec = 0;
    int64_t ring_groups = 0;
    std::function<void(int half)> wave_begin;
    std::function<void(int half, int64_t g0, int64_t g1)> wave_flush;
    const uint8_t *ref = nullptr;
    int64_t slack_groups = 1;
    int64_t need_slack = 0;
    std::vector<int64_t> task_need;
    const int64_t *task_groups = nullptr;
    int64_t n_pieces = 0;
    int64_t n_rec = 0;
    int64_t n_bases = 0;
    uint32_t max_pair = 0;
};

enum { SEG_OK = 0, SEG_CAPACITY = 1, SEG_MM_RANGE = 2, SEG_BAD_POS = 3, SEG_BAD_LEN = 4 };

int encode_segs(HostPool &pool, SegJob &job);
int encode_delta(HostPool &pool, SegJob &job);
int encode_planes(HostPool &pool, SegJob &job);
int64_t delta_groups_needed(HostPool &pool, const uint32_t *gpos, int64_t n, int64_t slack_groups);
int64_t seg_groups_needed(HostPool &pool, const uint32_t *gpos, int64_t n);
bool pack_ref_planes(HostPool &pool, const uint8_t *ref, int64_t n_pos, uint8_t *plane2, uint8_t *nplane);
void planes_from_words(const uint32_t *words, uint32_t len, uint64_t *planes);

}
```

instrain_amd/csrc/seg_planes.inc:

```

#if ISX_PLANES_VARIANT == 2
static inline __attribute__((always_inline)) __m256i ISX_DIFFERS_FN(const uint8_t *q, uint32_t sh, __m512i P)
{
    const __m512i lo = _mm512_maskz_loadu_epi64((__mmask8)0x1F, q), hi = _mm512_maskz_loadu_epi64((__mmask8)0x1F, q + 8);
    const __m512i r = _mm512_shrdv_epi64(lo, hi, _mm512_set1_epi64((long long)sh));
    const __m512i x = _mm512_xor_si512(r, P);
    const __m512i m = _mm512_or_si512(x, _mm512_srli_epi64(x, 1));
    const __m512i nib = _mm512_gf2p8affine_epi64_epi8(m, _mm512_set1_epi64((long long)0x0104104000000000ull), 0);
    const __m512i t = _mm512_or_si512(nib, _mm512_srli_epi16(nib, 4));
    return _mm512_cvtepi16_epi8(t);
}
#else
static inline __attribute__((always_inline)) void ISX_DIFFERS_FN(const uint8_t *q, uint32_t sh, const uint64_t *P, uint64_t d[3])
{
    uint64_t w[6];
    memcpy(w, q, 48);
    uint64_t e[5];
    for (int i = 0; i < 5; i++) {
        const uint64_t r = (w[i] >> sh) | ((w[i + 1] << 1) << (63 - sh));
        const uint64_t x = r ^ P[i];
        const uint64_t m = x | (x >> 1);
#if ISX_PLANES_VARIANT == 1
        e[i] = _pext_u64(m, 0x5555555555555555ull);
#else
        e[i] = even_bits_portable(m);
#endif
    }
    d[0] = e[0] | (e[1] << 32);
    d[1] = e[2] | (e[3] << 32);
    d[2] = e[4];
}
#endif

static __attribute__((noinline)) void ISX_CLOSE_FN(SegJob &J, const PlaneTask &K, PlaneGroup &G)
{
    if (!G.n) return;
    if (G.g < K.ge) {
        for (int r = G.n; r < ISX_DREC_GROUP; r++) put_empty_drec(G.rec[r]);
        uint32_t *o = K.rec0 + (size_t)(G.g - K.g0) * (size_t)ISX_DREC_GROUP * ISX_DREC_WORDS;
        if (!K.fast_store) memcpy(o, G.rec, sizeof G.rec);
        else {
#if ISX_PLANES_VARIANT == 2
            for (int r = 0; r < ISX_DREC_GROUP; r += 2) _mm512_stream_si512(reinterpret_cast<__m512i *>(o + (size_t)r * ISX_DREC_WORDS), _mm512_load_si512(G.rec[r]));
#else
            const __m128i *src = reinterpret_cast<const __m128i *>(G.rec);
            __m128i *dst = reinterpret_cast<__m128i *>(o);
            for (int i = 0; i < ISX_DREC_GROUP * ISX_DREC_WORDS / 4; i++) _mm_stream_si128(dst + i, _mm_load_si128(src + i));
#endif
        }
        J.gbase[G.g] = G.lo; J.cmin[G.g] = G.lo; J.cmax[G.g] = G.last; J.cany[G.g] = 1;
        G.g++;
    }
    G.used++;
    G.n = 0; G.open = -1;
}

#if ISX_PLANES_VARIANT == 0
#define ISX_TZ64(x) ((x) ? (uint32_t)__builtin_ctzll(x) : 64u)
#else
#define ISX_TZ64(x) ((uint32_t)_tzcnt_u64(x))
#endif
static void ISX_PLANES_FN(SegJob &J, std::atomic<int> &err, PlaneTask &K)
{
    static const LenMasks LM;
    PlaneGroup G;
    G.g = K.ga;
    const uint8_t *const ref2 = J.ref2, *const refn = J.refn;
    const int64_t n_pos = J.n_pos;
    const int64_t safe_pos = n_pos - 200;
    const uint32_t *const gp = K.gp, *const pr = K.pr, *const ga = K.gpos_all;
    const uint8_t *const ln = K.ln;
    int64_t nb = 0, np = 0;
    uint32_t maxp = 0;
    auto place = [&](uint32_t start, uint32_t len, bool plain, bool &fill) __attribute__((always_inline)) -> uint32_t * {
        fill = plain && G.open >= 0;
        if (G.n) {
            const uint32_t nlo = std::min(G.lo, start), nhi = std::max(G.hi, start);
            if (__builtin_expect(nhi - nlo > SPAN || (!fill && G.n == ISX_DREC_GROUP), 0)) { ISX_CLOSE_FN(J, K, G); fill = false; }
        }
        if (!G.n) { G.lo = G.hi = start; G.last = start + len - 1; }
        else {
            if (__builtin_expect(start < G.lo, 0)) rebase_drecs(G, start);
            G.hi = std::max(G.hi, start); G.last = std::max(G.last, start + len - 1);
        }
        np++;
        if (fill) { uint32_t *o = G.rec[G.open] + 4; G.open = -1; return o; }
        uint32_t *o = G.rec[G.n];
        G.open = plain ? G.n : -1;
        G.n++;
        return o;
    };
    uint32_t hdr_hi = 0;
    auto add_full = [&](uint32_t start, uint32_t len, uint32_t pid, uint64_t s0, uint64_t s1, uint64_t s2, uint32_t exc) __attribute__((always_inline)) {
        bool fill;
        uint32_t *o = place(start, len, false, fill);
        const uint64_t v0 = (uint64_t)((start - G.lo) | (len << 16) | hdr_hi) | (s0 << 32), v1 = (s0 >> 32) | ((uint64_t)exc << 32);
        const uint64_t v3 = (s2 & 0xFFFFFFFFull) | ((uint64_t)pid << 32);
        memcpy(o, &v0, 8); memcpy(o + 2, &v1, 8); memcpy(o + 4, &s1, 8); memcpy(o + 6, &v3, 8);
    };
    auto add_plain = [&](uint32_t start, uint32_t len, uint32_t pid, uint32_t exc0, uint32_t exc1) __attribute__((always_inline)) {
        bool fill;
        uint32_t *o = place(start, len, true, fill);
        const uint64_t v0 = (uint64_t)((start - G.lo) | (len << 16) | hdr_hi | ISX_DREC_DUAL) | ((uint64_t)pid << 32), v1 = (uint64_t)exc0 | ((uint64_t)exc1 << 32);
        memcpy(o, &v0, 8); memcpy(o + 2, &v1, 8);
        if (!fill) {
            const uint64_t v2 = (uint64_t)ISX_DREC_DUAL, v3 = (uint64_t)ISX_DREC_NO_EXC | ((uint64_t)ISX_DREC_NO_EXC << 32);
            memcpy(o + 4, &v2, 8); memcpy(o + 6, &v3, 8);
        }
    };
#if ISX_PLANES_VARIANT == 2
    const __m256i rec_idx = _mm256_setr_epi32(8, 0, 1, 8, 2, 3, 4, 8);
#endif
    const bool mm_on = J.n_mm_bins > 1;
    const int64_t pf_end = K.e - PLANES_PREFETCH;
    for (int64_t s = K.a; s < K.e; s++) {
        const uint32_t L = ln[s], p = gp[s];
        const uint64_t *P = K.pl + (size_t)s * ISX_PLANE_WORDS;
        if (s < pf_end) {
            _mm_prefetch(reinterpret_cast<const char *>(P + (size_t)PLANES_PREFETCH * ISX_PLANE_WORDS), _MM_HINT_T0);
            _mm_prefetch(reinterpret_cast<const char *>(ref2 + (gp[s + PLANES_PREFETCH] >> 2) + 40), _MM_HINT_T0);
        }
        if (__builtin_expect(L == 0 || L > ISX_SEG_BASES, 0)) { err.store(SEG_BAD_LEN); return; }
        if (__builtin_expect((int64_t)p + (int64_t)L > n_pos || p != ga[s], 0)) { err.store(SEG_BAD_POS); return; }
        const uint32_t pid = pr ? pr[s] : 0u;
        maxp = pid > maxp ? pid : maxp;
        nb += L;
        const uint64_t *lm = LM.m[L];
        uint64_t s0, s1, s2, ex[3];
        bool n_marked = false;
        if (mm_on) {
            const uint32_t mv = K.mm ? K.mm[s] : 0u;
            if (__builtin_expect((int)mv >= J.n_mm_bins || mv > 127u, 0)) { err.store(SEG_MM_RANGE); return; }
            hdr_hi = mv << 24;
            n_marked = (P[7] >> 63) != 0;
        }
#if ISX_PLANES_VARIANT == 2
        __m256i skv = _mm256_setzero_si256();
        const bool in_regs = (int64_t)p < safe_pos && !refn && !n_marked;
        if (__builtin_expect(in_regs, 1)) {
            const __m512i Pv = _mm512_loadu_si512(P);
            const __m256i lmv = _mm256_loadu_si256(reinterpret_cast<const __m256i *>(lm));
            skv = _mm256_and_si256(_mm256_maskz_loadu_epi64((__mmask8)0x7, P + 5), lmv);
            const __m256i dv = ISX_DIFFERS_FN(ref2 + (p >> 2), (p & 3u) * 2u, Pv);
            const __m256i exv = _mm256_and_si256(dv, _mm256_xor_si256(skv, lmv));
            alignas(32) uint64_t t[8];
            _mm256_store_si256(reinterpret_cast<__m256i *>(t), skv);
            _mm256_store_si256(reinterpret_cast<__m256i *>(t + 4), exv);
            s0 = t[0]; s1 = t[1]; s2 = t[2];
            ex[0] = t[4]; ex[1] = t[5]; ex[2] = t[6];
        } else
#endif
        {
            s0 = P[5] & lm[0]; s1 = P[6] & lm[1]; s2 = P[7] & lm[2];
            uint64_t d[3];
#if ISX_PLANES_VARIANT == 2
            alignas(32) uint64_t dq[4];
#define ISX_DIFFERS_AT(q_, sh_) do { _mm256_store_si256(reinterpret_cast<__m256i *>(dq), ISX_DIFFERS_FN((q_), (sh_), _mm512_loadu_si512(P))); d[0] = dq[0]; d[1] = dq[1]; d[2] = dq[2]; } while (0)
#else
#define ISX_DIFFERS_AT(q_, sh_) ISX_DIFFERS_FN((q_), (sh_), P, d)
#endif
            if (__builtin_expect((int64_t)p < safe_pos, 1)) {
                ISX_DIFFERS_AT(ref2 + (p >> 2), (p & 3u) * 2u);
                if (refn) {
                    uint64_t nn[3];
                    if (__builtin_expect((int64_t)p + 264 <= n_pos, 1)) bits160(refn + (p >> 3), p & 7u, nn);
                    else {
                        uint8_t bn[32] = {0};
                        const int64_t haven = (n_pos + 7) / 8 - (int64_t)(p >> 3);
                        memcpy(bn, refn + (p >> 3), (size_t)std::min<int64_t>(32, haven));
                        bits160(bn, p & 7u, nn);
                    }
                    d[0] |= nn[0]; d[1] |= nn[1]; d[2] |= nn[2];
                }
            } else {
                alignas(64) uint8_t buf[64] = {0};
                const int64_t have2 = (n_pos + 3) / 4 - (int64_t)(p >> 2);
                memcpy(buf, ref2 + (p >> 2), (size_t)std::min<int64_t>(48, have2));
                ISX_DIFFERS_AT(buf, (p & 3u) * 2u);
                if (refn) {
                    uint8_t bn[32] = {0};
                    const int64_t haven = (n_pos + 7) / 8 - (int64_t)(p >> 3);
                    memcpy(bn, refn + (p >> 3), (size_t)std::min<int64_t>(32, haven));
                    uint64_t nn[3];
                    bits160(bn, p & 7u, nn);
                    d[0] |= nn[0]; d[1] |= nn[1]; d[2] |= nn[2];
                }
            }
#undef ISX_DIFFERS_AT
            ex[0] = d[0] & (lm[0] ^ s0); ex[1] = d[1] & (lm[1] ^ s1); ex[2] = d[2] & (lm[2] ^ s2);
            if (__builtin_expect(n_marked, 0)) {
                ex[0] |= (even_bits_portable(P[0]) | (even_bits_portable(P[1]) << 32)) & s0;
                ex[1] |= (even_bits_portable(P[2]) | (even_bits_portable(P[3]) << 32)) & s1;
                ex[2] |= even_bits_portable(P[4]) & s2;
            }
        }
        const bool plain = (s0 | s1 | s2) == 0;
        const uint32_t n_exc = (uint32_t)(__builtin_popcountll(ex[0]) + __builtin_popcountll(ex[1]) + __builtin_popcountll(ex[2]));
        if (__builtin_expect(n_exc <= 1, 1)) {
            const uint32_t t0 = ISX_TZ64(ex[0]), t1 = ISX_TZ64(ex[1]), t2 = ISX_TZ64(ex[2] | ((uint64_t)1 << 63));
            const uint32_t m0 = 0u - (uint32_t)(ex[0] == 0), m01 = m0 & (0u - (uint32_t)(ex[1] == 0));
            const uint32_t col = t0 + (t1 & m0) + (t2 & m01);
            const uint32_t code = (uint32_t)(P[col >> 5] >> (2 * (col & 31u))) & 3u;
            const uint32_t w0 = 0x3FFFFC00u | ((col | (code << 8) | (0u - (uint32_t)(n_exc == 0))) & 0x3FFu);
            if (__builtin_expect(plain, 0)) { add_plain(p, L, pid, w0, ISX_DREC_NO_EXC); continue; }
#if ISX_PLANES_VARIANT == 2
            if (__builtin_expect(in_regs, 1)) {
                bool fill;
                uint32_t *o = place(p, L, false, fill);
                __m256i v = _mm256_permutex2var_epi32(skv, rec_idx, _mm256_set1_epi32((int)w0));
                v = _mm256_mask_set1_epi32(v, (__mmask8)0x01, (int)((p - G.lo) | (L << 16) | hdr_hi));
                v = _mm256_mask_set1_epi32(v, (__mmask8)0x80, (int)pid);
                _mm256_store_si256(reinterpret_cast<__m256i *>(o), v);
                continue;
            }
#endif
            add_full(p, L, pid, s0, s1, s2, w0);
            continue;
        }
        const uint32_t max_exc = plain ? ISX_DREC_EXC : ISX_DREC_EXC_FULL;
        if (__builtin_expect(n_exc <= max_exc, 1)) {
            uint64_t fields = 0;
            for (uint32_t i = 0; i < n_exc; i++) {
                const int k = ex[0] ? 0 : (ex[1] ? 1 : 2);
                const uint32_t col = (uint32_t)(64 * k + __builtin_ctzll(ex[k]));
                ex[k] &= ex[k] - 1;
                const uint64_t code = (P[col >> 5] >> (2 * (col & 31u))) & 3u;
                fields |= ((uint64_t)col | (code << 8)) << (10 * i);
            }
            const uint64_t all = (fields | (0x0FFFFFFFFFFFFFFFull << (10 * n_exc))) & 0x0FFFFFFFFFFFFFFFull;
            const uint32_t w0 = (uint32_t)all & ISX_DREC_NO_EXC, w1 = (uint32_t)(all >> 30) & ISX_DREC_NO_EXC;
            if (plain) add_plain(p, L, pid, w0, w1);
            else add_full(p, L, pid, s0, s1, s2, w0);
            continue;
        }
        const uint64_t sk[3] = {s0, s1, s2};
        uint32_t b = 0;
        while (b < L) {
            uint32_t w[2] = {ISX_DREC_NO_EXC, ISX_DREC_NO_EXC};
            uint32_t nf = 0, end = L;
            for (int k = 0; k < 3; k++) {
                while (ex[k]) {
                    const uint32_t col = (uint32_t)(64 * k + __builtin_ctzll(ex[k]));
                    if (nf == max_exc) { end = col; goto cut; }
                    ex[k] &= ex[k] - 1;
                    const uint32_t code = (uint32_t)(P[col >> 5] >> (2 * (col & 31u))) & 3u;
                    const uint32_t f = ((col - b) & 0xFFu) | (code << 8);
                    const int wi = (int)(nf / 3), shf = 10 * (int)(nf % 3);
                    w[wi] = (w[wi] & ~(0x3FFu << shf)) | (f << shf);
                    nf++;
                }
            }
        cut:
            if (plain) add_plain(p + b, end - b, pid, w[0], w[1]);
            else if (b == 0 && end == L) add_full(p, L, pid, s0, s1, s2, w[0]);
            else {
                uint64_t msk[3];
                window160(sk, b, end - b, msk);
                add_full(p + b, end - b, pid, msk[0], msk[1], msk[2], w[0]);
            }
            b = end;
        }
    }
    ISX_CLOSE_FN(J, K, G);
    for (; G.g < K.ge; G.g++) {
        uint32_t *o = K.rec0 + (size_t)(G.g - K.g0) * (size_t)ISX_DREC_GROUP * ISX_DREC_WORDS;
        for (int r = 0; r < ISX_DREC_GROUP; r++) put_empty_drec(o + (size_t)r * ISX_DREC_WORDS);
        J.gbase[G.g] = 0; J.cmin[G.g] = 0xFFFFFFFFu; J.cmax[G.g] = 0; J.cany[G.g] = 0;
    }
    if (K.fast_store) _mm_sfence();
    K.used = G.used; K.np = np; K.nb = nb; K.maxp = maxp;
}
#undef ISX_TZ64
```

Baseline: 169.8.

## Send only referenced reference-plane words to device and add AVX-512 group fast path

Measured after the change: 98.30. -42.1%, worse.

```diff
diff --git a/include/instrain_amd.h b/include/instrain_amd.h
--- a/include/instrain_amd.h
+++ b/include/instrain_amd.h
@@ -407,6 +407,9 @@
                       int64_t cap_rec, int64_t ring_records, uint32_t *rec, uint32_t *gbase, int64_t *n_rec, int64_t *need_slack);
 int isx_encode_planes_mm(const isx_read_planes *reads, const isx_ref_planes *ref, int64_t n_pos, int32_t n_mm_bins, int32_t host_threads, int32_t slack_groups,
                          int64_t cap_rec, int64_t ring_records, uint32_t *rec, uint32_t *gbase, int64_t *n_rec, int64_t *need_slack);
+int isx_encode_planes_words(const isx_read_planes *reads, const isx_ref_planes *ref, int64_t n_pos, int32_t host_threads, int32_t slack_groups,
+                            int64_t cap_rec, uint32_t *rec, uint32_t *gbase, int64_t *n_rec, int64_t *need_slack,
+                            uint32_t *words, int64_t cap_words, int64_t *n_words);
 
 int isx_count_read_segs(int64_t n_reads, const uint32_t *cigar, const int64_t *cigar_off, const int64_t *ref_start,
                         const int64_t *clip_lo, const int64_t *clip_hi, int64_t *n_seg);
diff --git a/instrain_amd/_lib.py b/instrain_amd/_lib.py
--- a/instrain_amd/_lib.py
+++ b/instrain_amd/_lib.py
@@ -161,7 +161,7 @@
            "isx_batch_summarize", "isx_batch_summarize_genomes", "isx_batch_genome_coverage", "isx_snv_level_counts", "isx_ld_level_sums", "isx_compare_coverage", "isx_compare_scaffolds", "isx_compare_fetch_snps",
            "isx_genes_create", "isx_genes_destroy", "isx_genes_sites", "isx_batch_profile_genes", "isx_genes_profile_snvs",
            "isx_pipe_create", "isx_pipe_destroy", "isx_pipe_submit", "isx_pipe_submit_reads", "isx_pipe_stage_reads", "isx_pipe_submit_wire", "isx_wire_bytes", "isx_wire_free", "isx_wire_keep_reference", "isx_pipe_submit_bam", "isx_encode_segs", "isx_encode_segs_ring", "isx_seg_records_needed", "isx_encode_delta", "isx_delta_records_needed", "isx_count_read_segs", "isx_pack_reads", "isx_pipe_collect", "isx_pipe_release", "isx_pipe_fetch_entries", "isx_pipe_fetch_entries_shrunk", "isx_levels_expand", "isx_encode_obs", "isx_encode_obs_ring",
-           "isx_pack_ref_planes", "isx_planes_from_segs", "isx_pack_read_planes", "isx_pipe_submit_planes", "isx_pipe_stage_planes", "isx_encode_planes", "isx_encode_planes_mm", "isx_pipe_set_reference_budget", "isx_host_register", "isx_host_unregister",
+           "isx_pack_ref_planes", "isx_planes_from_segs", "isx_pack_read_planes", "isx_pipe_submit_planes", "isx_pipe_stage_planes", "isx_encode_planes", "isx_encode_planes_mm", "isx_encode_planes_words", "isx_pipe_set_reference_budget", "isx_host_register", "isx_host_unregister",
            "isx_bgzf_index", "isx_bgzf_inflate_device", "isx_bgzf_inflate_host", "isx_bgzf_inflate_fast",
            "isx_bam_open", "isx_bam_close", "isx_bam_close_wait", "isx_bam_set_threads", "isx_bam_ref", "isx_bam_set_priority_reads", "isx_bam_scan", "isx_bam_scan_part",
            "isx_bam_insert_sizes", "isx_bam_set_wanted_refs", "isx_bam_pair_keys", "isx_bam_set_cross_names", "isx_bam_filter_insert_sizes", "isx_bam_filter", "isx_bam_set_r2m", "isx_bam_r2m", "isx_bam_drop_names", "isx_bam_batch_pair_names", "isx_bam_set_mm_cap", "isx_bam_mm_levels", "isx_bam_set_mm_levels", "isx_bam_ref_counts",
@@ -287,6 +287,7 @@
     lib.isx_pipe_stage_planes.argtypes = [vp, i64, C.POINTER(RefPlanes), i32, vp, C.POINTER(ReadPlanes), C.POINTER(vp)]
     lib.isx_encode_planes.argtypes = [C.POINTER(ReadPlanes), C.POINTER(RefPlanes), i64, i32, i32, i64, i64, vp, vp, C.POINTER(i64), C.POINTER(i64)]
     lib.isx_encode_planes_mm.argtypes = [C.POINTER(ReadPlanes), C.POINTER(RefPlanes), i64, i32, i32, i32, i64, i64, vp, vp, C.POINTER(i64), C.POINTER(i64)]
+    lib.isx_encode_planes_words.argtypes = [C.POINTER(ReadPlanes), C.POINTER(RefPlanes), i64, i32, i32, i64, vp, vp, C.POINTER(i64), C.POINTER(i64), vp, i64, C.POINTER(i64)]
     lib.isx_bam_ref.argtypes = [vp, i32, C.POINTER(C.c_char_p), C.POINTER(i64), C.POINTER(i64)]
     lib.isx_bam_copy.argtypes = [vp, vp, vp, vp, vp]
     lib.isx_bam_view.argtypes = [vp, C.POINTER(vp), C.POINTER(vp)]
diff --git a/instrain_amd/csrc/isx_api.hip b/instrain_amd/csrc/isx_api.hip
--- a/instrain_amd/csrc/isx_api.hip
+++ b/instrain_amd/csrc/isx_api.hip
@@ -195,8 +195,8 @@
     std::lock_guard<std::mutex> lk(g_hreg_mu);
     for (size_t i = 0; i < g_hreg.size(); i++)
         if (g_hreg[i].a == a) {
+            HIP_TRY(hipHostUnregister(const_cast<void *>(ptr)));
             g_hreg.erase(g_hreg.begin() + (long)i);
-            HIP_TRY(hipHostUnregister(const_cast<void *>(ptr)));
             return ISX_OK;
         }
     isx_set_error("isx_host_unregister: not a registered range");
diff --git a/instrain_amd/csrc/isx_pipe.hip b/instrain_amd/csrc/isx_pipe.hip
--- a/instrain_amd/csrc/isx_pipe.hip
+++ b/instrain_amd/csrc/isx_pipe.hip
@@ -43,6 +43,7 @@
 }
 
 static const bool pipe_timing = getenv("ISX_PIPE_TIMING") != nullptr;
+static const bool pipe_ref_words = [] { const char *e = getenv("ISX_PIPE_REF_WORDS"); return !(e && e[0] == '0' && !e[1]); }();
 #define H2D(p, s) ((s).h2d ? (s).h2d : (p)->s_h2d)
 struct Slot {
     isx_batch *b = nullptr;
@@ -51,6 +52,7 @@
     size_t in_bytes = 0;
     size_t off_bounds = 0, off_win = 0, off_ref = 0, off_gbase = 0, off_ridx = 0, off_rec = 0;
     size_t off_pairs = 0;
+    size_t off_refw = 0, cap_refw = 0;
     isxenc::PairRun *h_runs = nullptr;
     bool runs_pinned = true;
     uint2 *d_runs = nullptr;
@@ -440,6 +442,8 @@
     s.off_bounds = o; o = up(o + (size_t)(p->pp.max_splits + 1) * sizeof(int64_t));
     s.off_win = o; o = up(o + ((size_t)cap_pos / 64 + 2) * sizeof(uint2));
     s.off_ref = o; o = up(o + ref2_bytes(cap_pos) + refn_bytes(cap_pos));
+    s.off_refw = o; s.cap_refw = 0;
+    if (p->drec && b->lean && b->M == 1 && pipe_ref_words) { s.cap_refw = ref2_bytes(cap_pos) / 2 / sizeof(uint2); o = up(o + s.cap_refw * sizeof(uint2)); }
     s.off_gbase = o; o = up(o + ((size_t)(p->cap_rec / p->G) + ISX_TAIL_GROUPS) * sizeof(uint32_t));
     s.off_ridx = o; if (prm->enable_linkage && !p->segs) o = up(o + ((size_t)p->cap_rec / ISX_CHUNK + 2) * sizeof(uint32_t));
     s.off_pairs = o; if (prm->enable_linkage && p->segs && !p->drec) o = up(o + (size_t)p->cap_rec * sizeof(uint32_t));
@@ -1099,7 +1103,35 @@
     }
 }
 
+__global__ void __launch_bounds__(256) k_ref_words(const uint2 *__restrict__ pairs, uint32_t n_pairs, uint32_t *__restrict__ plane, uint32_t n_words)
+{
+    const uint32_t i = blockIdx.x * 256u + threadIdx.x;
+    if (i >= n_pairs) return;
+    const uint2 pw = pairs[i];
+    if (pw.x < n_words) plane[pw.x] = pw.y;
+}
+
+static int64_t gather_ref_words(isxenc::HostPool &pool, const std::vector<std::vector<uint32_t>> &lists, const uint8_t *plane2, int64_t n_pos, uint2 *out, size_t cap)
+{
+    std::vector<size_t> at(lists.size() + 1, 0);
+    for (size_t t = 0; t < lists.size(); t++) at[t + 1] = at[t] + lists[t].size();
+    if (at.back() > cap) return -1;
+    const size_t b2 = ((size_t)n_pos + 3) / 4;
+    pool.run((int)lists.size(), [&](int t) {
+        uint2 *o = out + at[(size_t)t];
+        for (const uint32_t w : lists[(size_t)t]) {
+            uint32_t v = 0;
+            const size_t a = (size_t)w * 4;
+            if (a + 4 <= b2) memcpy(&v, plane2 + a, 4);
+            else for (size_t k = a; k < b2; k++) v |= (uint32_t)plane2[k] << (8 * (k - a));
+            *o++ = make_uint2(w, v);
+        }
+    });
+    return (int64_t)at.back();
+}
+
 struct RefStage {
+    bool words = false;
     bool early = false;
     uint8_t *resident = nullptr;
     double host_ms = 0.0;
@@ -1127,6 +1159,15 @@
         HIP_TRY(hipEventRecord(s.ev_h2da, st));
         out->early = true;
         out->host_ms = now_ms() - t_r;
+        return ISX_OK;
+    }
+
+    if (rp && !rp->key && s.cap_refw && !(rp->nplane && plane_any(*p->pool, rp->nplane, bn))) {
+        s.ref_has_n = false;
+        J.ref2 = rp->plane2; J.refn = nullptr; J.want_ref_words = true;
+        out->host_ms = now_ms() - t_r;
+        if (!ring) { HIP_TRY(hipEventRecord(s.ev_h2d0, st)); HIP_TRY(hipEventRecord(s.ev_h2da, st)); }
+        out->early = true; out->words = true;
         return ISX_OK;
     }
 
@@ -1155,6 +1196,35 @@
     if (!ring) HIP_TRY(hipEventRecord(s.ev_h2da, st));
     out->early = true;
     if (rp && rp->key) ref_cache_insert(p, s, rp, n_pos);
+    return ISX_OK;
+}
+
+static int send_ref_words(isx_pipe *p, Slot &s, int64_t n_pos, const isx_ref_planes *rp, const isxenc::SegJob &J, size_t *sent)
+{
+    hipStream_t st = H2D(p, s);
+    const double t0 = now_ms();
+    uint2 *h = reinterpret_cast<uint2 *>(s.h_in + s.off_refw), *d = reinterpret_cast<uint2 *>(s.d_in + s.off_refw);
+    const int64_t n = gather_ref_words(*p->pool, J.ref_words, rp->plane2, n_pos, h, s.cap_refw);
+    const size_t b2 = ((size_t)n_pos + 3) / 4;
+    if (n < 0) {
+        if (isx_host_is_registered(rp->plane2, b2)) HIP_TRY(hipMemcpyAsync(s.d_in + s.off_ref, rp->plane2, b2, hipMemcpyHostToDevice, st));
+        else {
+            (void)copy_ref_planes(*p->pool, rp, n_pos, s.h_in + s.off_ref, s.h_in + s.off_ref + ref2_bytes(n_pos));
+            HIP_TRY(hipMemcpyAsync(s.d_in + s.off_ref, s.h_in + s.off_ref, ref2_bytes(n_pos), hipMemcpyHostToDevice, st));
+        }
+        *sent = ref2_bytes(n_pos);
+    } else {
+        if (n > 0) {
+            HIP_TRY(hipMemcpyAsync(d, h, (size_t)n * sizeof(uint2), hipMemcpyHostToDevice, st));
+            const uint32_t n_words = (uint32_t)((b2 + 3) / 4);
+            hipLaunchKernelGGL(k_ref_words, dim3((unsigned)((n + 255) / 256)), dim3(256), 0, st, d, (uint32_t)n, reinterpret_cast<uint32_t *>(s.d_in + s.off_ref), n_words);
+            HIP_TRY(hipGetLastError());
+        }
+        *sent = (size_t)n * sizeof(uint2);
+    }
+    if (pipe_timing)
+        fprintf(stderr, "[isx_pipe_submit_reads] reference words %.3f ms: %lld of %lld plane words listed%s\n", now_ms() - t0, (long long)n,
+                (long long)((b2 + 3) / 4), n < 0 ? " (list too long: the whole plane travels)" : "");
     return ISX_OK;
 }
 
@@ -1321,6 +1391,8 @@
         }
         early_rec = true;
     }
+    size_t refw_sent = 0;
+    if (rs.words && (rc = send_ref_words(p, s, n_pos, rp, J, &refw_sent)) != ISX_OK) return rc;
     if (!planes_in) s.ref_has_n = isxenc::pack_ref_planes(*p->pool, ref, n_pos, s.h_in + s.off_ref, s.h_in + s.off_ref + ref2_bytes(n_pos));
     const double t_ref = now_ms();
     memcpy(s.h_in + s.off_bounds, split_bounds, (size_t)(n_splits + 1) * sizeof(int64_t));
@@ -1351,6 +1423,7 @@
     if (ring) { if (feed.bytes != rec_bytes) { isx_set_error("internal: the staging ring did not carry the whole stream"); return ISX_ERR_STATE; } }
     else if (!early_rec) HIP_TRY(hipMemcpyAsync(s.d_in + s.off_rec, s.h_in + s.off_rec, rec_bytes, hipMemcpyHostToDevice, H2D(p, s)));
     s.h2d_bytes = (int64_t)(head + gb_bytes + rec_bytes) - (rs.resident ? (int64_t)ref_bytes : 0);
+    if (rs.words) s.h2d_bytes += (int64_t)refw_sent - (int64_t)ref_bytes;
     if (linkage && !p->drec) {
         HIP_TRY(hipMemcpyAsync(s.d_in + s.off_pairs, s.h_in + s.off_pairs, (size_t)b->n_rec * sizeof(uint32_t), hipMemcpyHostToDevice, H2D(p, s)));
         s.h2d_bytes += (int64_t)b->n_rec * 4;
diff --git a/instrain_amd/csrc/seg_encode.cpp b/instrain_amd/csrc/seg_encode.cpp
--- a/instrain_amd/csrc/seg_encode.cpp
+++ b/instrain_amd/csrc/seg_encode.cpp
@@ -546,7 +546,18 @@
     bool fast_store;
     int64_t used = 0, np = 0, nb = 0;
     uint32_t maxp = 0;
+    std::vector<uint32_t> *wl = nullptr;
+    uint32_t wl_last = 0xFFFFFFFFu;
 };
+
+inline void note_ref_words(std::vector<uint32_t> &wl, uint32_t &last, uint32_t p, const uint64_t ex[3])
+{
+    for (int k = 0; k < 3; k++)
+        for (uint64_t e = ex[k]; e; e &= e - 1) {
+            const uint32_t w = (p + 64u * (uint32_t)k + (uint32_t)__builtin_ctzll(e)) >> 4;
+            if (w != last) { wl.push_back(w); last = w; }
+        }
+}
 
 inline void put_empty_drec(uint32_t *o)
 {
@@ -656,6 +667,7 @@
     constexpr size_t group_words = (size_t)ISX_DREC_GROUP * ISX_DREC_WORDS;
     const bool fast_store = cpu_has_avx512() && (reinterpret_cast<uintptr_t>(J.rec) & 63) == 0;
     const int variant = planes_variant();
+    if (J.want_ref_words) J.ref_words.resize((size_t)n_tasks);
     if (n == 0) {
         if (RG) J.wave_begin(0);
         for (int r = 0; r < ISX_DREC_GROUP; r++) put_empty_drec(J.rec + (size_t)r * ISX_DREC_WORDS);
@@ -689,6 +701,7 @@
         K.a = a; K.e = e; K.gp = gp; K.ln = ln; K.mm = mmv; K.pr = pr; K.pl = pl; K.gpos_all = gpos_all;
         K.rec0 = RG ? J.rec + (size_t)((int64_t)half * RG) * group_words : J.rec;
         K.g0 = RG ? wave_g0 : 0; K.ga = g_at[(size_t)t]; K.ge = g_at[(size_t)t + 1]; K.fast_store = fast_store;
+        if (J.want_ref_words) { K.wl = &J.ref_words[(size_t)t]; K.wl->clear(); }
         if (variant == 2) planes_task_avx512(J, err, K);
         else if (variant == 1) planes_task_bmi2(J, err, K);
         else planes_task_portable(J, err, K);
@@ -1054,8 +1067,27 @@
     return isx_encode_planes_mm(reads, ref, n_pos, 1, host_threads, slack_groups, cap_rec, ring_records, rec, gbase, n_rec, need_slack);
 }
 
+static int encode_planes_host(const isx_read_planes *reads, const isx_ref_planes *ref, int64_t n_pos, int32_t n_mm_bins, int32_t host_threads, int32_t slack_groups,
+                              int64_t cap_rec, int64_t ring_records, uint32_t *rec, uint32_t *gbase, int64_t *n_rec, int64_t *need_slack,
+                              uint32_t *words, int64_t cap_words, int64_t *n_words);
+
 int isx_encode_planes_mm(const isx_read_planes *reads, const isx_ref_planes *ref, int64_t n_pos, int32_t n_mm_bins, int32_t host_threads, int32_t slack_groups,
                          int64_t cap_rec, int64_t ring_records, uint32_t *rec, uint32_t *gbase, int64_t *n_rec, int64_t *need_slack)
+{
+    return encode_planes_host(reads, ref, n_pos, n_mm_bins, host_threads, slack_groups, cap_rec, ring_records, rec, gbase, n_rec, need_slack, nullptr, 0, nullptr);
+}
+
+int isx_encode_planes_words(const isx_read_planes *reads, const isx_ref_planes *ref, int64_t n_pos, int32_t host_threads, int32_t slack_groups,
+                            int64_t cap_rec, uint32_t *rec, uint32_t *gbase, int64_t *n_rec, int64_t *need_slack,
+                            uint32_t *words, int64_t cap_words, int64_t *n_words)
+{
+    if (!n_words || cap_words < 0 || (cap_words && !words)) { isx_set_error("isx_encode_planes_words: bad argument"); return ISX_ERR_ARG; }
+    return encode_planes_host(reads, ref, n_pos, 1, host_threads, slack_groups, cap_rec, 0, rec, gbase, n_rec, need_slack, words, cap_words, n_words);
+}
+
+static int encode_planes_host(const isx_read_planes *reads, const isx_ref_planes *ref, int64_t n_pos, int32_t n_mm_bins, int32_t host_threads, int32_t slack_groups,
+                              int64_t cap_rec, int64_t ring_records, uint32_t *rec, uint32_t *gbase, int64_t *n_rec, int64_t *need_slack,
+                              uint32_t *words, int64_t cap_words, int64_t *n_words)
 {
     if (n_mm_bins < 1 || n_mm_bins > 128) { isx_set_error("isx_encode_planes: n_mm_bins must be in [1, 128]"); return ISX_ERR_ARG; }
     if (!reads || !ref || !ref->plane2 || !rec || !gbase || !n_rec || reads->n_seg < 0 || cap_rec < ISX_DREC_GROUP || (cap_rec % ISX_DREC_GROUP) || n_pos <= 0 ||
@@ -1086,9 +1118,16 @@
             std::fill_n(r0 + (size_t)h * half * ISX_DREC_WORDS, (size_t)half * ISX_DREC_WORDS, 0xABABABABu);
         };
     }
+    J.want_ref_words = n_words != nullptr;
     const int rc = isxenc::encode_planes(pool, J);
     if (need_slack) *need_slack = J.need_slack;
     *n_rec = J.n_rec;
+    if (n_words) {
+        int64_t n = 0;
+        for (const std::vector<uint32_t> &l : J.ref_words)
+            for (uint32_t w : l) { if (n < cap_words) words[n] = w; n++; }
+        *n_words = n;
+    }
     if (rc == isxenc::SEG_CAPACITY) {
         isx_set_error(J.need_slack > J.slack_groups ? "isx_encode_planes: a task needs more spare groups than slack_groups (see *need_slack)"
                                                     : "isx_encode_planes: the stream does not fit cap_rec records");
diff --git a/instrain_amd/csrc/seg_encode.h b/instrain_amd/csrc/seg_encode.h
--- a/instrain_amd/csrc/seg_encode.h
+++ b/instrain_amd/csrc/seg_encode.h
@@ -38,6 +38,8 @@
     std::vector<int64_t> task_need;
     const int64_t *task_groups = nullptr;
     int64_t n_pieces = 0;
+    bool want_ref_words = false;
+    std::vector<std::vector<uint32_t>> ref_words;
     int64_t n_rec = 0;
     int64_t n_bases = 0;
     uint32_t max_pair = 0;
diff --git a/instrain_amd/csrc/seg_planes.inc b/instrain_amd/csrc/seg_planes.inc
--- a/instrain_amd/csrc/seg_planes.inc
+++ b/instrain_amd/csrc/seg_planes.inc
@@ -113,7 +113,83 @@
 #endif
     const bool mm_on = J.n_mm_bins > 1;
     const int64_t pf_end = K.e - PLANES_PREFETCH;
+#if ISX_PLANES_VARIANT == 2
+    alignas(32) uint64_t fx[ISX_DREC_GROUP][4];
+    const bool fast_groups = K.fast_store && !refn && !mm_on;
+    const __m256i no_exc_v = _mm256_set1_epi32((int)ISX_DREC_NO_EXC);
+    auto fast_group = [&](int64_t s0) __attribute__((always_inline)) -> bool {
+        const uint32_t base = gp[s0];
+        uint32_t bad = 0, prev = base;
+        for (int i = 0; i < ISX_DREC_GROUP; i++) {
+            const uint32_t p = gp[s0 + i], L = ln[s0 + i];
+            bad |= (uint32_t)(p < prev) | (uint32_t)((int64_t)p >= safe_pos) | (uint32_t)(L - 1u >= (uint32_t)ISX_SEG_BASES) | (uint32_t)(p != ga[s0 + i]);
+            prev = p;
+        }
+        if (bad || prev - base > SPAN) return false;
+        int64_t gnb = 0;
+        uint32_t gmaxp = maxp, glast = 0, excm = 0;
+        int plain_any = 0;
+        for (int i = 0; i < ISX_DREC_GROUP; i++) {
+            const int64_t q = s0 + i;
+            const uint32_t L = ln[q], p = gp[q];
+            const uint64_t *P = K.pl + (size_t)q * ISX_PLANE_WORDS;
+            if (q < pf_end) {
+                _mm_prefetch(reinterpret_cast<const char *>(P + (size_t)PLANES_PREFETCH * ISX_PLANE_WORDS), _MM_HINT_T0);
+                _mm_prefetch(reinterpret_cast<const char *>(ref2 + (gp[q + PLANES_PREFETCH] >> 2) + 40), _MM_HINT_T0);
+            }
+            const uint32_t pid = pr ? pr[q] : 0u;
+            gmaxp = pid > gmaxp ? pid : gmaxp;
+            gnb += L;
+            glast = std::max(glast, p + L - 1);
+            const __m512i Pv = _mm512_loadu_si512(P);
+            const __m256i lmv = _mm256_load_si256(reinterpret_cast<const __m256i *>(LM.m[L]));
+            const __m256i skv = _mm256_and_si256(_mm256_maskz_loadu_epi64((__mmask8)0x7, P + 5), lmv);
+            const __m256i dv = ISX_DIFFERS_FN(ref2 + (p >> 2), (p & 3u) * 2u, Pv);
+            const __m256i exv = _mm256_and_si256(dv, _mm256_xor_si256(skv, lmv));
+            plain_any |= _mm256_testz_si256(skv, skv);
+            excm |= (uint32_t)!_mm256_testz_si256(exv, exv) << i;
+            _mm256_store_si256(reinterpret_cast<__m256i *>(fx[i]), exv);
+            __m256i v = _mm256_permutex2var_epi32(skv, rec_idx, no_exc_v);
+            v = _mm256_mask_set1_epi32(v, (__mmask8)0x01, (int)((p - base) | (L << 16)));
+            v = _mm256_mask_set1_epi32(v, (__mmask8)0x80, (int)pid);
+            _mm256_store_si256(reinterpret_cast<__m256i *>(G.rec[i]), v);
+        }
+        if (plain_any) return false;
+        for (uint32_t m = excm; m; m &= m - 1) {
+            const uint64_t *e = fx[__builtin_ctz(m)];
+            if (__builtin_popcountll(e[0]) + __builtin_popcountll(e[1]) + __builtin_popcountll(e[2]) > ISX_DREC_EXC_FULL) return false;
+        }
+        for (uint32_t m = excm; m; m &= m - 1) {
+            const int i = __builtin_ctz(m);
+            uint64_t *e = fx[i];
+            const uint64_t *P = K.pl + (size_t)(s0 + i) * ISX_PLANE_WORDS;
+            if (K.wl) note_ref_words(*K.wl, K.wl_last, gp[s0 + i], e);
+            uint64_t fields = 0;
+            uint32_t nf = 0;
+            for (int k = 0; k < 3; k++)
+                for (; e[k]; e[k] &= e[k] - 1, nf++) {
+                    const uint32_t col = (uint32_t)(64 * k + __builtin_ctzll(e[k]));
+                    const uint64_t code = (P[col >> 5] >> (2 * (col & 31u))) & 3u;
+                    fields |= ((uint64_t)col | (code << 8)) << (10 * nf);
+                }
+            G.rec[i][3] = (uint32_t)(fields | (0x0FFFFFFFFFFFFFFFull << (10 * nf))) & ISX_DREC_NO_EXC;
+        }
+        uint32_t *o = K.rec0 + (size_t)(G.g - K.g0) * (size_t)ISX_DREC_GROUP * ISX_DREC_WORDS;
+        for (int r = 0; r < ISX_DREC_GROUP; r += 2) _mm512_stream_si512(reinterpret_cast<__m512i *>(o + (size_t)r * ISX_DREC_WORDS), _mm512_load_si512(G.rec[r]));
+        J.gbase[G.g] = base; J.cmin[G.g] = base; J.cmax[G.g] = glast; J.cany[G.g] = 1;
+        G.g++; G.used++;
+        nb += gnb; np += ISX_DREC_GROUP; maxp = gmaxp;
+        return true;
+    };
+#endif
     for (int64_t s = K.a; s < K.e; s++) {
+#if ISX_PLANES_VARIANT == 2
+        if (fast_groups) {
+            if (G.n == ISX_DREC_GROUP && G.open < 0) ISX_CLOSE_FN(J, K, G);
+            while (G.n == 0 && G.g < K.ge && s + ISX_DREC_GROUP <= K.e && fast_group(s)) s += ISX_DREC_GROUP;
+            if (s >= K.e) break;
+        }
+#endif
         const uint32_t L = ln[s], p = gp[s];
         const uint64_t *P = K.pl + (size_t)s * ISX_PLANE_WORDS;
         if (s < pf_end) {
@@ -194,6 +270,7 @@
                 ex[2] |= even_bits_portable(P[4]) & s2;
             }
         }
+        if (K.wl && (ex[0] | ex[1] | ex[2])) note_ref_words(*K.wl, K.wl_last, p, ex);
         const bool plain = (s0 | s1 | s2) == 0;
         const uint32_t n_exc = (uint32_t)(__builtin_popcountll(ex[0]) + __builtin_popcountll(ex[1]) + __builtin_popcountll(ex[2]));
         if (__builtin_expect(n_exc <= 1, 1)) {
```
